# Nahuel-M/StereoVisionArray

Hardware: AMD Instinct MI355X
Metric: Mdisparities/sec (W·H·D/s) at 1080p D=128 (higher is better)
Workload: dtype u16

## Files before the change

### stereovisionarray_amd/csrc/sgm_common.h

```cpp
#pragma once

#include <utility>

#include "sva_device.h"
#include "sva_internal.h"
#include "sva_tuning.h"

namespace sva {
namespace sgm {

template <class F, int... S>
__device__ __forceinline__ void for_seq_impl(std::integer_sequence<int, S...>, F&& f) {
    (f(std::integral_constant<int, S>{}), ...);
}
template <int N, class F>
__device__ __forceinline__ void for_seq(F&& f) {
    for_seq_impl(std::make_integer_sequence<int, N>{}, static_cast<F&&>(f));
}

constexpr unsigned INF2 = 0x7fff7fffu;

struct PathGeom {
    int W, H, D;
    int P1, P2;
    int blk_h;
    int blk_w;
    size_t vol;
    int ckpt;
    int ns;
    size_t ckvol;
    int nsy;
    size_t ckvvol;
    int npair;
    size_t cstr, lstr, ckstr, ckvstr;
    int pair;
    int dreal;
};


typedef __amdgpu_buffer_rsrc_t rsrc_t;


constexpr int kStoreNT = 2;

__device__ __forceinline__ rsrc_t make_rsrc(const void* base, size_t bytes) {
    return __builtin_amdgcn_make_buffer_rsrc(const_cast<void*>(base), (short)0,
                                             (int)(unsigned)bytes, 0x00020000);
}

template <int NW>
struct Words {
    unsigned w[NW];
};

template <int NW, int AUX = tune::kCLoadAux>
__device__ __forceinline__ Words<NW> bload(rsrc_t r, unsigned off) {
    Words<NW> o;
    if constexpr (NW == 1) {
        o.w[0] = __builtin_amdgcn_raw_buffer_load_b32(r, off, 0, AUX);
    } else if constexpr (NW == 2) {
        auto v = __builtin_amdgcn_raw_buffer_load_b64(r, off, 0, AUX);
        o.w[0] = v[0]; o.w[1] = v[1];
    } else if constexpr (NW == 3) {
        auto v = __builtin_amdgcn_raw_buffer_load_b96(r, off, 0, AUX);
        o.w[0] = v[0]; o.w[1] = v[1]; o.w[2] = v[2];
    } else {
        auto v = __builtin_amdgcn_raw_buffer_load_b128(r, off, 0, AUX);
        o.w[0] = v[0]; o.w[1] = v[1]; o.w[2] = v[2]; o.w[3] = v[3];
    }
    return o;
}

template <int NW, int AUX = kStoreNT>
__device__ __forceinline__ void bstore(rsrc_t r, unsigned off, const unsigned (&w)[NW]) {
    if constexpr (NW == 1) {
        __builtin_amdgcn_raw_buffer_store_b32(w[0], r, off, 0, AUX);
    } else if constexpr (NW == 2) {
        typedef unsigned v2u __attribute__((ext_vector_type(2)));
        __builtin_amdgcn_raw_buffer_store_b64((v2u){w[0], w[1]}, r, off, 0, AUX);
    } else if constexpr (NW == 3) {
        typedef unsigned v3u __attribute__((ext_vector_type(3)));
        __builtin_amdgcn_raw_buffer_store_b96((v3u){w[0], w[1], w[2]}, r, off, 0, AUX);
    } else {
        typedef unsigned v4u __attribute__((ext_vector_type(4)));
        __builtin_amdgcn_raw_buffer_store_b128((v4u){w[0], w[1], w[2], w[3]}, r, off, 0, AUX);
    }
}

__device__ __forceinline__ unsigned add3(unsigned a, unsigned b, unsigned c) {
    unsigned r;
    asm("v_add3_u32 %0, %1, %2, %3" : "=v"(r) : "v"(a), "v"(b), "v"(c));
    return r;
}

template <bool DIAG>
struct Cursor {
    int x;
    unsigned off;
    __device__ __forceinline__ bool advance(int rx, unsigned stride, int W, unsigned WD) {
        off += stride;
        if constexpr (DIAG) {
            x += rx;
            const bool hi = x >= W, lo = x < 0;
            x = hi ? x - W : (lo ? x + W : x);
            off = hi ? off - WD : (lo ? off + WD : off);
            return hi || lo;
        }
        return false;
    }
};

__device__ __forceinline__ unsigned min3_u16x2(unsigned a, unsigned b, unsigned c) {
    unsigned r;
    asm("v_pk_minimum3_f16 %0, %1, %2, %3" : "=v"(r) : "v"(a), "v"(b), "v"(c));
    return r;
}

template <int NP>
__device__ __forceinline__ unsigned lane_min_u16(const unsigned (&A)[NP]) {
    unsigned mm[NP];
#pragma unroll
    for (int j = 0; j < NP; j++) mm[j] = A[j];
    int n = NP;
#pragma unroll
    for (int it = 0; it < 4; it++) {
        if (n > 1) {
            int o = 0, i = 0;
#pragma unroll
            for (int q = 0; q < 8; q++) {
                if (i + 2 < n) { mm[o++] = min3_u16x2(mm[i], mm[i + 1], mm[i + 2]); i += 3; }
                else if (i + 1 < n) { mm[o++] = as_u32(vmin2(as_v2(mm[i]), as_v2(mm[i + 1]))); i += 2; }
                else if (i < n) { mm[o++] = mm[i]; i += 1; }
            }
            n = o;
        }
    }
    const u16x2 mf = as_v2(mm[0]);
    return mf.x < mf.y ? mf.x : mf.y;
}

template <int DPL> __host__ __device__ constexpr int pair_d(int j, int h) {
    return tune::kSplitPairs ? j + h * (DPL / 2) : 2 * j + h;
}
template <int DPL> __host__ __device__ constexpr int pair_of(int e) {
    return tune::kSplitPairs ? e % (DPL / 2) : e >> 1;
}
template <int DPL> __host__ __device__ constexpr int half_of(int e) {
    return tune::kSplitPairs ? e / (DPL / 2) : e & 1;
}

template <int DPL>
__device__ __forceinline__ void words_to_pairs(const unsigned (&w)[DPL / 4], unsigned (&A)[DPL / 2]) {
    constexpr int NW = DPL / 4, NP = DPL / 2;
    if constexpr (tune::kSplitPairs != 0) {
#pragma unroll
        for (int j = 0; j < NP; j++) {
            constexpr unsigned Z = 0x0cu;
            const int el = j, eh = j + NP;
            const unsigned sel = (unsigned)(el & 3) | (Z << 8) | ((4u + (unsigned)(eh & 3)) << 16) | (Z << 24);
            A[j] = __builtin_amdgcn_perm(w[eh >> 2], w[el >> 2], sel);
        }
    } else {
#pragma unroll
        for (int q = 0; q < NW; q++) unpack4(w[q], A[2 * q], A[2 * q + 1]);
    }
}

template <int DPL>
__device__ __forceinline__ void pairs_to_words(const unsigned (&A)[DPL / 2], unsigned (&ow)[DPL / 4]) {
    constexpr int NW = DPL / 4, NP = DPL / 2;
    if constexpr (tune::kSplitPairs != 0) {
        unsigned T[NP / 2];
#pragma unroll
        for (int i = 0; i < NP / 2; i++) T[i] = __builtin_amdgcn_perm(A[2 * i + 1], A[2 * i], 0x06020400u);
        if constexpr (NP == 2) {
            ow[0] = T[0];
        } else {
#pragma unroll
            for (int q = 0; q < NW; q++) {
                const int e0 = 4 * q, e2 = 4 * q + 2;
                const int a = (e0 % NP) / 2, ha = e0 / NP, b = (e2 % NP) / 2, hb = e2 / NP;
                const unsigned sel = (unsigned)(2 * ha) | ((unsigned)(2 * ha + 1) << 8) |
                                     ((unsigned)(4 + 2 * hb) << 16) | ((unsigned)(5 + 2 * hb) << 24);
                ow[q] = __builtin_amdgcn_perm(T[b], T[a], sel);
            }
        }
    } else {
#pragma unroll
        for (int w = 0; w < NW; w++) ow[w] = pack4(A[2 * w], A[2 * w + 1]);
    }
}

struct Edges {
    unsigned X = INF2, Y = INF2;
};

template <int DPL, bool PIN = false>
__device__ __forceinline__ void sgm_step_c(const unsigned (&c)[DPL / 2], unsigned (&A)[DPL / 2],
                                           unsigned& m, unsigned (&ow)[DPL / 4], unsigned P1,
                                           unsigned P2, Edges& e) {
    constexpr int NP = DPL / 2;
    e.X = row_shr1(A[NP - 1], e.X);
    e.Y = row_shl1(A[0], e.Y);
    const unsigned X = e.X, Y = e.Y;
    unsigned lo[NP], hi[NP];
    if constexpr (tune::kSplitPairs != 0) {
#pragma unroll
        for (int j = 0; j < NP; j++) {
            lo[j] = j == 0 ? __builtin_amdgcn_alignbit(A[NP - 1], X, 16) : A[j - 1];
            hi[j] = j == NP - 1 ? __builtin_amdgcn_alignbit(Y, A[0], 16) : A[j + 1];
        }
    } else {
        unsigned M[NP];
        M[0] = __builtin_amdgcn_alignbit(A[0], X, 16);
#pragma unroll
        for (int j = 1; j < NP; j++) M[j] = __builtin_amdgcn_alignbit(A[j], A[j - 1], 16);
        const unsigned Qlast = __builtin_amdgcn_alignbit(Y, A[NP - 1], 16);
#pragma unroll
        for (int j = 0; j < NP; j++) {
            lo[j] = M[j];
            hi[j] = j < NP - 1 ? M[j + 1] : Qlast;
        }
    }
    unsigned K, mP2;
    asm("v_mul_i32_i24_e32 %0, 0xfffeffff, %1" : "=v"(K) : "v"(m));
    if constexpr (tune::kStepMadP2 != 0) {
        asm("v_mad_u32_u24 %0, %1, %2, %3" : "=&v"(mP2) : "v"(m), "s"(0x10001u), "v"(P2 * 0x10001u));
    } else {
        mP2 = P2 * 0x10001u - K;
    }
    u16x2 t[NP];
#pragma unroll
    for (int j = 0; j < NP; j++) t[j] = vmin2(as_v2(lo[j]), as_v2(hi[j]));
    unsigned tp[NP];
    if constexpr (tune::kStepAddU32 != 0) {
        const unsigned P1x2 = P1 * 0x10001u;
#pragma unroll
        for (int j = 0; j < NP; j++) tp[j] = as_u32(t[j]) + P1x2;
    } else {
#pragma unroll
        for (int j = 0; j < NP; j++) tp[j] = as_u32(t[j] + splat2(P1));
    }
#pragma unroll
    for (int j = 0; j < NP; j++) A[j] = add3(min3_u16x2(tp[j], A[j], mP2), c[j], K);
    pairs_to_words<DPL>(A, ow);
    m = row_min_u32<PIN>(lane_min_u16<NP>(A));
}

template <int DPL>
__device__ __forceinline__ void sgm_step_c(const unsigned (&c)[DPL / 2], unsigned (&A)[DPL / 2],
                                           unsigned& m, unsigned (&ow)[DPL / 4], unsigned P1,
                                           unsigned P2) {
    Edges e;
    sgm_step_c<DPL>(c, A, m, ow, P1, P2, e);
}

template <int DPL, bool PIN = false>
__device__ __forceinline__ void sgm_step(const unsigned (&cw)[DPL / 4], unsigned (&A)[DPL / 2],
                                         unsigned& m, unsigned (&ow)[DPL / 4], unsigned P1,
                                         unsigned P2, Edges& e) {
    unsigned c[DPL / 2];
    words_to_pairs<DPL>(cw, c);
    sgm_step_c<DPL, PIN>(c, A, m, ow, P1, P2, e);
}

__device__ __forceinline__ void dir_of(int r, int& rx, int& ry) {
    constexpr int T[8][2] = {{1, 0}, {-1, 0}, {0, 1}, {0, -1}, {1, 1}, {-1, -1}, {-1, 1}, {1, -1}};
    rx = T[r][0];
    ry = T[r][1];
}

template <int DPL> constexpr int pf_h() {
    return DPL == 4 ? tune::kPfH4 : DPL == 8 ? tune::kPfH8 : DPL == 12 ? tune::kPfH12 : tune::kPfH16;
}
template <int DPL> constexpr int pf_v() {
    return DPL == 4 ? tune::kPfV4 : DPL == 8 ? tune::kPfV8 : DPL == 12 ? tune::kPfV12 : tune::kPfV16;
}


template <int DPL, bool DIAG, int PF, int CKPT = 0, int SL = 0>
__device__ __forceinline__ void path_line(rsrc_t rC, rsrc_t rL, const PathGeom& g, int rx, int ry,
                                          int line, int k, rsrc_t rCK) {
    constexpr int NW = DPL / 4, NP = DPL / 2;
    const int W = g.W, H = g.H, D = g.D;
    const unsigned P1 = (unsigned)g.P1, P2 = (unsigned)g.P2;
    const int steps = ry == 0 ? W : H;
    const unsigned WD = (unsigned)W * (unsigned)D;
    const unsigned stride = (unsigned)((ry * W + rx) * D);
    int x0, y0;
    if (ry == 0) { y0 = line; x0 = rx > 0 ? 0 : W - 1; }
    else { y0 = ry > 0 ? 0 : H - 1; x0 = line; }
    Cursor<false> cc;
    cc.x = x0;
    cc.off = ((unsigned)y0 * (unsigned)W + (unsigned)x0) * (unsigned)D + (unsigned)(k * DPL);
    Cursor<false> pc = cc;
    constexpr bool STATIC_HITS = DPL <= tune::kStaticCkptHitsMaxDpl && (CKPT == 1 || CKPT == 2) &&
                                 SL > 0 && PF % (1 << SL) == 0;
    int lead = 0;
    if constexpr (STATIC_HITS) {
        constexpr int SEG = 1 << SL;
        lead = CKPT == 1 ? (rx > 0 ? 0 : (SEG - W % SEG) % SEG) : (ry > 0 ? 0 : (SEG - H % SEG) % SEG);
        pc.off -= (unsigned)lead * stride;
    }
    const int nsteps = steps + lead;
    int twc = 0, twp = 0, Tc = 0, Tp = 0;
    if constexpr (DIAG) {
        const int j = (int)((threadIdx.x >> 4) & 3);
        const int l0 = __builtin_amdgcn_readfirstlane(line - j);
        twc = twp = rx > 0 ? W - line : line + 1;
        Tc = Tp = rx > 0 ? W - l0 - 3 : l0 + 1;
    }
    const bool narrow = W < 4;

    unsigned A[NP];
#pragma unroll
    for (int j = 0; j < NP; j++) A[j] = 0u;
    unsigned m = 0u;
    Edges edges;

    Words<NW> ring[PF];
#pragma unroll
    for (int p = 0; p < PF; p++) {
        ring[p] = bload<NW>(rC, pc.off);
        if constexpr (STATIC_HITS) {
#pragma unroll
            for (int w = 0; w < NW; w++) ring[p].w[w] = p < lead ? 0u : ring[p].w[w];
        }
        pc.off += stride;
        if constexpr (DIAG) {
            if (p < PF - 1) {
                const bool w = p + 1 == twp;
                const unsigned fixed = rx > 0 ? pc.off - WD : pc.off + WD;
                pc.off = w ? fixed : pc.off;
                twp = w ? twp + W : twp;
            }
        }
    }
    if constexpr (DIAG) {
        while (Tp + 3 < PF) Tp += W;
    }

    auto step = [&](int p, bool refill, int ts) {
        unsigned cw[NW];
#pragma unroll
        for (int w = 0; w < NW; w++) cw[w] = ring[p].w[w];
        unsigned ow[NW];
        sgm_step<DPL>(cw, A, m, ow, P1, P2, edges);
        if constexpr (CKPT == 1 && STATIC_HITS) {
            constexpr int SEG = 1 << SL;
            if ((p & (SEG - 1)) == SEG - 1) {
                const int x = rx > 0 ? ts : W - 1 - (ts - lead);
                if (rx > 0 ? x + 1 < W : x > 0)
                    bstore<NW, tune::kCkptStoreAux>(rCK, ((unsigned)(y0 * g.ns + (x >> SL)) * (unsigned)D +
                                             (unsigned)(k * DPL)), ow);
            }
        } else if constexpr (CKPT == 2 && STATIC_HITS) {
            constexpr int SEG = 1 << SL;
            if ((p & (SEG - 1)) == SEG - 1) {
                const int y = ry > 0 ? ts : H - 1 - (ts - lead);
                if (ry > 0 ? y + 1 < H : y > 0)
                    bstore<NW, tune::kCkptStoreAux>(rCK, ((unsigned)((y >> SL) * W + x0) * (unsigned)D +
                                             (unsigned)(k * DPL)), ow);
            }
        } else if constexpr (CKPT == 1) {
            const int x = rx > 0 ? ts : W - 1 - ts;
            constexpr int SEG = 1 << SL;
            const bool hit = rx > 0 ? (((x + 1) & (SEG - 1)) == 0 && x + 1 < W)
                                    : ((x & (SEG - 1)) == 0 && x > 0);
            if (__builtin_expect(hit, 0))
                bstore<NW, tune::kCkptStoreAux>(rCK, ((unsigned)(y0 * g.ns + (x >> SL)) * (unsigned)D +
                                         (unsigned)(k * DPL)), ow);
        } else if constexpr (CKPT == 3) {
            const int y = ry > 0 ? ts : H - 1 - ts;
            constexpr int SEG = 1 << SL;
            const bool hit = ry > 0 ? (((y + 1) & (SEG - 1)) == 0 && y + 1 < H)
                                    : ((y & (SEG - 1)) == 0 && y > 0);
            if (__builtin_expect(hit, 0))
                bstore<NW, tune::kCkptStoreAux>(rCK, cc.off - (unsigned)(y - (y >> SL)) * WD, ow);
        } else if constexpr (CKPT == 2) {
            const int y = ry > 0 ? ts : H - 1 - ts;
            constexpr int SEG = 1 << SL;
            const bool hit = ry > 0 ? (((y + 1) & (SEG - 1)) == 0 && y + 1 < H)
                                    : ((y & (SEG - 1)) == 0 && y > 0);
            if (__builtin_expect(hit, 0))
                bstore<NW, tune::kCkptStoreAux>(rCK, ((unsigned)((y >> SL) * W + x0) * (unsigned)D +
                                         (unsigned)(k * DPL)), ow);
        } else {
            bstore<NW>(rL, cc.off, ow);
        }
        cc.off += stride;
        if constexpr (DIAG) {
            const int ec = ts + 1 - Tc;
            const int ep = ts + PF - Tp;
            const bool cev = narrow || (unsigned)ec < 4u;
            const bool pev = refill && (narrow || (unsigned)ep < 4u);
            if (__builtin_expect(cev || pev, 0)) {
                if (cev) {
                    const bool wrapped = ts + 1 == twc;
                    const unsigned fixed = rx > 0 ? cc.off - WD : cc.off + WD;
                    cc.off = wrapped ? fixed : cc.off;
                    twc = wrapped ? twc + W : twc;
#pragma unroll
                    for (int j = 0; j < NP; j++) A[j] = wrapped ? 0u : A[j];
                    m = wrapped ? 0u : m;
                    if (ec == 3) Tc += W;
                }
                if (pev) {
                    const bool wrapped = ts + PF == twp;
                    const unsigned fixed = rx > 0 ? pc.off - WD : pc.off + WD;
                    pc.off = wrapped ? fixed : pc.off;
                    twp = wrapped ? twp + W : twp;
                    if (ep == 3) Tp += W;
                }
            }
        }
        if (refill) {
            __builtin_amdgcn_sched_barrier(0);
            ring[p] = bload<NW>(rC, pc.off);
            pc.off += stride;
            __builtin_amdgcn_sched_barrier(0);
        }
    };

    int t = 0;
    for (; t + PF <= nsteps; t += PF) {
#pragma unroll
        for (int p = 0; p < PF; p++) step(p, true, t + p);
    }
#pragma unroll
    for (int p = 0; p < PF; p++)
        if (t + p < nsteps) step(p, false, t + p);
}



template <int NW>
__device__ __forceinline__ void unpack_add(const unsigned (&w)[NW], unsigned (&S)[2 * NW]) {
    unsigned a[2 * NW];
    words_to_pairs<4 * NW>(w, a);
#pragma unroll
    for (int j = 0; j < 2 * NW; j++) S[j] += a[j];
}

template <int DPL, bool PAD, bool PIN = false>
__device__ __forceinline__ void state_from_words(const Words<DPL / 4>& w, unsigned (&A)[DPL / 2],
                                                 unsigned& m, const unsigned (&padm)[DPL / 2]) {
    constexpr int NP = DPL / 2;
    words_to_pairs<DPL>(w.w, A);
    if constexpr (PAD) {
#pragma unroll
        for (int j = 0; j < NP; j++) A[j] |= padm[j] & 0x00ff00ffu;
    }
    if constexpr (tune::kStateMinTree) {
        m = row_min_u32<PIN>(lane_min_u16<NP>(A));
    } else {
        unsigned mm = 0xffffffffu;
#pragma unroll
        for (int j = 0; j < NP; j++) {
            const unsigned lo = A[j] & 0xffffu, hi = A[j] >> 16;
            mm = mm < lo ? mm : lo;
            mm = mm < hi ? mm : hi;
        }
        m = row_min_u32<PIN>(mm);
    }
}
template <int DPL, bool PAD, bool PIN = false>
__device__ __forceinline__ void load_state(rsrc_t r, unsigned off, unsigned (&A)[DPL / 2],
                                           unsigned& m, const unsigned (&padm)[DPL / 2]) {
    state_from_words<DPL, PAD, PIN>(bload<DPL / 4>(r, off), A, m, padm);
}

template <int DPL, int PF, int SL>
__device__ __forceinline__ void pair_line(rsrc_t rC, rsrc_t rE, const PathGeom& g, int rx, int line,
                                          int role, int k, rsrc_t rCK) {
    constexpr int NW = DPL / 4, NP = DPL / 2, SEG = 1 << SL;
    static_assert(PF >= SEG, "the lead steps sit in the prefetch prologue");
    const int W = g.W, H = g.H;
    const unsigned uW = (unsigned)W, uD = (unsigned)g.D;
    const unsigned WD = uW * uD;
    const unsigned P1 = (unsigned)g.P1, P2 = (unsigned)g.P2;
    const unsigned lane_d = (unsigned)(k * DPL);
    const int nseg = (H + SEG - 1) >> SL;
    const int qs = nseg >> 1;
    const int M = qs << SL;
    const bool up = role != 0;
    auto wrap = [&](int x) { return x >= W ? x - W : (x < 0 ? x + W : x); };
    auto col_of = [&](int y) {
        const int x = (line + rx * y) % W;
        return x < 0 ? x + W : x;
    };

    unsigned A1[NP], m1 = 0u;
    {
        const int n1 = M > H - M ? M : H - M;
        const int lead = n1 - (up ? H - M : M);
        const int ry = up ? -1 : 1, rxl = up ? -rx : rx;
        const int yv = up ? H - 1 + lead : -lead;
        const int xv = col_of(yv);
        const unsigned stride = (unsigned)((ry * W + rxl) * g.D);
        const unsigned wfix = rxl > 0 ? 0u - WD : WD;
        unsigned coff = (unsigned)(yv * W + xv) * uD + lane_d;
        unsigned poff = coff;
        int twc = rxl > 0 ? W - xv : xv + 1, twp = twc;
        const int zT = 1 - (n1 - M) - SEG, zB = H - 1 + (n1 - (H - M)) - (M + SEG);
        const int z0 = up ? zB : zT;
        const int zn = up ? H - (M + SEG) : M - 2 * SEG + 1;
#pragma unroll
        for (int j = 0; j < NP; j++) A1[j] = 0u;
        Edges e1;
        Words<NW> ring[PF];
#pragma unroll
        for (int p = 0; p < PF; p++) {
            ring[p] = bload<NW>(rC, poff);
#pragma unroll
            for (int w = 0; w < NW; w++) ring[p].w[w] = p < lead ? 0u : ring[p].w[w];
            poff += stride;
            if (p < PF - 1) {
                const bool wr = p + 1 == twp;
                poff = wr ? poff + wfix : poff;
                twp = wr ? twp + W : twp;
            }
        }
        auto step = [&](int p, bool refill, int ts) {
            unsigned cw[NW];
#pragma unroll
            for (int w = 0; w < NW; w++) cw[w] = ring[p].w[w];
            unsigned ow[NW];
            sgm_step<DPL>(cw, A1, m1, ow, P1, P2, e1);
            if (__builtin_expect((((zT + ts) & (SEG - 1)) == 0) | (((zB - ts) & (SEG - 1)) == 0), 0)) {
                const int zc = up ? z0 - ts : z0 + ts;
                if ((zc & (SEG - 1)) == 0 && zc >= 0 && zc < zn) {
                    const int y = zc + (up ? M + SEG : SEG - 1);
                    bstore<NW, tune::kCkptStoreAux>(rCK, coff - (unsigned)(y - (y >> SL)) * WD, ow);
                }
            }
            coff += stride;
            const bool cwr = ts + 1 == twc;
            const bool pwr = refill && ts + PF == twp;
            if (__builtin_expect(__builtin_amdgcn_ballot_w64(cwr || pwr) != 0, 0)) {
                coff = cwr ? coff + wfix : coff;
                twc = cwr ? twc + W : twc;
#pragma unroll
                for (int j = 0; j < NP; j++) A1[j] = cwr ? 0u : A1[j];
                m1 = cwr ? 0u : m1;
                poff = pwr ? poff + wfix : poff;
                twp = pwr ? twp + W : twp;
            }
            if (refill) {
                __builtin_amdgcn_sched_barrier(0);
                ring[p] = bload<NW>(rC, poff);
                poff += stride;
                __builtin_amdgcn_sched_barrier(0);
            }
        };
        int t = 0;
        for (; t + PF <= n1; t += PF) {
#pragma unroll
            for (int p = 0; p < PF; p++) step(p, true, t + p);
        }
#pragma unroll
        for (int p = 0; p < PF; p++)
            if (t + p < n1) step(p, false, t + p);
    }
    asm volatile("s_waitcnt vmcnt(0)" ::: "memory");

    const int nit = nseg - qs;
    const int xdn = rx > 0 ? 0 : W - 1, xup = rx > 0 ? W - 1 : 0;
    unsigned padm[NP];
#pragma unroll
    for (int j = 0; j < NP; j++) {
        const int dl = k * DPL + pair_d<DPL>(j, 0), dh = k * DPL + pair_d<DPL>(j, 1);
        padm[j] = (dl >= g.dreal ? 0x0000ffffu : 0u) | (dh >= g.dreal ? 0xffff0000u : 0u);
    }
    auto seg_of = [&](int i) {
        const int s = up ? qs - 1 - i : qs + i;
        return s < 0 ? 0 : s;
    };
    int s8 = (SEG * rx) % W;
    s8 = s8 < 0 ? s8 + W : s8;
    const int ds8 = up ? -s8 : s8;
    struct SegLoads {
        Words<NW> c[SEG], ck;
    };
    auto issue = [&](int s, int x, SegLoads& b) {
        const int xa = wrap(x - rx);
#pragma unroll
        for (int r = 0; r < SEG; r++) {
            b.c[r] = bload<NW>(rC, ((unsigned)((s << SL) + r) * uW + (unsigned)x) * uD + lane_d);
            x = wrap(x + rx);
        }
        const bool has = up ? s > 0 : s + 1 < nseg;
        const unsigned o = ((unsigned)(up ? s - 1 : s + 1) * uW + (unsigned)(up ? xa : x)) * uD + lane_d;
        b.ck = bload<NW, 16>(rCK, has ? o : lane_d);
    };
    auto reset_if = [&](bool rs, unsigned (&A)[NP], unsigned& m) {
        if (__builtin_expect(__builtin_amdgcn_ballot_w64(rs) != 0, 0)) {
#pragma unroll
            for (int j = 0; j < NP; j++) A[j] = rs ? 0u : A[j];
            m = rs ? 0u : m;
        }
    };

    unsigned Ad[NP], md = up ? 0u : m1, Au[NP], mu = up ? m1 : 0u;
#pragma unroll
    for (int j = 0; j < NP; j++) {
        Ad[j] = up ? 0u : A1[j];
        Au[j] = up ? A1[j] : 0u;
    }
    Edges ed, eu;
    SegLoads cur, nxt;
    int xs = col_of(seg_of(0) << SL), xn = xs;
    issue(seg_of(0), xs, cur);
    for (int i = 0; i < nit; i++) {
        __builtin_amdgcn_sched_barrier(0);
        if (i + 1 < nit) {
            xn = wrap(xs + ds8);
            issue(seg_of(i + 1), xn, nxt);
        }
        __builtin_amdgcn_sched_barrier(0);
        const int s = seg_of(i);
        const bool act = !up || i < qs;
        const int y0 = s << SL;
        const int nr = H - y0 < SEG ? H - y0 : SEG;
        int x[SEG];
        x[0] = xs;
#pragma unroll
        for (int r = 1; r < SEG; r++) x[r] = wrap(x[r - 1] + rx);
        {
            const bool has = up ? s > 0 : s + 1 < nseg;
            unsigned Ak[NP], mk;
            state_from_words<DPL, true>(cur.ck, Ak, mk, padm);
#pragma unroll
            for (int j = 0; j < NP; j++) {
                const unsigned a = has ? Ak[j] : 0u;
                Ad[j] = up ? a : Ad[j];
                Au[j] = up ? Au[j] : a;
            }
            mk = has ? mk : 0u;
            md = up ? mk : md;
            mu = up ? mu : mk;
        }
        unsigned Dn[SEG][NW];
        auto down_row = [&](int r, const Words<NW>& c) {
            unsigned cp[NP], ow[NW], t[NP];
            words_to_pairs<DPL>(c.w, cp);
            sgm_step_c<DPL>(cp, Ad, md, ow, P1, P2, ed);
#pragma unroll
            for (int j = 0; j < NP; j++) t[j] = Ad[j] - cp[j];
            pairs_to_words<DPL>(t, Dn[r]);
        };
        auto up_row = [&](const Words<NW>& c, unsigned (&e)[NW]) {
            unsigned cp[NP], ow[NW], t[NP];
            words_to_pairs<DPL>(c.w, cp);
            sgm_step_c<DPL>(cp, Au, mu, ow, P1, P2, eu);
#pragma unroll
            for (int j = 0; j < NP; j++) t[j] = Au[j] - cp[j];
            pairs_to_words<DPL>(t, e);
        };
        const bool inner = rx > 0 ? x[0] >= 1 && x[0] + SEG <= W - 1 : x[0] - SEG >= 0 && x[0] <= W - 2;
        if (__builtin_expect(__builtin_amdgcn_ballot_w64(!inner || nr != SEG || !act) == 0, 1)) {
            unsigned Up[SEG][NW];
            const unsigned off0 = ((unsigned)y0 * uW + (unsigned)x[0]) * uD + lane_d;
            const unsigned stride = (unsigned)((W + rx) * (int)uD);
            for_seq<SEG>([&](auto I) {
                constexpr int rd = decltype(I)::value, ru = SEG - 1 - rd;
                down_row(rd, cur.c[rd]);
                up_row(cur.c[ru], Up[ru]);
                if constexpr (rd >= SEG / 2) {
                    unsigned e[NW];
#pragma unroll
                    for (int w = 0; w < NW; w++) e[w] = Dn[rd][w] + Up[rd][w];
                    bstore<NW>(rE, off0 + (unsigned)rd * stride, e);
#pragma unroll
                    for (int w = 0; w < NW; w++) e[w] = Dn[ru][w] + Up[ru][w];
                    bstore<NW>(rE, off0 + (unsigned)ru * stride, e);
                }
            });
        } else {
            for_seq<SEG>([&](auto R) {
                constexpr int r = decltype(R)::value;
                if (r < nr && act) {
                    reset_if(x[r] == xdn, Ad, md);
                    down_row(r, cur.c[r]);
                }
            });
            for_seq<SEG>([&](auto Q) {
                constexpr int r = SEG - 1 - decltype(Q)::value;
                if (r < nr && act) {
                    reset_if(x[r] == xup, Au, mu);
                    unsigned e[NW];
                    up_row(cur.c[r], e);
#pragma unroll
                    for (int w = 0; w < NW; w++) e[w] += Dn[r][w];
                    bstore<NW>(rE, ((unsigned)(y0 + r) * uW + (unsigned)x[r]) * uD + lane_d, e);
                }
            });
        }
        if (i + 1 < nit) {
            cur = nxt;
            xs = xn;
        }
    }
}

}
}
```

### stereovisionarray_amd/csrc/sgm_paths.hip

```cpp
#include "sgm_common.h"
#include "sva_tuning.h"

namespace sva {
namespace {

using namespace sgm;

constexpr int PATH_BLOCK = 256;
constexpr int LINES_PER_BLOCK = PATH_BLOCK / 16;
constexpr int PAIR_LINES = LINES_PER_BLOCK / 2;

template <int DPL, bool PAIR>
__global__ __launch_bounds__(PATH_BLOCK) void sgm_paths_kernel(const uint8_t* __restrict__ C,
                                                               uint8_t* __restrict__ L8,
                                                               uint8_t* __restrict__ CK,
                                                               uint8_t* __restrict__ CKV,
                                                               PathGeom g) {
    int b = blockIdx.x, r, lb, f;
    if constexpr (PAIR) {
        f = 0;
        const int npb = 4 * g.blk_w;
        if (b < npb) {
            r = 4 + 2 * (b & 1);
            lb = b >> 1;
            __builtin_amdgcn_s_setprio(3);
        } else if (b < npb + 2 * g.blk_h) {
            b -= npb;
            r = b / g.blk_h;
            lb = b - r * g.blk_h;
            __builtin_amdgcn_s_setprio(1);
        } else {
            b -= npb + 2 * g.blk_h;
            r = 2 + (b & 1);
            lb = b >> 1;
        }
    } else if (b < 2 * g.blk_h * g.npair) {
        f = b / (2 * g.blk_h);
        b -= f * 2 * g.blk_h;
        r = b / g.blk_h;
        lb = b - r * g.blk_h;
        __builtin_amdgcn_s_setprio(1);
    } else {
        b -= 2 * g.blk_h * g.npair;
        f = b / (6 * g.blk_w);
        b -= f * 6 * g.blk_w;
        r = 2 + b % 6;
        lb = b / 6;
    }
    C += (size_t)f * g.cstr;
    L8 += (size_t)f * g.lstr;
    if (g.ckpt) {
        CK += (size_t)f * g.ckstr;
        CKV += (size_t)f * g.ckvstr;
    }
    int line = lb * LINES_PER_BLOCK + (threadIdx.x >> 4);
    int role = 0;
    if constexpr (PAIR) {
        if (r >= 4) {
            const int row = (int)(threadIdx.x >> 4);
            line = lb * PAIR_LINES + 2 * (row >> 2) + (row & 1);
            role = (row >> 1) & 1;
        }
    }
    const int k = threadIdx.x & 15;
    const int nlines = r < 2 ? g.H : g.W;
    if (line >= nlines) return;
    int rx, ry;
    dir_of(r, rx, ry);
    const rsrc_t rC = make_rsrc(C, g.vol);
    constexpr int SL = DPL <= 8 ? tune::kWtahvTileLog2 : tune::kWtahvTileLog2Wide;
    constexpr bool DOWN = diag_ckpt_down(DPL), UP = diag_ckpt_up(DPL);
    if constexpr (PAIR) {
        if (r >= 4) {
            const int pr = r == 4 ? 0 : 1;
            const rsrc_t rCK = make_rsrc(CKV + (size_t)(2 + pr) * g.ckvvol, g.ckvvol);
            const rsrc_t rE = make_rsrc(L8 + (size_t)pr * g.vol, g.vol);
            pair_line<DPL, pf_v<DPL>(), SL>(rC, rE, g, rx, line, role, k, rCK);
        } else if (r >= 2) {
            const rsrc_t rCK = make_rsrc(CKV + (size_t)(r - 2) * g.ckvvol, g.ckvvol);
            path_line<DPL, false, pf_v<DPL>(), 2, SL>(rC, rC, g, rx, ry, line, k, rCK);
        } else {
            const rsrc_t rCK = make_rsrc(CK + (size_t)r * g.ckvol, g.ckvol);
            path_line<DPL, false, pf_h<DPL>(), 1, SL>(rC, rC, g, rx, ry, line, k, rCK);
        }
    } else if (r >= 4 && g.ckpt && (ry > 0 ? DOWN : UP)) {
        const int plane = ry > 0 ? 2 + (r == 4 ? 0 : 1) : 2 + (DOWN ? 2 : 0) + (r == 5 ? 0 : 1);
        const rsrc_t rCK = make_rsrc(CKV + (size_t)plane * g.ckvvol, g.ckvvol);
        path_line<DPL, true, pf_v<DPL>(), 3, SL>(rC, rC, g, rx, ry, line, k, rCK);
    } else if (r >= 4) {
        const int slot = !g.ckpt ? r
                       : DOWN ? (r == 5 ? 0 : 1)
                       : UP ? (r == 4 ? 0 : 1)
                       : r - 4;
        const rsrc_t rL = make_rsrc(L8 + (size_t)slot * g.vol, g.vol);
        path_line<DPL, true, pf_v<DPL>()>(rC, rL, g, rx, ry, line, k, rL);
    } else if (r >= 2 && g.ckpt) {
        const rsrc_t rCK = make_rsrc(CKV + (size_t)(r - 2) * g.ckvvol, g.ckvvol);
        path_line<DPL, false, pf_v<DPL>(), 2, SL>(rC, rC, g, rx, ry, line, k, rCK);
    } else if (r >= 2) {
        const rsrc_t rL = make_rsrc(L8 + (size_t)r * g.vol, g.vol);
        path_line<DPL, false, pf_v<DPL>()>(rC, rL, g, rx, ry, line, k, rL);
    } else if (g.ckpt) {
        const rsrc_t rCK = make_rsrc(CK + (size_t)r * g.ckvol, g.ckvol);
        path_line<DPL, false, pf_h<DPL>(), 1, SL>(rC, rC, g, rx, ry, line, k, rCK);
    } else {
        const rsrc_t rL = make_rsrc(L8 + (size_t)r * g.vol, g.vol);
        path_line<DPL, false, pf_h<DPL>()>(rC, rL, g, rx, ry, line, k, rL);
    }
}

template <int DPL, bool EN>
void paths_launch(bool pair, dim3 grid, hipStream_t s, hipEvent_t start, hipEvent_t stop,
                  const uint8_t* C, uint8_t* L8, uint8_t* CK, uint8_t* CKV, const PathGeom& g) {
    if constexpr (EN) {
        if (pair) {
            hipExtLaunchKernelGGL((sgm_paths_kernel<DPL, true>), grid, dim3(PATH_BLOCK), 0, s, start,
                                  stop, 0, C, L8, CK, CKV, g);
            return;
        }
    }
    hipExtLaunchKernelGGL((sgm_paths_kernel<DPL, false>), grid, dim3(PATH_BLOCK), 0, s, start, stop,
                          0, C, L8, CK, CKV, g);
}

}

bool paths_supported(int D) { return D == 64 || D == 128 || D == 192 || D == 256; }

TileGeom tile_geom(int W, int H, int D) {
    TileGeom t;
    t.seg_log2 = D <= 128 ? tune::kWtahvTileLog2 : tune::kWtahvTileLog2Wide;
    const int seg = 1 << t.seg_log2;
    t.ntx = (W + 15) >> 4;
    t.nty = (H + seg - 1) >> t.seg_log2;
    t.nsx = (W + seg - 1) >> t.seg_log2;
    t.hck_bytes = 2 * (size_t)H * t.nsx * D;
    t.vck_bytes = 2 * (size_t)t.nty * W * D;
    const int dpl = D / 16;
    const int ndp = (diag_ckpt_down(dpl) ? 2 : 0) + (diag_ckpt_up(dpl) ? 2 : 0);
    t.dck_bytes = (size_t)ndp / 2 * t.vck_bytes;
    t.nvol = 4 - ndp;
    return t;
}

bool diag_pair_enabled(int D) {
    return (D == 64 && tune::kDiagPair4) || (D == 128 && tune::kDiagPair8) ||
           (D == 192 && tune::kDiagPair12) || (D == 256 && tune::kDiagPair16);
}

hipError_t launch_paths(Ctx& c, const uint8_t* C, int W, int H, int D, int P1, int P2,
                        uint8_t* L8, uint8_t* CK, uint8_t* CKV, int npair, bool pair, int dreal) {
    DispatchTimer t(c, "sgm_paths");
    PathGeom g;
    g.W = W; g.H = H; g.D = D; g.P1 = P1; g.P2 = P2;
    g.blk_h = (H + LINES_PER_BLOCK - 1) / LINES_PER_BLOCK;
    g.blk_w = (W + LINES_PER_BLOCK - 1) / LINES_PER_BLOCK;
    g.vol = (size_t)W * H * D;
    if ((CK == nullptr) != (CKV == nullptr)) return hipErrorInvalidValue;
    g.ckpt = CK ? 2 : 0;
    const TileGeom tg = tile_geom(W, H, D);
    g.nsy = tg.nty;
    g.ckvvol = tg.vck_bytes / 2;
    g.ns = tg.nsx;
    g.ckvol = tg.hck_bytes / 2;
    if (g.vol >= (size_t)1 << 32) return hipErrorInvalidValue;
    if (npair < 1 || (npair > 1 && !CK)) return hipErrorInvalidValue;
    g.npair = npair;
    g.cstr = g.vol;
    g.lstr = (size_t)tg.nvol * g.vol;
    g.ckstr = tg.hck_bytes;
    g.ckvstr = tg.vck_bytes + tg.dck_bytes;
    if (pair && (!CK || npair != 1 || 2 * P2 > 255 || !diag_pair_enabled(D) ||
                 tile_geom(W, H, D).nvol != 4))
        return hipErrorInvalidValue;
    g.pair = pair ? 1 : 0;
    g.dreal = dreal > 0 && dreal < D ? dreal : D;
    dim3 grid((unsigned)((2 * g.blk_h + 6 * g.blk_w) * npair));
    t.used = true;
    switch (D) {
        case 64: paths_launch<4, tune::kDiagPair4 != 0>(pair, grid, c.stream, t.start, t.stop, C, L8, CK, CKV, g); break;
        case 128: paths_launch<8, tune::kDiagPair8 != 0>(pair, grid, c.stream, t.start, t.stop, C, L8, CK, CKV, g); break;
        case 192: paths_launch<12, tune::kDiagPair12 != 0>(pair, grid, c.stream, t.start, t.stop, C, L8, CK, CKV, g); break;
        case 256: paths_launch<16, tune::kDiagPair16 != 0>(pair, grid, c.stream, t.start, t.stop, C, L8, CK, CKV, g); break;
        default: t.used = false; return hipErrorInvalidValue;
    }
    return hipGetLastError();
}

}
```

### stereovisionarray_amd/csrc/sva_api.cpp

```cpp
#include <hip/hip_runtime.h>

#include <algorithm>
#include <cstdio>
#include <cstring>
#include <new>
#include <string>
#include <functional>
#include <thread>
#include <vector>

#include "sva_internal.h"
#include "sva_tuning.h"

using namespace sva;

namespace sva {

hipEvent_t KernelTimer::get_event() {
    if (!pool.empty()) {
        hipEvent_t e = pool.back();
        pool.pop_back();
        return e;
    }
    hipEvent_t e = nullptr;
    if (hipEventCreate(&e) != hipSuccess) return nullptr;
    return e;
}

void KernelTimer::begin(hipStream_t s, const char*, hipEvent_t* start_out) {
    hipEvent_t e = get_event();
    if (e && hipEventRecord(e, s) == hipSuccess) *start_out = e;
    else *start_out = nullptr;
}

void KernelTimer::end(hipStream_t s, const char* name, hipEvent_t start) {
    hipEvent_t e = get_event();
    if (!e) return;
    if (hipEventRecord(e, s) != hipSuccess) { pool.push_back(e); return; }
    pending.push_back(Pending{name, start, e});
}

hipError_t KernelTimer::resolve() {
    hipError_t st = hipSuccess;
    for (auto& p : pending) {
        float ms = 0.f;
        hipError_t e = hipEventSynchronize(p.stop);
        if (e == hipSuccess) e = hipEventElapsedTime(&ms, p.start, p.stop);
        if (e != hipSuccess) st = e;
        auto& t = totals[p.name];
        t.first += ms;
        t.second += 1;
        pool.push_back(p.start);
        pool.push_back(p.stop);
    }
    pending.clear();
    return st;
}

void KernelTimer::release_all() {
    for (auto& p : pending) {
        (void)hipEventDestroy(p.start);
        (void)hipEventDestroy(p.stop);
    }
    pending.clear();
    for (auto e : pool) (void)hipEventDestroy(e);
    pool.clear();
}

hipError_t DevBuf::ensure(size_t n) {
    if (n <= bytes && ptr) return hipSuccess;
    if (ptr) {
        (void)hipFree(ptr);
        ptr = nullptr;
        bytes = 0;
    }
    size_t want = std::max<size_t>(n, 256);
    hipError_t e = flags ? hipExtMallocWithFlags(&ptr, want, flags) : hipMalloc(&ptr, want);
    if (e != hipSuccess) {
        ptr = nullptr;
        return e;
    }
    bytes = want;
    return hipSuccess;
}

void DevBuf::release() {
    if (ptr) (void)hipFree(ptr);
    ptr = nullptr;
    bytes = 0;
}

}

namespace {

Ctx* as_ctx(void* p) { return static_cast<Ctx*>(p); }

int fail(Ctx* c, int code, const std::string& msg) {
    if (c) c->last_error = msg;
    return code;
}

int hip_fail(Ctx* c, hipError_t e, const char* what) {
    std::string m = std::string(what) + ": " + hipGetErrorString(e);
    if (e == hipErrorOutOfMemory || e == hipErrorMemoryAllocation)
        return fail(c, SVA_ERR_OUT_OF_MEMORY, m);
    return fail(c, SVA_ERR_DEVICE, m);
}

#define SVA_HIP(c, expr, what)                           \
    do {                                                 \
        hipError_t _e = (expr);                          \
        if (_e != hipSuccess) return hip_fail(c, _e, what); \
    } while (0)

#define SVA_CHECK_CTX(c)                                                       \
    do {                                                                       \
        if (!(c)) return SVA_ERR_INVALID_ARG;                                  \
        if (hipSetDevice((c)->device) != hipSuccess)                           \
            return fail(c, SVA_ERR_DEVICE, "hipSetDevice failed");             \
    } while (0)

int check_image(Ctx* c, const void* a, int W, int H, size_t pitch) {
    if (!a) return fail(c, SVA_ERR_INVALID_ARG, "null image pointer");
    if (W <= 0 || H <= 0) return fail(c, SVA_ERR_INVALID_ARG, "image size must be positive");
    if (pitch < (size_t)W) return fail(c, SVA_ERR_INVALID_ARG, "pitch smaller than width");
    if ((long long)W * H > (1ll << 31) - 1) return fail(c, SVA_ERR_INVALID_ARG, "image too large");
    return SVA_OK;
}

int check_sgm(Ctx* c, const sva_sgm_params* p, int W, int H, bool native = false) {
    if (!p) return fail(c, SVA_ERR_INVALID_ARG, "null params");
    if (p->D <= 0) return fail(c, SVA_ERR_INVALID_ARG, "D must be positive");
    const int Dp = padded_D(p->D);
    if (!Dp) return fail(c, SVA_ERR_UNSUPPORTED, "GPU path built for D in 1..256");
    if (native && !paths_supported(p->D))
        return fail(c, SVA_ERR_UNSUPPORTED,
                    "stage entry points take D in {64,128,192,256} (whole frames: any D <= 256)");
    if (p->dir < -255 || p->dir > 255 || p->dir_y < -255 || p->dir_y > 255 ||
        (p->dir == 0 && p->dir_y == 0))
        return fail(c, SVA_ERR_INVALID_ARG, "(dir, dir_y) must be a nonzero step, |comp| <= 255");
    if (p->dmin < 0) return fail(c, SVA_ERR_INVALID_ARG, "dmin must be >= 0");
    if (p->dmin + p->D > 65535)
        return fail(c, SVA_ERR_INVALID_ARG, "dmin + D must fit the u16 disparity map");
    if (p->P1 < 0 || p->P2 < 0 || p->P1 > 193 || p->P2 > 193)
        return fail(c, SVA_ERR_INVALID_ARG, "penalties must satisfy 0 <= P1, P2 <= 193");
    if (p->lr_check && p->lr_max_diff < 0)
        return fail(c, SVA_ERR_INVALID_ARG, "lr_max_diff must be >= 0");
    if (H > 65535) return fail(c, SVA_ERR_UNSUPPORTED, "H must be <= 65535");
    if (W > 0 && H > 0 && (unsigned long long)W * (unsigned long long)H * (unsigned)Dp >=
                              (1ull << 32))
        return fail(c, SVA_ERR_UNSUPPORTED, "W*H*D must be < 2^32 (32-bit volume offsets)");
    return SVA_OK;
}

size_t pair_ckpt_bytes(const TileGeom& tg) { return tg.hck_bytes + tg.vck_bytes + tg.vck_bytes; }

int paths_wta(Ctx* c, const uint8_t* C, int W, int H, const sva_sgm_params* p, int Dp,
              uint16_t* disp, float* sub) {
    if (!wta_hv_supported(Dp)) return fail(c, SVA_ERR_UNSUPPORTED, "no tile pipeline for this D");
    const size_t nv = (size_t)W * H * (size_t)Dp;
    const TileGeom tg = tile_geom(W, H, Dp);
    const long long minpx = c->dbg_pair_min_pixels >= 0 ? (long long)c->dbg_pair_min_pixels
                                                        : tune::kDiagPairMinPixels;
    const bool pair = tg.nvol == 4 && diag_pair_ok(Dp, p->P2) && (long long)W * H >= minpx;
    SVA_HIP(c, c->paths.ensure(nv * (pair ? 2 : tg.nvol)), "path workspace");
    SVA_HIP(c, c->ckpt.ensure(pair ? pair_ckpt_bytes(tg) : tg.hck_bytes + tg.vck_bytes + tg.dck_bytes),
            "checkpoint workspace");
    uint8_t* L4 = (uint8_t*)c->paths.ptr;
    uint8_t* CK = (uint8_t*)c->ckpt.ptr;
    uint8_t* CKV = CK + tg.hck_bytes;
    SVA_HIP(c, launch_paths(*c, C, W, H, Dp, p->P1, p->P2, L4, CK, CKV, 1, pair, p->D), "paths launch");
    SVA_HIP(c, launch_wta_hv(*c, C, L4, CK, CKV, W, H, Dp, p->P1, p->P2, p->dmin, disp, sub, p->D, 1,
                             pair),
            "wta launch");
    c->last_diag_route = pair ? 1 : 0;
    return SVA_OK;
}

sva_tile_layout tile_layout(int W, int H, int D) {
    sva_tile_layout l;
    std::memset(&l, 0, sizeof(l));
    const TileGeom tg = tile_geom(W, H, D);
    l.seg = 1 << tg.seg_log2;
    l.nsx = tg.nsx;
    l.nsy = tg.nty;
    l.cost_bytes = (size_t)W * H * (size_t)D;
    l.diag_volumes = tg.nvol;
    l.diag_bytes = (size_t)tg.nvol * l.cost_bytes;
    l.hckpt_bytes = tg.hck_bytes;
    l.vckpt_bytes = tg.vck_bytes + tg.dck_bytes;
    return l;
}

int check_tile_buffers(Ctx* c, int W, int H, int D, const void* C, size_t C_bytes,
                       const void* diag, size_t diag_bytes, const void* hck, size_t hck_bytes,
                       const void* vck, size_t vck_bytes) {
    const sva_tile_layout l = tile_layout(W, H, D);
    if (!C || (!diag && l.diag_bytes) || !hck || !vck)
        return fail(c, SVA_ERR_INVALID_ARG, "null stage buffer");
    if (C_bytes < l.cost_bytes) return fail(c, SVA_ERR_INVALID_ARG, "cost buffer smaller than [H][W][D]");
    if (diag_bytes < l.diag_bytes)
        return fail(c, SVA_ERR_INVALID_ARG, "diagonal volume buffer smaller than [nvol][H][W][D]");
    if (hck_bytes < l.hckpt_bytes)
        return fail(c, SVA_ERR_INVALID_ARG, "horizontal checkpoint buffer smaller than [2][H][nsx][D]");
    if (vck_bytes < l.vckpt_bytes)
        return fail(c, SVA_ERR_INVALID_ARG, "row checkpoint buffer smaller than [np][nsy][W][D]");
    return SVA_OK;
}

int run_sgm_device(Ctx* c, const uint8_t* left, const uint8_t* right, int W, int H, size_t pitch,
                   const sva_sgm_params* p, uint16_t* disp, float* sub) {
    const int Dp = padded_D(p->D);
    const size_t np = (size_t)W * H, nv = np * (size_t)Dp;
    int s;
    SVA_HIP(c, c->cost.ensure(nv), "cost workspace");
    uint8_t* C = (uint8_t*)c->cost.ptr;
    uint16_t* dr = nullptr;
    if (p->lr_check) {
        SVA_HIP(c, c->disp_r.ensure(np * 2), "lr workspace");
        dr = (uint16_t*)c->disp_r.ptr;
    }
    if (p->dir_y == 0 && Dp >= tune::kCensusCostMinD && census_cost_supported(Dp)) {
        SVA_HIP(c, launch_census_cost(*c, left, right, W, H, pitch, Dp, p->dmin, p->dir, C, p->D),
                "cost launch");
        if ((s = paths_wta(c, C, W, H, p, Dp, disp, sub))) return s;
        if (p->lr_check) {
            SVA_HIP(c, launch_census_cost(*c, right, left, W, H, pitch, Dp, p->dmin, -p->dir, C,
                                          p->D),
                    "cost launch");
            if ((s = paths_wta(c, C, W, H, p, Dp, dr, nullptr))) return s;
            SVA_HIP(c, launch_lr_check(*c, disp, dr, sub, W, H, p->dir, 0, p->lr_max_diff,
                                       p->invalid),
                    "lr launch");
        }
        return SVA_OK;
    }
    if (census_cost2_supported(Dp, p->dir, p->dir_y)) {
        SVA_HIP(c, launch_census_cost2(*c, left, right, W, H, pitch, Dp, p->dmin, p->dir,
                                       p->dir_y, C, p->D),
                "cost launch");
        if ((s = paths_wta(c, C, W, H, p, Dp, disp, sub))) return s;
        if (p->lr_check) {
            SVA_HIP(c, launch_census_cost2(*c, right, left, W, H, pitch, Dp, p->dmin, -p->dir,
                                           -p->dir_y, C, p->D),
                    "cost launch");
            if ((s = paths_wta(c, C, W, H, p, Dp, dr, nullptr))) return s;
            SVA_HIP(c, launch_lr_check(*c, disp, dr, sub, W, H, p->dir, p->dir_y, p->lr_max_diff,
                                       p->invalid),
                    "lr launch");
        }
        return SVA_OK;
    }
    SVA_HIP(c, c->census_l.ensure(np * 8), "census workspace");
    SVA_HIP(c, c->census_r.ensure(np * 8), "census workspace");
    uint64_t* cl = (uint64_t*)c->census_l.ptr;
    uint64_t* cr = (uint64_t*)c->census_r.ptr;
    SVA_HIP(c, launch_census_pair(*c, left, right, W, H, pitch, cl, cr), "census launch");
    SVA_HIP(c, launch_cost2(*c, cl, cr, W, H, Dp, p->dmin, p->dir, p->dir_y, C, p->D),
            "cost launch");
    if ((s = paths_wta(c, C, W, H, p, Dp, disp, sub))) return s;
    if (p->lr_check) {
        SVA_HIP(c, launch_cost2(*c, cr, cl, W, H, Dp, p->dmin, -p->dir, -p->dir_y, C, p->D),
                "cost launch");
        if ((s = paths_wta(c, C, W, H, p, Dp, dr, nullptr))) return s;
        SVA_HIP(c, launch_lr_check(*c, disp, dr, sub, W, H, p->dir, p->dir_y, p->lr_max_diff,
                                   p->invalid),
                "lr launch");
    }
    return SVA_OK;
}

int run_sgm_batch(Ctx* c, const sva_pair_d* jobs, int n, int W, int H, size_t pitch,
                  uint16_t* maps, float* sub) {
    const sva_sgm_params* p = &jobs[0].params;
    const int Dp = padded_D(p->D);
    const size_t np = (size_t)W * H, nv = np * (size_t)Dp;
    const TileGeom tg = tile_geom(W, H, Dp);
    const size_t ckb = tg.hck_bytes + tg.vck_bytes + tg.dck_bytes;
    const int sb = tune::kBatchSubFrames > 0 ? std::min(n, tune::kBatchSubFrames) : n;
    const int nsub = (n + sb - 1) / sb;
    SVA_HIP(c, c->cost.ensure(nv * n), "cost workspace");
    SVA_HIP(c, c->paths.ensure(nv * tg.nvol * sb), "path workspace");
    SVA_HIP(c, c->ckpt.ensure(ckb * sb), "checkpoint workspace");
    uint8_t* C = (uint8_t*)c->cost.ptr;
    const int ns = std::min(n, tune::kBatchCostStreams);
    if (ns > 1) {
        while ((int)c->side.size() < ns) {
            hipStream_t s = nullptr;
            SVA_HIP(c, hipStreamCreateWithFlags(&s, hipStreamNonBlocking), "side stream");
            c->side.push_back(s);
        }
        while ((int)c->side_done.size() < ns * nsub) {
            hipEvent_t e = nullptr;
            SVA_HIP(c, hipEventCreateWithFlags(&e, hipEventDisableTiming), "side stream event");
            c->side_done.push_back(e);
        }
        if (!c->fork) SVA_HIP(c, hipEventCreateWithFlags(&c->fork, hipEventDisableTiming), "fork event");
        SVA_HIP(c, hipEventRecord(c->fork, c->stream), "fork");
        for (int s = 0; s < ns; s++) SVA_HIP(c, hipStreamWaitEvent(c->side[s], c->fork, 0), "fork");
    }
    SVA_HIP(c, c->census_side.ensure(np * 16 * (size_t)std::max(ns, 1)), "census workspace");
    const hipStream_t own = c->stream;
    const int fail_at = c->dbg_fail_cost_at;
    c->dbg_fail_cost_at = 0;
    int st = SVA_OK;
    for (int i = 0; i < n && st == SVA_OK; i++) {
        const sva_sgm_params* q = &jobs[i].params;
        uint8_t* Ci = C + (size_t)i * nv;
        if (ns > 1) c->stream = c->side[i % ns];
        hipError_t e;
        if (i + 1 == fail_at) {
            e = hipErrorLaunchFailure;
        } else if (q->dir_y == 0 && Dp >= tune::kCensusCostMinD && census_cost_supported(Dp)) {
            e = launch_census_cost(*c, jobs[i].left, jobs[i].right, W, H, pitch, Dp, q->dmin, q->dir,
                                   Ci, q->D);
        } else if (census_cost2_supported(Dp, q->dir, q->dir_y)) {
            e = launch_census_cost2(*c, jobs[i].left, jobs[i].right, W, H, pitch, Dp, q->dmin,
                                    q->dir, q->dir_y, Ci, q->D);
        } else {
            uint64_t* cl = (uint64_t*)c->census_side.ptr + (size_t)(i % std::max(ns, 1)) * 2 * np;
            uint64_t* cr = cl + np;
            e = launch_census_pair(*c, jobs[i].left, jobs[i].right, W, H, pitch, cl, cr);
            if (e == hipSuccess)
                e = launch_cost2(*c, cl, cr, W, H, Dp, q->dmin, q->dir, q->dir_y, Ci, q->D);
        }
        if (e == hipSuccess && ns > 1 && (i + ns >= n || (i + ns) / sb != i / sb))
            e = hipEventRecord(c->side_done[(size_t)(i / sb) * ns + i % ns], c->stream);
        c->stream = own;
        if (e != hipSuccess) st = hip_fail(c, e, "cost launch");
    }
    for (int j = 0; j < nsub && st == SVA_OK; j++) {
        const int i0 = j * sb, m = std::min(sb, n - i0);
        hipError_t e = hipSuccess;
        if (ns > 1) {
            for (int s = 0; s < ns && s < n && e == hipSuccess; s++) {
                bool has = false;
                for (int i = i0; i < i0 + m; i++) has = has || i % ns == s;
                if (has) e = hipStreamWaitEvent(c->stream, c->side_done[(size_t)j * ns + s], 0);
            }
        }
        if (e != hipSuccess) { st = hip_fail(c, e, "join"); break; }
        uint8_t* L4 = (uint8_t*)c->paths.ptr;
        uint8_t* CK = (uint8_t*)c->ckpt.ptr;
        uint8_t* CKV = CK + tg.hck_bytes * m;
        const uint8_t* Cj = C + (size_t)i0 * nv;
        if ((e = launch_paths(*c, Cj, W, H, Dp, p->P1, p->P2, L4, CK, CKV, m)) != hipSuccess) {
            st = hip_fail(c, e, "paths launch");
            break;
        }
        if ((e = launch_wta_hv(*c, Cj, L4, CK, CKV, W, H, Dp, p->P1, p->P2, p->dmin,
                               maps + (size_t)i0 * np, p->subpixel ? sub + (size_t)i0 * np : nullptr,
                               p->D, m)) != hipSuccess) {
            st = hip_fail(c, e, "wta launch");
            break;
        }
    }
    if (st != SVA_OK && ns > 1) {
        for (int s = 0; s < ns; s++) {
            if (hipEventRecord(c->side_done[s], c->side[s]) != hipSuccess ||
                hipStreamWaitEvent(c->stream, c->side_done[s], 0) != hipSuccess)
                (void)hipStreamSynchronize(c->side[s]);
        }
    }
    return st;
}

int check_camera(Ctx* c, const sva_camera* cam) {
    if (!cam) return fail(c, SVA_ERR_INVALID_ARG, "null camera");
    return SVA_OK;
}

int run_ref_device(Ctx* c, const uint8_t* ref, const uint8_t* other, int W, int H, size_t pitch,
                   const uint8_t* mask, const sva_camera* cref, const sva_camera* coth, int k,
                   double t_near, double t_far, uint8_t* d8, uint16_t* d16, uint8_t* valid) {
    const size_t np = (size_t)W * H;
    SVA_HIP(c, c->census_l.ensure(np * 16), "endpoint workspace");
    SVA_HIP(c, c->census_r.ensure(np), "endpoint workspace");
    int32_t* ends = (int32_t*)c->census_l.ptr;
    uint8_t* ok = (uint8_t*)c->census_r.ptr;
    SVA_HIP(c, launch_ref_endpoints(*c, W, H, *cref, *coth, k, t_near, t_far, ends, ok),
            "endpoint launch");
    SVA_HIP(c, launch_ref_match(*c, ref, other, W, H, pitch, mask, ends, ok, k, d8, d16, valid),
            "match launch");
    return SVA_OK;
}

int check_ref_args(Ctx* c, int W, int H, int k, double t_near, double t_far) {
    if (k < 1) return fail(c, SVA_ERR_INVALID_ARG, "kernel half-size k must be >= 1");
    if (2LL * k >= W || 2LL * k >= H) return fail(c, SVA_ERR_INVALID_ARG, "image smaller than window");
    if (!(t_near > 0.0) || !(t_far > 0.0))
        return fail(c, SVA_ERR_INVALID_ARG, "ray parameters must be positive");
    if (W > 32767 || H > 32767)
        return fail(c, SVA_ERR_UNSUPPORTED, "Mode R supports W, H <= 32767");
    return SVA_OK;
}


int check_planes(Ctx* c, int W, int H, size_t pitch) {
    if (W <= 0 || H <= 0) return fail(c, SVA_ERR_INVALID_ARG, "image size must be positive");
    if (pitch < (size_t)W) return fail(c, SVA_ERR_INVALID_ARG, "pitch smaller than width");
    if ((long long)W * H > (1ll << 31) - 1) return fail(c, SVA_ERR_INVALID_ARG, "image too large");
    if (H > 65535) return fail(c, SVA_ERR_UNSUPPORTED, "H must be <= 65535 (gridDim.y)");
    return SVA_OK;
}

int check_window(Ctx* c, int window_size) {
    if (window_size < 1 || (window_size - 1) / 2 > 32)
        return fail(c, SVA_ERR_UNSUPPORTED, "window_size must give kernelSize (w-1)/2 in 0..32");
    return SVA_OK;
}

int run_improve(Ctx* c, const uint8_t* disp, const uint8_t* center, const uint8_t* const* images,
                const sva_camera* cams, int n, int W, int H, size_t pitch, const uint8_t* mask,
                int window_size, int strict, uint8_t* out,
                const std::function<int(int, const uint8_t**)>& fetch) {
    const size_t bytes = (size_t)H * pitch;
    SVA_HIP(c, c->shifted.ensure(bytes), "shift workspace");
    SVA_HIP(c, c->total.ensure(sizeof(long long)), "fault flag");
    int* fault = (int*)c->total.ptr;
    SVA_HIP(c, hipMemsetAsync(fault, 0, sizeof(int), c->stream), "memset");
    uint8_t* sh = (uint8_t*)c->shifted.ptr;
    const int k = (window_size - 1) / 2;
    for (int i = 0; i < n; i++) {
        const uint8_t* img = images ? images[i] : nullptr;
        int s;
        if (fetch && (s = fetch(i, &img))) return s;
        SVA_HIP(c, launch_shift_perspective(*c, cams[2 * i], cams[2 * i + 1], disp, img, W, H,
                                            pitch, sh, true), "shift launch");
        SVA_HIP(c, launch_refine(*c, disp, center, sh, mask, W, H, pitch, k, cams[2 * i],
                                 cams[2 * i + 1], out, fault), "refine launch");
    }
    if (strict) {
        int f = 0;
        SVA_HIP(c, hipMemcpyAsync(&f, fault, sizeof(int), hipMemcpyDeviceToHost, c->stream),
                "download");
        SVA_HIP(c, hipStreamSynchronize(c->stream), "sync");
        if (f)
            return fail(c, SVA_ERR_INVALID_ARG,
                        "a masked pixel's window leaves the image (the reference's ROI throws)");
    }
    return SVA_OK;
}

}

extern "C" {

void sva_sgm_params_default(sva_sgm_params* p) {
    if (!p) return;
    std::memset(p, 0, sizeof(*p));
    p->D = 128;
    p->dmin = 0;
    p->dir = -1;
    p->P1 = 10;
    p->P2 = 120;
    p->subpixel = 0;
    p->lr_check = 0;
    p->lr_max_diff = 1;
    p->invalid = 0xffff;
}

int sva_abi_version(void) { return SVA_ABI_VERSION; }

int sva_device_count(int* count) {
    if (!count) return SVA_ERR_INVALID_ARG;
    int n = 0;
    if (hipGetDeviceCount(&n) != hipSuccess) n = 0;
    *count = n;
    return SVA_OK;
}

const char* sva_status_string(int s) {
    switch (s) {
        case SVA_OK: return "ok";
        case SVA_ERR_INVALID_ARG: return "invalid argument";
        case SVA_ERR_UNSUPPORTED: return "unsupported configuration";
        case SVA_ERR_DEVICE: return "device error";
        case SVA_ERR_OUT_OF_MEMORY: return "out of device memory";
        case SVA_ERR_NO_DEVICE: return "no usable HIP device";
        default: return "unknown status";
    }
}

int sva_create(int device, void** out) {
    if (!out) return SVA_ERR_INVALID_ARG;
    *out = nullptr;
    int n = 0;
    if (hipGetDeviceCount(&n) != hipSuccess || n <= 0) return SVA_ERR_NO_DEVICE;
    if (device < 0 || device >= n) return SVA_ERR_INVALID_ARG;
    if (hipSetDevice(device) != hipSuccess) return SVA_ERR_DEVICE;
    Ctx* c = new (std::nothrow) Ctx();
    if (!c) return SVA_ERR_OUT_OF_MEMORY;
    c->device = device;
    if (hipStreamCreateWithFlags(&c->own_stream, hipStreamNonBlocking) != hipSuccess) {
        delete c;
        return SVA_ERR_DEVICE;
    }
    c->stream = c->own_stream;
    hipDeviceProp_t prop;
    if (hipGetDeviceProperties(&prop, device) == hipSuccess) c->cu_count = prop.multiProcessorCount;
    *out = c;
    return SVA_OK;
}

int sva_destroy(void* ctx) {
    Ctx* c = as_ctx(ctx);
    if (!c) return SVA_ERR_INVALID_ARG;
    (void)hipSetDevice(c->device);
    if (c->stream) (void)hipStreamSynchronize(c->stream);
    c->batch_lane.reset();
    for (hipStream_t s : c->side) {
        (void)hipStreamSynchronize(s);
        (void)hipStreamDestroy(s);
    }
    for (hipEvent_t e : c->side_done) (void)hipEventDestroy(e);
    if (c->fork) (void)hipEventDestroy(c->fork);
    c->census_side.release();
    for (DevBuf* b : {&c->census_l, &c->census_r, &c->cost, &c->paths, &c->ckpt, &c->scratch_u16,
                      &c->disp_r, &c->in_a, &c->in_b, &c->in_mask, &c->out_a, &c->out_b,
                      &c->out_c, &c->in_c, &c->shifted, &c->keys, &c->counts, &c->total, &c->ref_keys})
        b->release();
    c->timer.release_all();
    if (c->own_stream) (void)hipStreamDestroy(c->own_stream);
    delete c;
    return SVA_OK;
}

int sva_set_stream(void* ctx, void* stream) {
    Ctx* c = as_ctx(ctx);
    SVA_CHECK_CTX(c);
    c->stream = stream ? (hipStream_t)stream : c->own_stream;
    return SVA_OK;
}

int sva_synchronize(void* ctx) {
    Ctx* c = as_ctx(ctx);
    SVA_CHECK_CTX(c);
    SVA_HIP(c, hipStreamSynchronize(c->stream), "hipStreamSynchronize");
    return SVA_OK;
}

const char* sva_last_error(void* ctx) {
    Ctx* c = as_ctx(ctx);
    return c ? c->last_error.c_str() : "null context";
}

namespace {

int time_stage_set(Ctx* c, int W, int H, int D, int64_t* ns) {
    const TileGeom tg = tile_geom(W, H, D);
    const uint8_t* C = (const uint8_t*)c->cost.ptr;
    uint8_t* L4 = (uint8_t*)c->paths.ptr;
    uint8_t* CK = (uint8_t*)c->ckpt.ptr;
    hipEvent_t a = nullptr, b = nullptr;
    SVA_HIP(c, hipEventCreate(&a), "placement event");
    if (hipEventCreate(&b) != hipSuccess) {
        (void)hipEventDestroy(a);
        return fail(c, SVA_ERR_DEVICE, "placement event");
    }
    hipError_t e = hipSuccess;
    float best = 0.f;
    for (int r = 0; r < 4 && e == hipSuccess; r++) {
        e = hipEventRecord(a, c->stream);
        if (e == hipSuccess)
            e = launch_paths(*c, C, W, H, D, 10, 120, L4, CK, CK + tg.hck_bytes, 1,
                             tg.nvol == 4 && diag_pair_ok(D, 120) &&
                                 (long long)W * H >= tune::kDiagPairMinPixels);
        if (e == hipSuccess) e = hipEventRecord(b, c->stream);
        if (e == hipSuccess) e = hipEventSynchronize(b);
        float ms = 0.f;
        if (e == hipSuccess) e = hipEventElapsedTime(&ms, a, b);
        if (e == hipSuccess && r > 0) best = r == 1 ? ms : std::min(best, ms);
    }
    (void)hipEventDestroy(a);
    (void)hipEventDestroy(b);
    if (e != hipSuccess) return hip_fail(c, e, "placement timing");
    *ns = (int64_t)((double)best * 1e6);
    return SVA_OK;
}

int place_stage_buffers(Ctx* c, int W, int H, int D, int trials) {
    struct Set {
        DevBuf cost, paths, ckpt;
        int64_t ns = 0;
    };
    const bool timing = c->timer.enabled;
    c->timer.enabled = false;
    std::vector<Set> sets(1);
    int rc = time_stage_set(c, W, H, D, &sets[0].ns);
    const size_t set_bytes = c->cost.bytes + c->paths.bytes + c->ckpt.bytes;
    for (int t = 1; rc == SVA_OK && t < trials; t++) {
        size_t free_b = 0, total_b = 0;
        if (hipMemGetInfo(&free_b, &total_b) != hipSuccess) break;
        const size_t keep = std::max(total_b / 4, (size_t)16 << 30);
        if (free_b < set_bytes + keep) break;
        Set n;
        n.cost.flags = c->cost.flags;
        n.paths.flags = c->paths.flags;
        n.ckpt.flags = c->ckpt.flags;
        if (n.cost.ensure(c->cost.bytes) != hipSuccess || n.paths.ensure(c->paths.bytes) != hipSuccess ||
            n.ckpt.ensure(c->ckpt.bytes) != hipSuccess) {
            n.cost.release();
            n.paths.release();
            n.ckpt.release();
            (void)hipGetLastError();
            break;
        }
        std::swap(c->cost, n.cost);
        std::swap(c->paths, n.paths);
        std::swap(c->ckpt, n.ckpt);
        rc = time_stage_set(c, W, H, D, &n.ns);
        std::swap(c->cost, n.cost);
        std::swap(c->paths, n.paths);
        std::swap(c->ckpt, n.ckpt);
        sets.push_back(n);
    }
    c->timer.enabled = timing;
    size_t best = 0;
    int64_t worst = sets[0].ns;
    for (size_t i = 1; i < sets.size(); i++) {
        if (sets[i].ns < sets[best].ns) best = i;
        worst = std::max(worst, sets[i].ns);
    }
    if (rc == SVA_OK && best != 0) {
        std::swap(c->cost, sets[best].cost);
        std::swap(c->paths, sets[best].paths);
        std::swap(c->ckpt, sets[best].ckpt);
    }
    const int64_t kept = sets[rc == SVA_OK ? best : 0].ns;
    for (size_t i = 1; i < sets.size(); i++) {
        sets[i].cost.release();
        sets[i].paths.release();
        sets[i].ckpt.release();
    }
    if (rc != SVA_OK) return rc;
    c->placement_ns = kept;
    c->placement_worst_ns = worst;
    c->placement_paths = c->paths.ptr;
    return SVA_OK;
}

}

int sva_reserve(void* ctx, int W, int H, int D) {
    Ctx* c = as_ctx(ctx);
    SVA_CHECK_CTX(c);
    if (W <= 0 || H <= 0 || D <= 0) return fail(c, SVA_ERR_INVALID_ARG, "bad reserve size");
    if (padded_D(D)) D = padded_D(D);
    const size_t np = (size_t)W * H, nv = np * (size_t)D;
    SVA_HIP(c, c->census_l.ensure(np * 8), "reserve");
    SVA_HIP(c, c->census_r.ensure(np * 8), "reserve");
    SVA_HIP(c, c->cost.ensure(nv), "reserve");
    const TileGeom tg = tile_geom(W, H, D);
    const size_t ckb = tg.nvol == 4 && diag_pair_enabled(D)
                           ? pair_ckpt_bytes(tg)
                           : tg.hck_bytes + tg.vck_bytes + tg.dck_bytes;
    SVA_HIP(c, c->paths.ensure(nv * tg.nvol), "reserve");
    SVA_HIP(c, c->ckpt.ensure(ckb), "reserve");
    const int trials = c->placement_trials > 0 ? c->placement_trials : tune::kPlacementTrials;
    if (trials > 1 && wta_hv_supported(D) && nv < ((size_t)1 << 32) &&
        nv + nv * tg.nvol + ckb >= tune::kPlacementMinBytes && c->paths.ptr != c->placement_paths)
        return place_stage_buffers(c, W, H, D, trials);
    return SVA_OK;
}

int sva_set_path_kernel(void* ctx, int kernel) {
    Ctx* c = as_ctx(ctx);
    SVA_CHECK_CTX(c);
    if (kernel == SVA_PATH_KERNEL_FUSED)
        return fail(c, SVA_ERR_UNSUPPORTED,
                    "the census-fused path kernel was removed in ABI v4 (DESIGN.md §4.5)");
    if (kernel != SVA_PATH_KERNEL_COST_VOLUME && kernel != SVA_PATH_KERNEL_AUTO)
        return fail(c, SVA_ERR_INVALID_ARG, "unknown path kernel");
    return SVA_OK;
}

int sva_set_timing(void* ctx, int enable) {
    Ctx* c = as_ctx(ctx);
    SVA_CHECK_CTX(c);
    if (enable < 0 || enable > SVA_TIMING_AGG)
        return fail(c, SVA_ERR_INVALID_ARG, "timing mode must be 0, 1, 2 or 3");
    c->timer.enabled = enable != 0;
    c->timer.mode = enable;
    return SVA_OK;
}

int sva_reset_timing(void* ctx) {
    Ctx* c = as_ctx(ctx);
    SVA_CHECK_CTX(c);
    hipError_t e = c->timer.resolve();
    c->timer.totals.clear();
    if (e != hipSuccess) return hip_fail(c, e, "timer resolve");
    return SVA_OK;
}

int sva_set_debug(void* ctx, int key, int64_t value) {
    Ctx* c = as_ctx(ctx);
    SVA_CHECK_CTX(c);
    switch (key) {
        case SVA_DEBUG_PLANE_SPLIT:
            if (value < 0 || value > 16) return fail(c, SVA_ERR_INVALID_ARG, "plane split must be 0..16");
            c->dbg_plane_split = (int)value;
            return SVA_OK;
        case SVA_DEBUG_FAIL_COST_AT:
            if (value < 0 || value > (1 << 30)) return fail(c, SVA_ERR_INVALID_ARG, "bad frame index");
            c->dbg_fail_cost_at = (int)value;
            return SVA_OK;
        case SVA_DEBUG_PLACEMENT_TRIALS:
            if (value < 0 || value > 8) return fail(c, SVA_ERR_INVALID_ARG, "placement trials must be 0..8");
            c->placement_trials = (int)value;
            return SVA_OK;
        case SVA_DEBUG_DIAG_PAIR_MIN_PIXELS:
            if (value < -1) return fail(c, SVA_ERR_INVALID_ARG, "pair route threshold must be >= -1");
            c->dbg_pair_min_pixels = value;
            return SVA_OK;
        default:
            return fail(c, SVA_ERR_INVALID_ARG, "unknown or read-only debug key");
    }
}

int sva_get_debug(void* ctx, int key, int64_t* value) {
    Ctx* c = as_ctx(ctx);
    SVA_CHECK_CTX(c);
    if (!value) return fail(c, SVA_ERR_INVALID_ARG, "null value");
    switch (key) {
        case SVA_DEBUG_PLANE_SPLIT: *value = c->dbg_plane_split; return SVA_OK;
        case SVA_DEBUG_FAIL_COST_AT: *value = c->dbg_fail_cost_at; return SVA_OK;
        case SVA_DEBUG_PLACEMENT_TRIALS: *value = c->placement_trials; return SVA_OK;
        case SVA_DEBUG_PLACEMENT_NS: *value = c->placement_ns; return SVA_OK;
        case SVA_DEBUG_PLACEMENT_WORST_NS: *value = c->placement_worst_ns; return SVA_OK;
        case SVA_DEBUG_DIAG_ROUTE: *value = c->last_diag_route; return SVA_OK;
        case SVA_DEBUG_DIAG_PAIR_MIN_PIXELS:
            *value = c->dbg_pair_min_pixels >= 0 ? c->dbg_pair_min_pixels : (int64_t)tune::kDiagPairMinPixels;
            return SVA_OK;
        case SVA_DEBUG_SIDE_IDLE: {
            bool idle = true;
            for (hipStream_t s : c->side) {
                const hipError_t e = hipStreamQuery(s);
                if (e == hipErrorNotReady) idle = false;
                else if (e != hipSuccess) return hip_fail(c, e, "side stream query");
            }
            *value = idle ? 1 : 0;
            return SVA_OK;
        }
        default:
            return fail(c, SVA_ERR_INVALID_ARG, "unknown debug key");
    }
}

int sva_kernel_time(void* ctx, const char* name, double* total_ms, int64_t* count) {
    Ctx* c = as_ctx(ctx);
    SVA_CHECK_CTX(c);
    if (!name || !total_ms || !count) return fail(c, SVA_ERR_INVALID_ARG, "null argument");
    hipError_t e = c->timer.resolve();
    if (e != hipSuccess) return hip_fail(c, e, "timer resolve");
    auto it = c->timer.totals.find(name);
    *total_ms = it == c->timer.totals.end() ? 0.0 : it->second.first;
    *count = it == c->timer.totals.end() ? 0 : it->second.second;
    return SVA_OK;
}

int sva_disparity_sgm_d(void* ctx, const uint8_t* left, const uint8_t* right, int W, int H,
                        size_t pitch, const sva_sgm_params* p, uint16_t* disp, float* sub) {
    Ctx* c = as_ctx(ctx);
    SVA_CHECK_CTX(c);
    int s;
    if ((s = check_image(c, left, W, H, pitch)) || (s = check_image(c, right, W, H, pitch)) ||
        (s = check_sgm(c, p, W, H)))
        return s;
    if (!disp) return fail(c, SVA_ERR_INVALID_ARG, "null disparity output");
    return run_sgm_device(c, left, right, W, H, pitch, p, disp, p->subpixel ? sub : nullptr);
}

int sva_disparity_sgm_batch_d(void* ctx, const sva_pair_d* jobs, int n, int W, int H,
                              size_t pitch, uint16_t* maps, float* sub) {
    Ctx* c = as_ctx(ctx);
    SVA_CHECK_CTX(c);
    if (!jobs || n <= 0 || !maps) return fail(c, SVA_ERR_INVALID_ARG, "bad batch argument");
    int s;
    const sva_sgm_params* p0 = &jobs[0].params;
    for (int i = 0; i < n; i++) {
        const sva_sgm_params* q = &jobs[i].params;
        if ((s = check_image(c, jobs[i].left, W, H, pitch)) ||
            (s = check_image(c, jobs[i].right, W, H, pitch)) || (s = check_sgm(c, q, W, H)))
            return s;
        if (q->D != p0->D || q->dmin != p0->dmin || q->P1 != p0->P1 || q->P2 != p0->P2 ||
            q->subpixel != p0->subpixel)
            return fail(c, SVA_ERR_INVALID_ARG,
                        "a batch's pairs must share D, dmin, P1, P2 and subpixel");
        if (q->lr_check) return fail(c, SVA_ERR_UNSUPPORTED, "the batch route has no L/R check");
    }
    if (!wta_hv_supported(padded_D(p0->D)))
        return fail(c, SVA_ERR_UNSUPPORTED, "no tile pipeline for this D");
    const int Dp = padded_D(p0->D);
    const TileGeom tg = tile_geom(W, H, Dp);
    const size_t per = (size_t)W * H * (size_t)Dp * (1 + tg.nvol) + tg.hck_bytes + tg.vck_bytes +
                       tg.dck_bytes;
    int chunk = tune::kBatchMaxPairs;
    while (chunk > 1 && per * (size_t)chunk > tune::kBatchMaxBytes) chunk--;
    const size_t np = (size_t)W * H;
    for (int i0 = 0; i0 < n; i0 += chunk) {
        const int m = std::min(chunk, n - i0);
        if ((s = run_sgm_batch(c, jobs + i0, m, W, H, pitch, maps + (size_t)i0 * np,
                               sub ? sub + (size_t)i0 * np : nullptr)))
            return s;
    }
    return SVA_OK;
}

int sva_disparity_sgm(void* ctx, const uint8_t* left, const uint8_t* right, int W, int H,
                      size_t pitch, const sva_sgm_params* p, uint16_t* disp, float* sub) {
    Ctx* c = as_ctx(ctx);
    SVA_CHECK_CTX(c);
    int s;
    if ((s = check_image(c, left, W, H, pitch)) || (s = check_image(c, right, W, H, pitch)) ||
        (s = check_sgm(c, p, W, H)))
        return s;
    if (!disp) return fail(c, SVA_ERR_INVALID_ARG, "null disparity output");
    const bool want_sub = p->subpixel && sub;
    const size_t np = (size_t)W * H;
    SVA_HIP(c, c->in_a.ensure(np), "staging");
    SVA_HIP(c, c->in_b.ensure(np), "staging");
    SVA_HIP(c, c->out_a.ensure(np * 2), "staging");
    if (want_sub) SVA_HIP(c, c->out_b.ensure(np * 4), "staging");
    SVA_HIP(c, hipMemcpy2DAsync(c->in_a.ptr, W, left, pitch, W, H, hipMemcpyHostToDevice, c->stream),
            "upload");
    SVA_HIP(c, hipMemcpy2DAsync(c->in_b.ptr, W, right, pitch, W, H, hipMemcpyHostToDevice, c->stream),
            "upload");
    if ((s = run_sgm_device(c, (uint8_t*)c->in_a.ptr, (uint8_t*)c->in_b.ptr, W, H, W, p,
                            (uint16_t*)c->out_a.ptr, want_sub ? (float*)c->out_b.ptr : nullptr)))
        return s;
    SVA_HIP(c, hipMemcpyAsync(disp, c->out_a.ptr, np * 2, hipMemcpyDeviceToHost, c->stream),
            "download");
    if (want_sub)
        SVA_HIP(c, hipMemcpyAsync(sub, c->out_b.ptr, np * 4, hipMemcpyDeviceToHost, c->stream),
                "download");
    SVA_HIP(c, hipStreamSynchronize(c->stream), "sync");
    return SVA_OK;
}

int sva_census_d(void* ctx, const uint8_t* img, int W, int H, size_t pitch, uint64_t* census) {
    Ctx* c = as_ctx(ctx);
    SVA_CHECK_CTX(c);
    int s;
    if ((s = check_image(c, img, W, H, pitch))) return s;
    if (!census) return fail(c, SVA_ERR_INVALID_ARG, "null census output");
    SVA_HIP(c, launch_census(*c, img, W, H, pitch, census), "census launch");
    return SVA_OK;
}

int sva_cost_d(void* ctx, const uint64_t* cl, const uint64_t* cr, int W, int H,
               const sva_sgm_params* p, uint8_t* C) {
    Ctx* c = as_ctx(ctx);
    SVA_CHECK_CTX(c);
    int s;
    if ((s = check_sgm(c, p, W, H, true))) return s;
    if (!cl || !cr || !C || W <= 0 || H <= 0) return fail(c, SVA_ERR_INVALID_ARG, "bad argument");
    SVA_HIP(c, launch_cost2(*c, cl, cr, W, H, p->D, p->dmin, p->dir, p->dir_y, C), "cost launch");
    return SVA_OK;
}

int sva_census_cost_d(void* ctx, const uint8_t* left, const uint8_t* right, int W, int H,
                      size_t pitch, const sva_sgm_params* p, uint8_t* C) {
    Ctx* c = as_ctx(ctx);
    SVA_CHECK_CTX(c);
    int s;
    if ((s = check_sgm(c, p, W, H, true))) return s;
    if ((s = check_image(c, left, W, H, pitch))) return s;
    if ((s = check_image(c, right, W, H, pitch))) return s;
    if (!C) return fail(c, SVA_ERR_INVALID_ARG, "null cost output");
    if (p->dir_y == 0 && census_cost_supported(p->D)) {
        SVA_HIP(c, launch_census_cost(*c, left, right, W, H, pitch, p->D, p->dmin, p->dir, C),
                "cost launch");
        return SVA_OK;
    }
    if (!census_cost2_supported(p->D, p->dir, p->dir_y))
        return fail(c, SVA_ERR_UNSUPPORTED,
                    "census+cost kernel: D in {64,128,192,256}, 1-D steps or 2-D steps whose "
                    "primitive form has |dir_y| = 1 and |dir| <= 3");
    SVA_HIP(c, launch_census_cost2(*c, left, right, W, H, pitch, p->D, p->dmin, p->dir, p->dir_y, C),
            "cost launch");
    return SVA_OK;
}

int sva_paths_d(void* ctx, const uint8_t* C, int W, int H, const sva_sgm_params* p, uint8_t* L8) {
    Ctx* c = as_ctx(ctx);
    SVA_CHECK_CTX(c);
    int s;
    if ((s = check_sgm(c, p, W, H, true))) return s;
    if (!C || !L8 || W <= 0 || H <= 0) return fail(c, SVA_ERR_INVALID_ARG, "bad argument");
    SVA_HIP(c, launch_paths(*c, C, W, H, p->D, p->P1, p->P2, L8), "paths launch");
    return SVA_OK;
}

int sva_aggregate_d(void* ctx, const uint8_t* C, int W, int H, const sva_sgm_params* p,
                    uint16_t* S) {
    Ctx* c = as_ctx(ctx);
    SVA_CHECK_CTX(c);
    int s;
    if ((s = check_sgm(c, p, W, H, true))) return s;
    if (!C || !S || W <= 0 || H <= 0) return fail(c, SVA_ERR_INVALID_ARG, "bad argument");
    const size_t nv = (size_t)W * H * (size_t)p->D;
    SVA_HIP(c, c->paths.ensure(nv * 8), "path workspace");
    uint8_t* L8 = (uint8_t*)c->paths.ptr;
    SVA_HIP(c, launch_paths(*c, C, W, H, p->D, p->P1, p->P2, L8), "paths launch");
    SVA_HIP(c, launch_sum(*c, L8, W, H, p->D, S), "sum launch");
    return SVA_OK;
}

int sva_tile_layout_of(int W, int H, int D, sva_tile_layout* out) {
    if (!out || W <= 0 || H <= 0 || !paths_supported(D)) return SVA_ERR_INVALID_ARG;
    *out = tile_layout(W, H, D);
    return SVA_OK;
}

int sva_tile_check(int W, int H, int D, size_t C_bytes, size_t diag_bytes, size_t hckpt_bytes,
                   size_t vckpt_bytes) {
    if (W <= 0 || H <= 0 || !paths_supported(D)) return SVA_ERR_INVALID_ARG;
    const char one = 0;
    return check_tile_buffers(nullptr, W, H, D, &one, C_bytes, &one, diag_bytes, &one, hckpt_bytes,
                              &one, vckpt_bytes);
}

int sva_paths_tile_d(void* ctx, const uint8_t* C, size_t C_bytes, int W, int H,
                     const sva_sgm_params* p, uint8_t* diag, size_t diag_bytes, uint8_t* hckpt,
                     size_t hckpt_bytes, uint8_t* vckpt, size_t vckpt_bytes) {
    Ctx* c = as_ctx(ctx);
    SVA_CHECK_CTX(c);
    int s;
    if ((s = check_sgm(c, p, W, H, true))) return s;
    if ((s = check_tile_buffers(c, W, H, p->D, C, C_bytes, diag, diag_bytes, hckpt, hckpt_bytes,
                                vckpt, vckpt_bytes)))
        return s;
    SVA_HIP(c, launch_paths(*c, C, W, H, p->D, p->P1, p->P2, diag, hckpt, vckpt), "paths launch");
    return SVA_OK;
}

int sva_wta_hv_d(void* ctx, const uint8_t* C, size_t C_bytes, const uint8_t* diag,
                 size_t diag_bytes, const uint8_t* hckpt, size_t hckpt_bytes, const uint8_t* vckpt,
                 size_t vckpt_bytes, int W, int H, const sva_sgm_params* p, uint16_t* disp,
                 float* sub) {
    Ctx* c = as_ctx(ctx);
    SVA_CHECK_CTX(c);
    int s;
    if ((s = check_sgm(c, p, W, H, true))) return s;
    if ((s = check_tile_buffers(c, W, H, p->D, C, C_bytes, diag, diag_bytes, hckpt, hckpt_bytes,
                                vckpt, vckpt_bytes)))
        return s;
    if (!disp) return fail(c, SVA_ERR_INVALID_ARG, "null disparity output");
    SVA_HIP(c, launch_wta_hv(*c, C, diag, hckpt, vckpt, W, H, p->D, p->P1, p->P2, p->dmin, disp,
                             p->subpixel ? sub : nullptr),
            "wta launch");
    return SVA_OK;
}

int sva_wta_d(void* ctx, const uint16_t* S, int W, int H, const sva_sgm_params* p, uint16_t* disp,
              float* sub) {
    Ctx* c = as_ctx(ctx);
    SVA_CHECK_CTX(c);
    int s;
    if ((s = check_sgm(c, p, W, H, true))) return s;
    if (!S || !disp || W <= 0 || H <= 0) return fail(c, SVA_ERR_INVALID_ARG, "bad argument");
    SVA_HIP(c, launch_wta_from_sum(*c, S, W, H, p->D, p->dmin, disp, p->subpixel ? sub : nullptr),
            "wta launch");
    return SVA_OK;
}

int sva_ref_endpoints_d(void* ctx, int W, int H, const sva_camera* cref, const sva_camera* coth,
                        int k, double t_near, double t_far, int32_t* ends, uint8_t* valid) {
    Ctx* c = as_ctx(ctx);
    SVA_CHECK_CTX(c);
    int s;
    if ((s = check_camera(c, cref)) || (s = check_camera(c, coth)) ||
        (s = check_ref_args(c, W, H, k, t_near, t_far)))
        return s;
    if (!ends || !valid) return fail(c, SVA_ERR_INVALID_ARG, "null output");
    SVA_HIP(c, launch_ref_endpoints(*c, W, H, *cref, *coth, k, t_near, t_far, ends, valid),
            "endpoint launch");
    return SVA_OK;
}

int sva_disparity_ref_d(void* ctx, const uint8_t* ref, const uint8_t* other, int W, int H,
                        size_t pitch, const uint8_t* mask, const sva_camera* cref,
                        const sva_camera* coth, int k, double t_near, double t_far, uint8_t* d8,
                        uint16_t* d16, uint8_t* valid) {
    Ctx* c = as_ctx(ctx);
    SVA_CHECK_CTX(c);
    int s;
    if ((s = check_image(c, ref, W, H, pitch)) || (s = check_image(c, other, W, H, pitch)) ||
        (s = check_camera(c, cref)) || (s = check_camera(c, coth)) ||
        (s = check_ref_args(c, W, H, k, t_near, t_far)))
        return s;
    if (!d8) return fail(c, SVA_ERR_INVALID_ARG, "null disparity output");
    return run_ref_device(c, ref, other, W, H, pitch, mask, cref, coth, k, t_near, t_far, d8, d16,
                          valid);
}

int sva_disparity_ref(void* ctx, const uint8_t* ref, const uint8_t* other, int W, int H,
                      size_t pitch, const uint8_t* mask, const sva_camera* cref,
                      const sva_camera* coth, int k, double t_near, double t_far, uint8_t* d8,
                      uint16_t* d16, uint8_t* valid) {
    Ctx* c = as_ctx(ctx);
    SVA_CHECK_CTX(c);
    int s;
    if ((s = check_image(c, ref, W, H, pitch)) || (s = check_image(c, other, W, H, pitch)) ||
        (s = check_camera(c, cref)) || (s = check_camera(c, coth)) ||
        (s = check_ref_args(c, W, H, k, t_near, t_far)))
        return s;
    if (!d8) return fail(c, SVA_ERR_INVALID_ARG, "null disparity output");
    const size_t np = (size_t)W * H;
    SVA_HIP(c, c->in_a.ensure(np), "staging");
    SVA_HIP(c, c->in_b.ensure(np), "staging");
    SVA_HIP(c, c->out_a.ensure(np), "staging");
    if (mask) SVA_HIP(c, c->in_mask.ensure(np), "staging");
    if (d16) SVA_HIP(c, c->out_b.ensure(np * 2), "staging");
    if (valid) SVA_HIP(c, c->out_c.ensure(np), "staging");
    hipStream_t st = c->stream;
    SVA_HIP(c, hipMemcpy2DAsync(c->in_a.ptr, W, ref, pitch, W, H, hipMemcpyHostToDevice, st), "upload");
    SVA_HIP(c, hipMemcpy2DAsync(c->in_b.ptr, W, other, pitch, W, H, hipMemcpyHostToDevice, st), "upload");
    if (mask) SVA_HIP(c, hipMemcpyAsync(c->in_mask.ptr, mask, np, hipMemcpyHostToDevice, st), "upload");
    SVA_HIP(c, hipMemcpyAsync(c->out_a.ptr, d8, np, hipMemcpyHostToDevice, st), "upload");
    if (d16) SVA_HIP(c, hipMemcpyAsync(c->out_b.ptr, d16, np * 2, hipMemcpyHostToDevice, st), "upload");
    if (valid) SVA_HIP(c, hipMemcpyAsync(c->out_c.ptr, valid, np, hipMemcpyHostToDevice, st), "upload");
    if ((s = run_ref_device(c, (uint8_t*)c->in_a.ptr, (uint8_t*)c->in_b.ptr, W, H, W,
                            mask ? (uint8_t*)c->in_mask.ptr : nullptr, cref, coth, k, t_near,
                            t_far, (uint8_t*)c->out_a.ptr, d16 ? (uint16_t*)c->out_b.ptr : nullptr,
                            valid ? (uint8_t*)c->out_c.ptr : nullptr)))
        return s;
    SVA_HIP(c, hipMemcpyAsync(d8, c->out_a.ptr, np, hipMemcpyDeviceToHost, st), "download");
    if (d16) SVA_HIP(c, hipMemcpyAsync(d16, c->out_b.ptr, np * 2, hipMemcpyDeviceToHost, st), "download");
    if (valid) SVA_HIP(c, hipMemcpyAsync(valid, c->out_c.ptr, np, hipMemcpyDeviceToHost, st), "download");
    SVA_HIP(c, hipStreamSynchronize(st), "sync");
    return SVA_OK;
}

int sva_disparity_to_depth_d(void* ctx, const uint8_t* disp, int n, double cam_distance,
                             double f, double pixel_size, double* depth) {
    Ctx* c = as_ctx(ctx);
    SVA_CHECK_CTX(c);
    if (!disp || !depth || n < 0) return fail(c, SVA_ERR_INVALID_ARG, "bad argument");
    if (n == 0) return SVA_OK;
    SVA_HIP(c, launch_disp_to_depth(*c, disp, n, cam_distance, f, pixel_size, depth), "depth launch");
    return SVA_OK;
}

int sva_disparity_to_depth(void* ctx, const uint8_t* disp, int n, double cam_distance, double f,
                           double pixel_size, double* depth) {
    Ctx* c = as_ctx(ctx);
    SVA_CHECK_CTX(c);
    if (!disp || !depth || n < 0) return fail(c, SVA_ERR_INVALID_ARG, "bad argument");
    if (n == 0) return SVA_OK;
    SVA_HIP(c, c->in_a.ensure((size_t)n), "staging");
    SVA_HIP(c, c->out_a.ensure((size_t)n * 8), "staging");
    SVA_HIP(c, hipMemcpyAsync(c->in_a.ptr, disp, (size_t)n, hipMemcpyHostToDevice, c->stream),
            "upload");
    SVA_HIP(c, launch_disp_to_depth(*c, (uint8_t*)c->in_a.ptr, n, cam_distance, f, pixel_size,
                                    (double*)c->out_a.ptr), "depth launch");
    SVA_HIP(c, hipMemcpyAsync(depth, c->out_a.ptr, (size_t)n * 8, hipMemcpyDeviceToHost, c->stream),
            "download");
    SVA_HIP(c, hipStreamSynchronize(c->stream), "sync");
    return SVA_OK;
}

int check_fuse(Ctx* c, const uint16_t* disps, int n_maps, int W, int H, const double* b,
               const double* depth) {
    if (!disps || !b || !depth) return fail(c, SVA_ERR_INVALID_ARG, "null pointer");
    if (n_maps < 1 || n_maps > 32) return fail(c, SVA_ERR_UNSUPPORTED, "n_maps must be 1..32");
    if (W <= 0 || H <= 0) return fail(c, SVA_ERR_INVALID_ARG, "image size must be positive");
    return SVA_OK;
}

int sva_fuse_depth_d(void* ctx, const uint16_t* disps, int n_maps, int W, int H,
                     const double* baselines, double f, double pixel_size, uint16_t invalid,
                     double* depth, uint8_t* n_valid) {
    Ctx* c = as_ctx(ctx);
    SVA_CHECK_CTX(c);
    int s;
    if ((s = check_fuse(c, disps, n_maps, W, H, baselines, depth))) return s;
    double num[32];
    for (int i = 0; i < n_maps; i++) num[i] = baselines[i] * f;
    SVA_HIP(c, launch_fuse_depth(*c, disps, n_maps, (size_t)W * H, num, pixel_size, invalid,
                                 depth, n_valid), "fuse launch");
    return SVA_OK;
}

int sva_fuse_depth(void* ctx, const uint16_t* disps, int n_maps, int W, int H,
                   const double* baselines, double f, double pixel_size, uint16_t invalid,
                   double* depth, uint8_t* n_valid) {
    Ctx* c = as_ctx(ctx);
    SVA_CHECK_CTX(c);
    int s;
    if ((s = check_fuse(c, disps, n_maps, W, H, baselines, depth))) return s;
    const size_t np = (size_t)W * H, in_bytes = np * 2 * (size_t)n_maps;
    double num[32];
    for (int i = 0; i < n_maps; i++) num[i] = baselines[i] * f;
    SVA_HIP(c, c->in_a.ensure(in_bytes), "staging");
    SVA_HIP(c, c->out_a.ensure(np * 8), "staging");
    SVA_HIP(c, c->out_b.ensure(np), "staging");
    SVA_HIP(c, hipMemcpyAsync(c->in_a.ptr, disps, in_bytes, hipMemcpyHostToDevice, c->stream),
            "upload");
    SVA_HIP(c, launch_fuse_depth(*c, (const uint16_t*)c->in_a.ptr, n_maps, np, num, pixel_size,
                                 invalid, (double*)c->out_a.ptr, (uint8_t*)c->out_b.ptr),
            "fuse launch");
    SVA_HIP(c, hipMemcpyAsync(depth, c->out_a.ptr, np * 8, hipMemcpyDeviceToHost, c->stream),
            "download");
    if (n_valid)
        SVA_HIP(c, hipMemcpyAsync(n_valid, c->out_b.ptr, np, hipMemcpyDeviceToHost, c->stream),
                "download");
    SVA_HIP(c, hipStreamSynchronize(c->stream), "sync");
    return SVA_OK;
}

int sva_shift_perspective_d(void* ctx, const sva_camera* in_cam, const sva_camera* out_cam,
                            const uint8_t* disparity, const uint8_t* image, int W, int H,
                            size_t pitch, uint8_t* shifted) {
    Ctx* c = as_ctx(ctx);
    SVA_CHECK_CTX(c);
    int s;
    if ((s = check_planes(c, W, H, pitch)) || (s = check_camera(c, in_cam)) ||
        (s = check_camera(c, out_cam)))
        return s;
    if (!disparity || !image || !shifted) return fail(c, SVA_ERR_INVALID_ARG, "null plane");
    SVA_HIP(c, launch_shift_perspective(*c, *in_cam, *out_cam, disparity, image, W, H, pitch,
                                        shifted), "shift launch");
    return SVA_OK;
}

int sva_shift_perspective(void* ctx, const sva_camera* in_cam, const sva_camera* out_cam,
                          const uint8_t* disparity, const uint8_t* image, int W, int H,
                          size_t pitch, uint8_t* shifted) {
    Ctx* c = as_ctx(ctx);
    SVA_CHECK_CTX(c);
    int s;
    if ((s = check_planes(c, W, H, pitch)) || (s = check_camera(c, in_cam)) ||
        (s = check_camera(c, out_cam)))
        return s;
    if (!disparity || !image || !shifted) return fail(c, SVA_ERR_INVALID_ARG, "null plane");
    const size_t bytes = (size_t)H * pitch;
    SVA_HIP(c, c->in_a.ensure(bytes), "staging");
    SVA_HIP(c, c->in_b.ensure(bytes), "staging");
    SVA_HIP(c, c->out_a.ensure(bytes), "staging");
    hipStream_t st = c->stream;
    SVA_HIP(c, hipMemcpyAsync(c->in_a.ptr, disparity, bytes, hipMemcpyHostToDevice, st), "upload");
    SVA_HIP(c, hipMemcpyAsync(c->in_b.ptr, image, bytes, hipMemcpyHostToDevice, st), "upload");
    SVA_HIP(c, hipMemcpyAsync(c->out_a.ptr, shifted, bytes, hipMemcpyHostToDevice, st), "upload");
    SVA_HIP(c, launch_shift_perspective(*c, *in_cam, *out_cam, (uint8_t*)c->in_a.ptr,
                                        (uint8_t*)c->in_b.ptr, W, H, pitch,
                                        (uint8_t*)c->out_a.ptr), "shift launch");
    SVA_HIP(c, hipMemcpyAsync(shifted, c->out_a.ptr, bytes, hipMemcpyDeviceToHost, st), "download");
    SVA_HIP(c, hipStreamSynchronize(st), "sync");
    return SVA_OK;
}

int sva_improve_with_disparity_d(void* ctx, const uint8_t* disparity, const uint8_t* center,
                                 const uint8_t* const* images, const sva_camera* cam_pairs,
                                 int n_pairs, int W, int H, size_t pitch, const uint8_t* mask,
                                 int window_size, int strict, uint8_t* out) {
    Ctx* c = as_ctx(ctx);
    SVA_CHECK_CTX(c);
    int s;
    if ((s = check_planes(c, W, H, pitch)) || (s = check_window(c, window_size))) return s;
    if (n_pairs < 0 || (n_pairs > 0 && (!images || !cam_pairs)))
        return fail(c, SVA_ERR_INVALID_ARG, "bad pair list");
    if (!disparity || !center || !out) return fail(c, SVA_ERR_INVALID_ARG, "null plane");
    for (int i = 0; i < n_pairs; i++)
        if (!images[i]) return fail(c, SVA_ERR_INVALID_ARG, "null pair image");
    return run_improve(c, disparity, center, images, cam_pairs, n_pairs, W, H, pitch, mask,
                       window_size, strict, out, nullptr);
}

int sva_improve_with_disparity(void* ctx, const uint8_t* disparity, const uint8_t* center,
                               const uint8_t* const* images, const sva_camera* cam_pairs,
                               int n_pairs, int W, int H, size_t pitch, const uint8_t* mask,
                               int window_size, int strict, uint8_t* out) {
    Ctx* c = as_ctx(ctx);
    SVA_CHECK_CTX(c);
    int s;
    if ((s = check_planes(c, W, H, pitch)) || (s = check_window(c, window_size))) return s;
    if (n_pairs < 0 || (n_pairs > 0 && (!images || !cam_pairs)))
        return fail(c, SVA_ERR_INVALID_ARG, "bad pair list");
    if (!disparity || !center || !out) return fail(c, SVA_ERR_INVALID_ARG, "null plane");
    for (int i = 0; i < n_pairs; i++)
        if (!images[i]) return fail(c, SVA_ERR_INVALID_ARG, "null pair image");
    const size_t bytes = (size_t)H * pitch;
    SVA_HIP(c, c->in_a.ensure(bytes), "staging");
    SVA_HIP(c, c->in_b.ensure(bytes), "staging");
    SVA_HIP(c, c->in_c.ensure(bytes), "staging");
    SVA_HIP(c, c->out_a.ensure(bytes), "staging");
    if (mask) SVA_HIP(c, c->in_mask.ensure(bytes), "staging");
    hipStream_t st = c->stream;
    SVA_HIP(c, hipMemcpyAsync(c->in_a.ptr, disparity, bytes, hipMemcpyHostToDevice, st), "upload");
    SVA_HIP(c, hipMemcpyAsync(c->in_b.ptr, center, bytes, hipMemcpyHostToDevice, st), "upload");
    if (mask) SVA_HIP(c, hipMemcpyAsync(c->in_mask.ptr, mask, bytes, hipMemcpyHostToDevice, st), "upload");
    SVA_HIP(c, hipMemcpyAsync(c->out_a.ptr, out, bytes, hipMemcpyHostToDevice, st), "upload");
    uint8_t* dimg = (uint8_t*)c->in_c.ptr;
    auto fetch = [&](int i, const uint8_t** img) -> int {
        SVA_HIP(c, hipMemcpyAsync(dimg, images[i], bytes, hipMemcpyHostToDevice, st), "upload");
        *img = dimg;
        return SVA_OK;
    };
    if ((s = run_improve(c, (uint8_t*)c->in_a.ptr, (uint8_t*)c->in_b.ptr, nullptr, cam_pairs,
                         n_pairs, W, H, pitch, mask ? (uint8_t*)c->in_mask.ptr : nullptr,
                         window_size, strict, (uint8_t*)c->out_a.ptr, fetch)))
        return s;
    SVA_HIP(c, hipMemcpyAsync(out, c->out_a.ptr, bytes, hipMemcpyDeviceToHost, st), "download");
    SVA_HIP(c, hipStreamSynchronize(st), "sync");
    return SVA_OK;
}

int sva_shift_perspective2_d(void* ctx, const sva_camera* in_cam, const sva_camera* out_cam,
                             const double* depth, int W, int H, double* shifted) {
    Ctx* c = as_ctx(ctx);
    SVA_CHECK_CTX(c);
    int s;
    if ((s = check_planes(c, W, H, (size_t)W)) || (s = check_camera(c, in_cam)) ||
        (s = check_camera(c, out_cam)))
        return s;
    if (!depth || !shifted) return fail(c, SVA_ERR_INVALID_ARG, "null plane");
    SVA_HIP(c, c->keys.ensure((size_t)W * H * 4), "key workspace");
    SVA_HIP(c, launch_shift_perspective2(*c, *in_cam, *out_cam, depth, W, H,
                                         (unsigned*)c->keys.ptr, shifted), "shift2 launch");
    return SVA_OK;
}

int sva_shift_perspective2(void* ctx, const sva_camera* in_cam, const sva_camera* out_cam,
                           const double* depth, int W, int H, double* shifted) {
    Ctx* c = as_ctx(ctx);
    SVA_CHECK_CTX(c);
    int s;
    if ((s = check_planes(c, W, H, (size_t)W)) || (s = check_camera(c, in_cam)) ||
        (s = check_camera(c, out_cam)))
        return s;
    if (!depth || !shifted) return fail(c, SVA_ERR_INVALID_ARG, "null plane");
    const size_t bytes = (size_t)W * H * 8;
    SVA_HIP(c, c->in_a.ensure(bytes), "staging");
    SVA_HIP(c, c->out_a.ensure(bytes), "staging");
    SVA_HIP(c, c->keys.ensure((size_t)W * H * 4), "key workspace");
    hipStream_t st = c->stream;
    SVA_HIP(c, hipMemcpyAsync(c->in_a.ptr, depth, bytes, hipMemcpyHostToDevice, st), "upload");
    SVA_HIP(c, hipMemcpyAsync(c->out_a.ptr, shifted, bytes, hipMemcpyHostToDevice, st), "upload");
    SVA_HIP(c, launch_shift_perspective2(*c, *in_cam, *out_cam, (double*)c->in_a.ptr, W, H,
                                         (unsigned*)c->keys.ptr, (double*)c->out_a.ptr),
            "shift2 launch");
    SVA_HIP(c, hipMemcpyAsync(shifted, c->out_a.ptr, bytes, hipMemcpyDeviceToHost, st), "download");
    SVA_HIP(c, hipStreamSynchronize(st), "sync");
    return SVA_OK;
}

int sva_points_to_depth_d(void* ctx, const double* points, int64_t n_points,
                          const sva_camera* cam, int W, int H, double* depth) {
    Ctx* c = as_ctx(ctx);
    SVA_CHECK_CTX(c);
    int s;
    if ((s = check_planes(c, W, H, (size_t)W)) || (s = check_camera(c, cam))) return s;
    if (n_points < 0 || n_points > 0xfffffffell || (n_points > 0 && !points) || !depth)
        return fail(c, SVA_ERR_INVALID_ARG, "bad point list");
    SVA_HIP(c, c->keys.ensure((size_t)W * H * 4), "key workspace");
    SVA_HIP(c, launch_points_to_depth(*c, points, n_points, *cam, W, H, (unsigned*)c->keys.ptr,
                                      depth), "points launch");
    return SVA_OK;
}

int sva_points_to_depth(void* ctx, const double* points, int64_t n_points, const sva_camera* cam,
                        int W, int H, double* depth) {
    Ctx* c = as_ctx(ctx);
    SVA_CHECK_CTX(c);
    int s;
    if ((s = check_planes(c, W, H, (size_t)W)) || (s = check_camera(c, cam))) return s;
    if (n_points < 0 || n_points > 0xfffffffell || (n_points > 0 && !points) || !depth)
        return fail(c, SVA_ERR_INVALID_ARG, "bad point list");
    const size_t pbytes = (size_t)n_points * 24, dbytes = (size_t)W * H * 8;
    SVA_HIP(c, c->in_a.ensure(pbytes ? pbytes : 8), "staging");
    SVA_HIP(c, c->out_a.ensure(dbytes), "staging");
    SVA_HIP(c, c->keys.ensure((size_t)W * H * 4), "key workspace");
    hipStream_t st = c->stream;
    if (pbytes)
        SVA_HIP(c, hipMemcpyAsync(c->in_a.ptr, points, pbytes, hipMemcpyHostToDevice, st), "upload");
    SVA_HIP(c, hipMemcpyAsync(c->out_a.ptr, depth, dbytes, hipMemcpyHostToDevice, st), "upload");
    SVA_HIP(c, launch_points_to_depth(*c, (double*)c->in_a.ptr, n_points, *cam, W, H,
                                      (unsigned*)c->keys.ptr, (double*)c->out_a.ptr),
            "points launch");
    SVA_HIP(c, hipMemcpyAsync(depth, c->out_a.ptr, dbytes, hipMemcpyDeviceToHost, st), "download");
    SVA_HIP(c, hipStreamSynchronize(st), "sync");
    return SVA_OK;
}

int sva_depth_to_points_d(void* ctx, const double* depth, int W, int H, const sva_camera* cam,
                          double* points, int64_t* n_points) {
    Ctx* c = as_ctx(ctx);
    SVA_CHECK_CTX(c);
    int s;
    if ((s = check_planes(c, W, H, (size_t)W)) || (s = check_camera(c, cam))) return s;
    if (!depth || !points || !n_points) return fail(c, SVA_ERR_INVALID_ARG, "null argument");
    SVA_HIP(c, c->counts.ensure(d2p_units(W, H) * 4), "count workspace");
    SVA_HIP(c, c->total.ensure(sizeof(long long)), "count workspace");
    SVA_HIP(c, launch_depth_to_points(*c, depth, W, H, *cam, (unsigned*)c->counts.ptr,
                                      (long long*)c->total.ptr, points), "d2p launch");
    long long n = 0;
    SVA_HIP(c, hipMemcpyAsync(&n, c->total.ptr, sizeof(n), hipMemcpyDeviceToHost, c->stream),
            "download");
    SVA_HIP(c, hipStreamSynchronize(c->stream), "sync");
    *n_points = n;
    return SVA_OK;
}

int sva_depth_to_points(void* ctx, const double* depth, int W, int H, const sva_camera* cam,
                        double* points, int64_t* n_points) {
    Ctx* c = as_ctx(ctx);
    SVA_CHECK_CTX(c);
    int s;
    if ((s = check_planes(c, W, H, (size_t)W)) || (s = check_camera(c, cam))) return s;
    if (!depth || !points || !n_points) return fail(c, SVA_ERR_INVALID_ARG, "null argument");
    const size_t np = (size_t)W * H;
    SVA_HIP(c, c->in_a.ensure(np * 8), "staging");
    SVA_HIP(c, c->out_a.ensure(np * 24), "staging");
    SVA_HIP(c, c->counts.ensure(d2p_units(W, H) * 4), "count workspace");
    SVA_HIP(c, c->total.ensure(sizeof(long long)), "count workspace");
    hipStream_t st = c->stream;
    SVA_HIP(c, hipMemcpyAsync(c->in_a.ptr, depth, np * 8, hipMemcpyHostToDevice, st), "upload");
    SVA_HIP(c, launch_depth_to_points(*c, (double*)c->in_a.ptr, W, H, *cam,
                                      (unsigned*)c->counts.ptr, (long long*)c->total.ptr,
                                      (double*)c->out_a.ptr), "d2p launch");
    long long n = 0;
    SVA_HIP(c, hipMemcpyAsync(&n, c->total.ptr, sizeof(n), hipMemcpyDeviceToHost, st), "download");
    SVA_HIP(c, hipStreamSynchronize(st), "sync");
    if (n > 0)
        SVA_HIP(c, hipMemcpyAsync(points, c->out_a.ptr, (size_t)n * 24, hipMemcpyDeviceToHost, st),
                "download");
    SVA_HIP(c, hipStreamSynchronize(st), "sync");
    *n_points = n;
    return SVA_OK;
}

int sva_resize_half_size(int W, int H, int* out_w, int* out_h) {
    if (W < 0 || H < 0 || !out_w || !out_h) return SVA_ERR_INVALID_ARG;
    resize_half_size(W, H, out_w, out_h);
    return SVA_OK;
}

int sva_resize_half_d(void* ctx, const uint8_t* src, int W, int H, size_t pitch, uint8_t* dst,
                      size_t dst_pitch) {
    Ctx* c = as_ctx(ctx);
    SVA_CHECK_CTX(c);
    int s, dw, dh;
    if ((s = check_planes(c, W, H, pitch))) return s;
    resize_half_size(W, H, &dw, &dh);
    if (!src || (!dst && dw > 0 && dh > 0) || dst_pitch < (size_t)dw)
        return fail(c, SVA_ERR_INVALID_ARG, "bad resize argument");
    SVA_HIP(c, launch_resize_half(*c, src, W, H, pitch, dst, dst_pitch), "resize launch");
    return SVA_OK;
}

int sva_resize_half(void* ctx, const uint8_t* src, int W, int H, size_t pitch, uint8_t* dst,
                    size_t dst_pitch) {
    Ctx* c = as_ctx(ctx);
    SVA_CHECK_CTX(c);
    int s, dw, dh;
    if ((s = check_planes(c, W, H, pitch))) return s;
    resize_half_size(W, H, &dw, &dh);
    if (!src || (!dst && dw > 0 && dh > 0) || dst_pitch < (size_t)dw)
        return fail(c, SVA_ERR_INVALID_ARG, "bad resize argument");
    if (dw == 0 || dh == 0) return SVA_OK;
    const size_t sb = (size_t)H * pitch, db = (size_t)dh * dst_pitch;
    SVA_HIP(c, c->in_a.ensure(sb), "staging");
    SVA_HIP(c, c->out_a.ensure(db), "staging");
    hipStream_t st = c->stream;
    SVA_HIP(c, hipMemcpyAsync(c->in_a.ptr, src, sb, hipMemcpyHostToDevice, st), "upload");
    SVA_HIP(c, launch_resize_half(*c, (uint8_t*)c->in_a.ptr, W, H, pitch, (uint8_t*)c->out_a.ptr,
                                  dst_pitch), "resize launch");
    SVA_HIP(c, hipMemcpyAsync(dst, c->out_a.ptr, db, hipMemcpyDeviceToHost, st), "download");
    SVA_HIP(c, hipStreamSynchronize(st), "sync");
    return SVA_OK;
}

namespace {
int check_dims(Ctx* c, int w, int h) {
    if (w <= 0 || h <= 0 || (size_t)w * h > ((size_t)1 << 31))
        return fail(c, SVA_ERR_INVALID_ARG, "matrix dimensions must be positive (< 2^31 elements)");
    return SVA_OK;
}

int host_resize(Ctx* c, const double* src, int sw, int sh, const double* ref, int dw, int dh,
                double scale, double* dst) {
    const size_t sb = (size_t)sw * sh * 8, db = (size_t)dw * dh * 8;
    SVA_HIP(c, c->in_a.ensure(sb), "staging");
    SVA_HIP(c, c->out_a.ensure(db), "staging");
    if (ref) SVA_HIP(c, c->in_b.ensure(db), "staging");
    hipStream_t st = c->stream;
    SVA_HIP(c, hipMemcpyAsync(c->in_a.ptr, src, sb, hipMemcpyHostToDevice, st), "upload");
    if (ref) SVA_HIP(c, hipMemcpyAsync(c->in_b.ptr, ref, db, hipMemcpyHostToDevice, st), "upload");
    SVA_HIP(c, launch_resize_linear(*c, (double*)c->in_a.ptr, sw, sh, (double*)c->out_a.ptr, dw, dh,
                                    ref ? (double*)c->in_b.ptr : nullptr, scale), "resize launch");
    SVA_HIP(c, hipMemcpyAsync(dst, c->out_a.ptr, db, hipMemcpyDeviceToHost, st), "download");
    SVA_HIP(c, hipStreamSynchronize(st), "sync");
    return SVA_OK;
}
}

int sva_resize_linear_f64_d(void* ctx, const double* src, int sw, int sh, double* dst, int dw,
                            int dh) {
    Ctx* c = as_ctx(ctx);
    SVA_CHECK_CTX(c);
    int s;
    if ((s = check_dims(c, sw, sh)) || (s = check_dims(c, dw, dh))) return s;
    if (!src || !dst) return fail(c, SVA_ERR_INVALID_ARG, "null matrix");
    SVA_HIP(c, launch_resize_linear(*c, src, sw, sh, dst, dw, dh, nullptr, 0.0), "resize launch");
    return SVA_OK;
}

int sva_resize_linear_f64(void* ctx, const double* src, int sw, int sh, double* dst, int dw,
                          int dh) {
    Ctx* c = as_ctx(ctx);
    SVA_CHECK_CTX(c);
    int s;
    if ((s = check_dims(c, sw, sh)) || (s = check_dims(c, dw, dh))) return s;
    if (!src || !dst) return fail(c, SVA_ERR_INVALID_ARG, "null matrix");
    return host_resize(c, src, sw, sh, nullptr, dw, dh, 0.0, dst);
}

int sva_ref_error_d(void* ctx, const double* depth, int w, int h, const double* ref, int rw,
                    int rh, double scale, double* error) {
    Ctx* c = as_ctx(ctx);
    SVA_CHECK_CTX(c);
    int s;
    if ((s = check_dims(c, w, h)) || (s = check_dims(c, rw, rh))) return s;
    if (!depth || !ref || !error) return fail(c, SVA_ERR_INVALID_ARG, "null matrix");
    SVA_HIP(c, launch_resize_linear(*c, depth, w, h, error, rw, rh, ref, scale), "resize launch");
    return SVA_OK;
}

int sva_ref_error(void* ctx, const double* depth, int w, int h, const double* ref, int rw, int rh,
                  double scale, double* error) {
    Ctx* c = as_ctx(ctx);
    SVA_CHECK_CTX(c);
    int s;
    if ((s = check_dims(c, w, h)) || (s = check_dims(c, rw, rh))) return s;
    if (!depth || !ref || !error) return fail(c, SVA_ERR_INVALID_ARG, "null matrix");
    return host_resize(c, depth, w, h, ref, rw, rh, scale, error);
}

int sva_masked_mean_d(void* ctx, const double* image, const uint8_t* mask, int w, int h,
                      double* mean) {
    Ctx* c = as_ctx(ctx);
    SVA_CHECK_CTX(c);
    int s;
    if ((s = check_dims(c, w, h))) return s;
    if (!image || !mean) return fail(c, SVA_ERR_INVALID_ARG, "null argument");
    SVA_HIP(c, c->scratch_u16.ensure(masked_mean_workspace()), "reduction workspace");
    double* dmean = (double*)((char*)c->scratch_u16.ptr + masked_mean_workspace() - sizeof(double));
    SVA_HIP(c, launch_masked_mean(*c, image, mask, (size_t)w * h, c->scratch_u16.ptr, dmean),
            "mean launch");
    SVA_HIP(c, hipMemcpyAsync(mean, dmean, sizeof(double), hipMemcpyDeviceToHost, c->stream),
            "download");
    SVA_HIP(c, hipStreamSynchronize(c->stream), "sync");
    return SVA_OK;
}

int sva_masked_mean(void* ctx, const double* image, const uint8_t* mask, int w, int h,
                    double* mean) {
    Ctx* c = as_ctx(ctx);
    SVA_CHECK_CTX(c);
    int s;
    if ((s = check_dims(c, w, h))) return s;
    if (!image || !mean) return fail(c, SVA_ERR_INVALID_ARG, "null argument");
    const size_t n = (size_t)w * h;
    SVA_HIP(c, c->in_a.ensure(n * 8), "staging");
    SVA_HIP(c, c->in_mask.ensure(mask ? n : 1), "staging");
    hipStream_t st = c->stream;
    SVA_HIP(c, hipMemcpyAsync(c->in_a.ptr, image, n * 8, hipMemcpyHostToDevice, st), "upload");
    if (mask) SVA_HIP(c, hipMemcpyAsync(c->in_mask.ptr, mask, n, hipMemcpyHostToDevice, st), "upload");
    return sva_masked_mean_d(ctx, (double*)c->in_a.ptr, mask ? (uint8_t*)c->in_mask.ptr : nullptr, w,
                             h, mean);
}

}
```

### stereovisionarray_amd/csrc/sva_internal.h

```cpp
#pragma once

#include <hip/hip_ext.h>
#include <hip/hip_runtime.h>

#include <cstdint>
#include <cstring>
#include <map>
#include <memory>
#include <string>
#include <vector>

#include "sva.h"
#include "sva_tuning.h"

namespace sva {

struct Status {
    int code = SVA_OK;
    std::string msg;
};

struct KernelTimer {
    bool enabled = false;
    int mode = 0;
    struct Pending {
        std::string name;
        hipEvent_t start, stop;
    };
    std::vector<Pending> pending;
    std::vector<hipEvent_t> pool;
    std::map<std::string, std::pair<double, int64_t>> totals;

    hipEvent_t get_event();
    void begin(hipStream_t s, const char* name, hipEvent_t* start_out);
    void end(hipStream_t s, const char* name, hipEvent_t start);
    hipError_t resolve();
    void release_all();
};

struct DevBuf {
    void* ptr = nullptr;
    size_t bytes = 0;
    unsigned flags = 0;
    hipError_t ensure(size_t n);
    void release();
};

struct Ctx {
    int device = -1;
    hipStream_t own_stream = nullptr;
    hipStream_t stream = nullptr;
    std::string last_error;
    KernelTimer timer;
    DevBuf census_l, census_r, cost, paths, ckpt, scratch_u16, disp_r;
    DevBuf in_a, in_b, in_mask, out_a, out_b, out_c;
    DevBuf in_c, shifted, keys, counts, total;
    DevBuf ref_keys;
    size_t ref_keys_clean = 0;
    const void* ref_keys_alloc = nullptr;
    int cu_count = 256;
    std::shared_ptr<void> batch_lane;
    std::vector<hipStream_t> side;
    std::vector<hipEvent_t> side_done;
    hipEvent_t fork = nullptr;
    DevBuf census_side;
    int dbg_plane_split = 0;
    int dbg_fail_cost_at = 0;
    int last_diag_route = 0;
    int64_t dbg_pair_min_pixels = -1;
    int placement_trials = 0;
    int64_t placement_ns = 0, placement_worst_ns = 0;
    const void* placement_paths = nullptr;
};

inline bool timer_wants(const KernelTimer& t, const char* name) {
    if (!t.enabled) return false;
    if (t.mode == SVA_TIMING_ALL) return true;
    if (std::strcmp(name, "sgm_paths") == 0) return true;
    return t.mode == SVA_TIMING_AGG && std::strcmp(name, "wta_hv") == 0;
}

struct ScopedKernelTimer {
    Ctx& c;
    const char* name;
    hipEvent_t start = nullptr;
    ScopedKernelTimer(Ctx& ctx, const char* n) : c(ctx), name(n) {
        if (timer_wants(c.timer, name)) c.timer.begin(c.stream, name, &start);
    }
    ~ScopedKernelTimer() {
        if (c.timer.enabled && start) c.timer.end(c.stream, name, start);
    }
};

struct DispatchTimer {
    Ctx& c;
    const char* name;
    hipEvent_t start = nullptr, stop = nullptr;
    bool used = false;
    DispatchTimer(Ctx& ctx, const char* n) : c(ctx), name(n) {
        if (timer_wants(c.timer, name)) {
            start = c.timer.get_event();
            stop = start ? c.timer.get_event() : nullptr;
            if (!stop && start) { c.timer.pool.push_back(start); start = nullptr; }
        }
    }
    ~DispatchTimer() {
        if (start && stop && used)
            c.timer.pending.push_back(KernelTimer::Pending{name, start, stop});
        else if (start && stop) {
            c.timer.pool.push_back(start);
            c.timer.pool.push_back(stop);
        }
    }
};


hipError_t launch_census(Ctx& c, const uint8_t* img, int W, int H, size_t pitch, uint64_t* out);
hipError_t launch_census_pair(Ctx& c, const uint8_t* left, const uint8_t* right, int W, int H,
                              size_t pitch, uint64_t* out_l, uint64_t* out_r);
bool census_cost_supported(int D);
hipError_t launch_census_cost(Ctx& c, const uint8_t* left, const uint8_t* right, int W, int H,
                              size_t pitch, int D, int dmin, int dir, uint8_t* C, int dreal = 0);
bool census_cost2_supported(int D, int sx, int sy);
hipError_t launch_census_cost2(Ctx& c, const uint8_t* left, const uint8_t* right, int W, int H,
                               size_t pitch, int D, int dmin, int sx, int sy, uint8_t* C,
                               int dreal = 0);
hipError_t launch_cost(Ctx& c, const uint64_t* cl, const uint64_t* cr, int W, int H, int D,
                       int dmin, int dir, uint8_t* C, int dreal = 0);
hipError_t launch_paths(Ctx& c, const uint8_t* C, int W, int H, int D, int P1, int P2,
                        uint8_t* L8, uint8_t* CK = nullptr, uint8_t* CKV = nullptr,
                        int npair = 1, bool pair = false, int dreal = 0);
bool diag_pair_enabled(int D);
inline bool diag_pair_ok(int D, int P2) { return diag_pair_enabled(D) && 2 * P2 <= 255; }
struct TileGeom {
    int seg_log2;
    int ntx, nty;
    int nsx;
    size_t hck_bytes;
    size_t vck_bytes;
    size_t dck_bytes;
    int nvol;
};
TileGeom tile_geom(int W, int H, int D);
constexpr bool diag_ckpt_down(int dpl) {
    return (tune::kStripRoute != 0 && dpl <= 8) || tune::kTileDiagDown != 0;
}
constexpr bool diag_ckpt_up(int dpl) {
    return (tune::kStripRoute != 0 && dpl <= 8) || tune::kTileDiagUp != 0;
}
bool wta_strip_supported(int D);
hipError_t launch_wta_strip(Ctx& c, const uint8_t* C, const uint8_t* CK, const uint8_t* CKV, int W,
                            int H, int D, int P1, int P2, int dmin, uint16_t* disp, float* sub,
                            int dreal = 0, int npair = 1);
bool paths_supported(int D);
inline int padded_D(int D) {
    return D <= 0 ? 0 : D <= 64 ? 64 : D <= 128 ? 128 : D <= 192 ? 192 : D <= 256 ? 256 : 0;
}
bool wta_hv_supported(int D);
hipError_t launch_wta_hv(Ctx& c, const uint8_t* C, const uint8_t* L4, const uint8_t* CK,
                         const uint8_t* CKV, int W, int H, int D, int P1, int P2, int dmin,
                         uint16_t* disp, float* sub, int dreal = 0, int npair = 1,
                         bool pair = false);
hipError_t launch_sum(Ctx& c, const uint8_t* L8, int W, int H, int D, uint16_t* S);
hipError_t launch_wta_from_sum(Ctx& c, const uint16_t* S, int W, int H, int D, int dmin,
                               uint16_t* disp, float* sub);
hipError_t launch_lr_check(Ctx& c, uint16_t* disp_l, const uint16_t* disp_r, float* sub, int W, int H,
                           int sx, int sy, int max_diff, uint16_t invalid);
hipError_t launch_cost2(Ctx& c, const uint64_t* cl, const uint64_t* cr, int W, int H, int D,
                        int dmin, int sx, int sy, uint8_t* C, int dreal = 0);
hipError_t launch_fuse_depth(Ctx& c, const uint16_t* disps, int n_maps, size_t np,
                             const double* num, double pixel_size, uint16_t invalid,
                             double* depth, uint8_t* n_valid);
hipError_t launch_ref_endpoints(Ctx& c, int W, int H, const sva_camera& cref,
                                const sva_camera& coth, int k, double t_near, double t_far,
                                int32_t* ends, uint8_t* valid);
hipError_t launch_ref_match(Ctx& c, const uint8_t* ref, const uint8_t* other, int W, int H,
                            size_t pitch, const uint8_t* mask, const int32_t* ends,
                            const uint8_t* valid_in, int k, uint8_t* disp_u8,
                            uint16_t* disp_u16, uint8_t* valid_out);
hipError_t launch_shift_perspective(Ctx& c, const sva_camera& in, const sva_camera& out,
                                    const uint8_t* disp, const uint8_t* img, int W, int H,
                                    size_t pitch, uint8_t* shifted, bool zero_fill = false);
hipError_t launch_refine(Ctx& c, const uint8_t* disp, const uint8_t* center,
                         const uint8_t* shifted, const uint8_t* mask, int W, int H, size_t pitch,
                         int k, const sva_camera& c0, const sva_camera& c1, uint8_t* out,
                         int* fault);
hipError_t launch_shift_perspective2(Ctx& c, const sva_camera& in, const sva_camera& out,
                                     const double* depth, int W, int H, unsigned* keys,
                                     double* shifted);
hipError_t launch_points_to_depth(Ctx& c, const double* pts, long long n, const sva_camera& cam,
                                  int W, int H, unsigned* keys, double* depth);
size_t d2p_units(int W, int H);
hipError_t launch_depth_to_points(Ctx& c, const double* depth, int W, int H,
                                  const sva_camera& cam, unsigned* counts, long long* total,
                                  double* pts);
void resize_half_size(int W, int H, int* dw, int* dh);
hipError_t launch_resize_linear(Ctx& c, const double* src, int sw, int sh, double* dst, int dw,
                                int dh, const double* ref, double scale);
size_t masked_mean_workspace();
hipError_t launch_masked_mean(Ctx& c, const double* img, const uint8_t* mask, size_t n,
                              void* ws, double* mean);
hipError_t launch_resize_half(Ctx& c, const uint8_t* src, int W, int H, size_t pitch,
                              uint8_t* dst, size_t dpitch);
hipError_t launch_disp_to_depth(Ctx& c, const uint8_t* disp, int n, double cam_distance,
                                double f, double pixel_size, double* depth);

}
```

### stereovisionarray_amd/csrc/sva_tuning.h

```cpp
#pragma once

#include <cstddef>

namespace sva {
namespace tune {

constexpr int kStepAddU32 = 1;
constexpr int kSplitPairs = 1;
constexpr int kStepMadP2 = 0;
constexpr int kPfH4 = 40, kPfV4 = 24;
constexpr int kPfH8 = 32, kPfV8 = 12;
constexpr int kPfH12 = 24, kPfV12 = 8;
constexpr int kPfH16 = 12, kPfV16 = 8;
constexpr int kCLoadAux = 0;
constexpr int kCkptStoreAux = 0;
constexpr int kStaticCkptHitsMaxDpl = 4;

constexpr int kStateMinTree = 1;

constexpr int kTileDiagDown = 0;
constexpr int kTileDiagUp = 0;
constexpr int kDiagPair4 = 0, kDiagPair8 = 1, kDiagPair12 = 0, kDiagPair16 = 0;
constexpr long long kDiagPairMinPixels = 1450000;
constexpr int kWtahvPfVolPair = 4;
constexpr int kStripRoute = 0;
constexpr int kStripTileW = 16;
constexpr int kStripCols = 128;
constexpr int kStripMinWaves = 3;
constexpr int kWtahvTileLog2 = 3;
constexpr int kWtahvTileLog2Wide = 3;
constexpr int kWtahvPfVol = 3;
constexpr int kWtahvPfVol4 = 4;
constexpr int kWtahvPfVol16 = 2;
constexpr int kWtahvInterleaveV = 0;
constexpr int kWtahvEarlyLoads = 1;
constexpr int kWtahvRowCFirst = 1;
constexpr int kWtahvKeepU16 = 3;
constexpr int kWtahvKeepU16Wide = 3;
constexpr int kWtahvPinRowMin = 1;
constexpr int kWtahvPinWta = 1;
constexpr int kWtahvSubLds = 1;
constexpr int kWtahvKeyPerm = 1;
constexpr int kWtahvSubDeferred = 1;
constexpr int kWtahvUnpackOnce = 0;
constexpr int kWtahvMinWaves = 1;
constexpr int kWtahvVSwizzle = 0;

constexpr int kBatchMaxPairs = 8;
constexpr int kBatchCostStreams = 3;
constexpr int kBatchSubFrames = 4;
constexpr size_t kBatchMaxBytes = (size_t)24 << 30;

constexpr int kPlacementTrials = 6;
constexpr size_t kPlacementMinBytes = (size_t)4 << 30;

constexpr int kCensusRows = 16;
constexpr int kCensusCostMinD = 64;
constexpr int kCensusCostRows = 8;
constexpr int kCensusCostRowsSmall = 4;
constexpr int kCensusCostMinGroups = 1536;
constexpr int kCensusCostPx4 = 64, kCensusCostPx8 = 64, kCensusCostPx12 = 64, kCensusCostPx16 = 128;
constexpr int kCostStoreNT = 1;
constexpr int kCensusCostSlotOrder = 1;
constexpr int kCensusCostWS = 0;
constexpr int kCensusCost2Lines = 8;

constexpr int kPlaneOuKB = 24;
constexpr int kPlaneWords = 1024;
constexpr int kPlaneMinBlocks = 3;
constexpr int kPlaneStageMajor = 2;
constexpr int kPlaneNoHoistDiv = 0;
constexpr int kPlanePoLds = 1;
constexpr int kPlaneSplitMin = 3;
constexpr int kPlaneSplitMax = 6;
constexpr int kPlaneSplitRounds = 4;
constexpr int kPlaneSplitInner = 2;
constexpr int kPlaneWalkRange = 1;

}
}
```

### stereovisionarray_amd/csrc/wta_hv.hip

```cpp
#include "sgm_common.h"
#include "wta_common.h"
#include "sva_tuning.h"

namespace sva {
namespace {

using namespace sgm;

constexpr int TB = 256;
constexpr int TW = 16;

struct WtaHvGeom {
    int W, H, D, P1, P2, dmin;
    int ntx, nty;
    int nsx;
    int dreal;
    unsigned vol;
    unsigned hck;
    unsigned vck;
    int tiles;
};

template <int DPL, bool PAIR> constexpr int pf_vol() {
    return PAIR ? tune::kWtahvPfVolPair : DPL >= 16 ? tune::kWtahvPfVol16 : DPL <= 4 ? tune::kWtahvPfVol4 : tune::kWtahvPfVol;
}

template <int DPL, int TYL, bool PAD, bool PAIR>
__global__ __launch_bounds__(TB, tune::kWtahvMinWaves) void wta_hv_kernel(const uint8_t* __restrict__ C,
                                                    const uint8_t* __restrict__ L4,
                                                    const uint8_t* __restrict__ CK,
                                                    const uint8_t* __restrict__ CKV, WtaHvGeom g,
                                                    uint16_t* __restrict__ disp,
                                                    float* __restrict__ sub) {
    constexpr int NW = DPL / 4, NP = DPL / 2;
    constexpr int TY = 1 << TYL;
    constexpr int kPfVol = pf_vol<DPL, PAIR>();
    constexpr int KEEPM = DPL <= 8 ? tune::kWtahvKeepU16 : tune::kWtahvKeepU16Wide;
    constexpr bool KEEP16 = (KEEPM & 1) != 0, KEEP16H = (KEEPM & 2) != 0;
    constexpr bool PIN = tune::kWtahvPinRowMin != 0;
    constexpr bool UNPACK1 = ((tune::kWtahvUnpackOnce >> (DPL / 4 - 1)) & 1) != 0;

    constexpr int SPR = TW / TY;
    static_assert(TY <= TW && TW % TY == 0, "tile rows must divide 16");
    const unsigned f = blockIdx.x / (unsigned)g.tiles;
    const unsigned tb = blockIdx.x - f * (unsigned)g.tiles;
    const int tx = (int)(tb % (unsigned)g.ntx);
    const int ty = (int)(tb / (unsigned)g.ntx);
    constexpr bool DOWN = diag_ckpt_down(DPL), UP = diag_ckpt_up(DPL);
    constexpr int ND = (DOWN ? 2 : 0) + (UP ? 2 : 0);
    constexpr int NV = PAIR ? 2 : 4 - ND;
    static_assert(!PAIR || ND == 0, "the pair route replaces all four diagonal volumes");
    C += (size_t)f * g.vol;
    L4 += (size_t)f * NV * g.vol;
    CK += (size_t)f * 2 * g.hck;
    CKV += (size_t)f * (2 + ND) * g.vck;
    disp += (size_t)f * (size_t)g.W * (size_t)g.H;
    if (sub) sub += (size_t)f * (size_t)g.W * (size_t)g.H;
    const int slot = (int)(threadIdx.x >> 4);
    const int k = (int)(threadIdx.x & 15);
    const int W = g.W, H = g.H;
    const unsigned uD = (unsigned)g.D, uW = (unsigned)W;
    const unsigned P1 = (unsigned)g.P1, P2 = (unsigned)g.P2;
    const int x0 = tx * TW, y0 = ty * TY;
    const int nx = W - x0 < TW ? W - x0 : TW;
    const int ny = H - y0 < TY ? H - y0 : TY;
    const unsigned lane_d = (unsigned)(k * DPL);
    const rsrc_t rC = make_rsrc(C, g.vol);
    unsigned padm[NP];
#pragma unroll
    for (int j = 0; j < NP; j++) {
        const int dl = k * DPL + pair_d<DPL>(j, 0), dh = k * DPL + pair_d<DPL>(j, 1);
        padm[j] = PAD ? ((dl >= g.dreal ? 0x0000ffffu : 0u) | (dh >= g.dreal ? 0xffff0000u : 0u))
                      : 0u;
    }

    __shared__ unsigned vsum[TY * TW * 16 * NP];
    constexpr bool VSW = NP == 8 && tune::kWtahvVSwizzle != 0;
    auto vsw_of = [](int kk) -> int { return VSW ? (((kk >> 2) ^ (kk >> 3)) & 1) * 4 : 0; };
    const int vb0 = k * NP + vsw_of(k), vb1 = k * NP + (4 ^ vsw_of(k));
    auto vw = [&](int p) -> int { return (p < 4 ? vb0 : vb1) + (p & 3); };

    const bool vcol = slot < nx;
    const int hr = slot / SPR, hseg = slot % SPR;
    const int hx = x0 + hseg * TY;
    const int nh = W - hx < TY ? W - hx : TY;
    const bool hrow = hr < ny && nh > 0;
    const unsigned xv = (unsigned)(x0 + slot), yh = (unsigned)(y0 + hr);

    Words<NW> cv[TY], ch[TY];
#pragma unroll
    for (int r = 0; r < TY; r++)
        cv[r] = bload<NW>(rC, ((unsigned)(y0 + r) * uW + xv) * uD + lane_d);
    auto load_row = [&]() {
#pragma unroll
        for (int j = 0; j < TY; j++)
            ch[j] = bload<NW>(rC, (yh * uW + (unsigned)(hx + j)) * uD + lane_d);
    };
    if constexpr (tune::kWtahvRowCFirst != 0) load_row();

    auto zero_state = [](unsigned (&A)[NP], unsigned& m) {
#pragma unroll
        for (int j = 0; j < NP; j++) A[j] = 0u;
        m = 0u;
    };
    unsigned Aa[NP], Ab[NP], ma, mb;
    Edges ea, eb;
    if (vcol) {
        if (ty > 0)
            load_state<DPL, PAD, PIN>(make_rsrc(CKV, g.vck), ((unsigned)(ty - 1) * uW + xv) * uD + lane_d,
                                 Aa, ma, padm);
        else
            zero_state(Aa, ma);
        if (y0 + TY < H)
            load_state<DPL, PAD, PIN>(make_rsrc(CKV + g.vck, g.vck),
                                 ((unsigned)(ty + 1) * uW + xv) * uD + lane_d, Ab, mb, padm);
        else
            zero_state(Ab, mb);
        constexpr int NK = KEEP16 ? NP : NW;
        auto keep = [&](unsigned (&dst)[NK], const unsigned (&A)[NP], const unsigned (&ow)[NW]) {
#pragma unroll
            for (int q = 0; q < NK; q++) dst[q] = KEEP16 ? A[q] : ow[q];
        };
        auto put_v = [&](int r, const unsigned (&ld)[NK], const unsigned (&Au)[NP],
                         const unsigned (&lu)[NW], const unsigned (&cw)[NW]) {
            unsigned V[NP];
            if constexpr (KEEP16) {
#pragma unroll
                for (int p = 0; p < NP; p++) V[p] = ld[p] + Au[p];
            } else {
                words_to_pairs<DPL>(ld, V);
                unpack_add<NW>(lu, V);
            }
            if constexpr (PAIR) {
                unsigned c4[NP];
                words_to_pairs<DPL>(cw, c4);
#pragma unroll
                for (int p = 0; p < NP; p++) V[p] += c4[p] << 2;
            }
            unsigned* dst = &vsum[(r * TW + slot) * 16 * NP];
#pragma unroll
            for (int p = 0; p < NP; p++) dst[vw(p)] = V[p];
        };
        unsigned LD[TY][NK];
        if constexpr (tune::kWtahvInterleaveV != 0) {
            unsigned LU[TY][NK];
            for_seq<TY>([&](auto I) {
                constexpr int i = decltype(I)::value, ru = TY - 1 - i;
                unsigned ow[NW];
                if (i < ny) { sgm_step<DPL, PIN>(cv[i].w, Aa, ma, ow, P1, P2, ea); keep(LD[i], Aa, ow); }
                if (ru < ny) { sgm_step<DPL, PIN>(cv[ru].w, Ab, mb, ow, P1, P2, eb); keep(LU[ru], Ab, ow); }
            });
            for_seq<TY>([&](auto R) {
                constexpr int r = decltype(R)::value;
                if (r < ny) {
                    if constexpr (KEEP16) {
                        const unsigned none[NW] = {};
                        put_v(r, LD[r], LU[r], none, cv[r].w);
                    } else {
                        unsigned V[NP] = {};
                        put_v(r, LD[r], V, LU[r], cv[r].w);
                    }
                }
            });
        } else {
            unsigned cvp[UNPACK1 ? TY : 1][NP];
            for_seq<TY>([&](auto I) {
                constexpr int i = decltype(I)::value;
                unsigned ow[NW];
                if (i < ny) {
                    if constexpr (UNPACK1) {
                        words_to_pairs<DPL>(cv[i].w, cvp[i]);
                        sgm_step_c<DPL, PIN>(cvp[i], Aa, ma, ow, P1, P2, ea);
                    } else {
                        sgm_step<DPL, PIN>(cv[i].w, Aa, ma, ow, P1, P2, ea);
                    }
                    keep(LD[i], Aa, ow);
                }
            });
            for_seq<TY>([&](auto Q) {
                constexpr int r = TY - 1 - decltype(Q)::value;
                if (r < ny) {
                    unsigned lu[NW];
                    if constexpr (UNPACK1) sgm_step_c<DPL, PIN>(cvp[UNPACK1 ? r : 0], Ab, mb, lu, P1, P2, eb);
                    else sgm_step<DPL, PIN>(cv[r].w, Ab, mb, lu, P1, P2, eb);
                    put_v(r, LD[r], Ab, lu, cv[r].w);
                }
            });
        }
    }
    if constexpr (ND > 0) {
        __syncthreads();
        constexpr int NL = TW + TY - 1;
        constexpr int NRUN = (ND * NL + 15) / 16;
        const rsrc_t rCKD = make_rsrc(CKV + 2 * (size_t)g.vck, (unsigned)ND * g.vck);
        struct Run {
            int c, rx, yck;
            unsigned plane;
            bool up, ok;
        };
        auto run_of = [&](int i) __attribute__((always_inline)) -> Run {
            Run u;
            const int q = slot + 16 * i;
            const int dd = q / NL, li = q - dd * NL;
            u.ok = q < ND * NL;
            u.up = !DOWN || dd >= 2;
            const int e = u.up && DOWN ? dd - 2 : dd;
            u.rx = u.up ? (e ? 1 : -1) : (e ? -1 : 1);
            u.c = u.rx > 0 ? x0 - TY + li : x0 + 1 + li;
            u.plane = (unsigned)dd;
            u.yck = u.up ? (y0 + TY < H ? ty + 1 : -1) : ty - 1;
            return u;
        };
        auto issue_d = [&](int i, Words<NW>& ck, Words<NW> (&cd)[TY]) __attribute__((always_inline)) {
            const Run u = run_of(i);
            const bool ckin = u.yck >= 0 && (unsigned)u.c < (unsigned)W;
            ck = bload<NW>(rCKD, ckin ? u.plane * g.vck + ((unsigned)u.yck * uW + (unsigned)u.c) * uD +
                                            lane_d
                                      : 0u);
#pragma unroll
            for (int s = 0; s < TY; s++) {
                const int x = u.c + u.rx * (s + 1);
                const int y = u.up ? y0 + TY - 1 - s : y0 + s;
                cd[s] = bload<NW>(rC, (unsigned)x < (unsigned)W && y < H
                                          ? ((unsigned)y * uW + (unsigned)x) * uD + lane_d
                                          : 0u);
            }
        };
        auto run_d = [&](int i, const Words<NW>& ck, const Words<NW> (&cd)[TY]) __attribute__((always_inline)) {
            const Run u = run_of(i);
            if (!u.ok) return;
            unsigned A[NP], m;
            if (u.yck >= 0 && (unsigned)u.c < (unsigned)W) state_from_words<DPL, PAD, PIN>(ck, A, m, padm);
            else zero_state(A, m);
            for_seq<TY>([&](auto R) {
                constexpr int s = decltype(R)::value;
                const int x = u.c + u.rx * (s + 1);
                const int r = u.up ? TY - 1 - s : s;
                if ((unsigned)x < (unsigned)W && r < ny) {
                    unsigned ow[NW];
                    sgm_step<DPL, PIN>(cd[s].w, A, m, ow, P1, P2, eb);
                    if (x >= x0 && x < x0 + nx) {
                        unsigned* dst = &vsum[(r * TW + (x - x0)) * 16 * NP];
#pragma unroll
                        for (int p = 0; p < NP; p++) atomicAdd(&dst[vw(p)], A[p]);
                    }
                } else {
                    zero_state(A, m);
                }
            });
        };
        if constexpr (DPL <= 8) {
            Words<NW> ck[2], cd[2][TY];
            issue_d(0, ck[0], cd[0]);
            for_seq<NRUN>([&](auto I) {
                constexpr int i = decltype(I)::value;
                if constexpr (i + 1 < NRUN) issue_d(i + 1, ck[(i + 1) & 1], cd[(i + 1) & 1]);
                run_d(i, ck[i & 1], cd[i & 1]);
            });
        } else {
            Words<NW> ck, cd[TY];
            for_seq<NRUN>([&](auto I) {
                constexpr int i = decltype(I)::value;
                issue_d(i, ck, cd);
                run_d(i, ck, cd);
            });
        }
    }
    if constexpr (tune::kWtahvRowCFirst == 0) load_row();
    const int hs = hx >> TYL;
    const unsigned ckrow = yh * (unsigned)g.nsx;
    Words<NW> ckw[2];
    constexpr int NVA = NV > 0 ? NV : 1;
    rsrc_t rV[NVA];
#pragma unroll
    for (int r = 0; r < NV; r++) rV[r] = make_rsrc(L4 + (size_t)r * g.vol, g.vol);
    Words<NW> rv[kPfVol][NVA];
    auto issue = [&](int s, int j) {
        const unsigned off = (yh * uW + (unsigned)(hx + j)) * uD + lane_d;
#pragma unroll
        for (int r = 0; r < NV; r++) rv[s][r] = bload<NW, 2>(rV[r], off);
    };
    auto issue_first = [&]() {
        ckw[0] = bload<NW>(make_rsrc(CK, g.hck), (ckrow + (unsigned)(hs - 1)) * uD + lane_d);
        ckw[1] = bload<NW>(make_rsrc(CK + g.hck, g.hck), (ckrow + (unsigned)(hs + 1)) * uD + lane_d);
#pragma unroll
        for (int q = 0; q < kPfVol && q < TY; q++) issue(q, TY - 1 - q);
    };
    if constexpr (tune::kWtahvEarlyLoads != 0) {
        if (hrow) issue_first();
    }
    __syncthreads();

    if (!hrow) return;
    if constexpr (tune::kWtahvEarlyLoads == 0) issue_first();
    if (hs > 0) state_from_words<DPL, PAD, PIN>(ckw[0], Aa, ma, padm);
    else zero_state(Aa, ma);
    constexpr int NKH = KEEP16H ? NP : NW;
    unsigned LF[TY][NKH];
    unsigned chp[UNPACK1 ? TY : 1][NP];
    for_seq<TY>([&](auto I) {
        constexpr int i = decltype(I)::value;
        unsigned ow[NW];
        if (i < nh) {
            if constexpr (UNPACK1) {
                words_to_pairs<DPL>(ch[i].w, chp[i]);
                sgm_step_c<DPL, PIN>(chp[i], Aa, ma, ow, P1, P2, ea);
            } else {
                sgm_step<DPL, PIN>(ch[i].w, Aa, ma, ow, P1, P2, ea);
            }
#pragma unroll
            for (int q = 0; q < NKH; q++) LF[i][q] = KEEP16H ? Aa[q] : ow[q];
        }
    });
    if (hx + TY < W) state_from_words<DPL, PAD, PIN>(ckw[1], Aa, ma, padm);
    else zero_state(Aa, ma);
    unsigned dres = 0u, sm = 0u, s0 = 0u;
    const bool want_sub = sub != nullptr;
    unsigned dpair[NP];
#pragma unroll
    for (int j = 0; j < NP; j++)
        dpair[j] = (lane_d + (unsigned)pair_d<DPL>(j, 0)) | ((lane_d + (unsigned)pair_d<DPL>(j, 1)) << 16);
    constexpr bool DEFER = tune::kWtahvSubLds != 0 && tune::kWtahvSubDeferred != 0;
    unsigned* const vrow = &vsum[(hr * TW + hseg * TY) * 16 * NP];
    for_seq<TY>([&](auto Q) {
        constexpr int q = decltype(Q)::value, j = TY - 1 - q, s = q % kPfVol;
        if (j < nh) {
            unsigned ow[NW];
            if constexpr (UNPACK1) sgm_step_c<DPL, PIN>(chp[UNPACK1 ? j : 0], Aa, ma, ow, P1, P2, ea);
            else sgm_step<DPL, PIN>(ch[j].w, Aa, ma, ow, P1, P2, ea);
            unsigned* const vpix = vrow + j * 16 * NP;
            unsigned S[NP];
#pragma unroll
            for (int p = 0; p < NP; p++) S[p] = vpix[vw(p)] + Aa[p];
            if constexpr (KEEP16H) {
#pragma unroll
                for (int p = 0; p < NP; p++) S[p] += LF[j][p];
            } else {
                unpack_add<NW>(LF[j], S);
            }
#pragma unroll
            for (int r = 0; r < NV; r++) unpack_add<NW>(rv[s][r].w, S);
            if constexpr (PAD) {
#pragma unroll
                for (int p = 0; p < NP; p++) S[p] |= padm[p];
            }
            unsigned spm, sb;
            if constexpr (tune::kWtahvSubLds != 0) {
                const unsigned best = tune::kWtahvKeyPerm
                                          ? wta_pick_key_perm<DPL, PIN && tune::kWtahvPinWta>(S, dpair)
                                          : wta_pick_key<DPL, PIN && tune::kWtahvPinWta, tune::kSplitPairs != 0>(S, k);
                const int ds = (int)(best & 0xffffu);
                if (want_sub) {
#pragma unroll
                    for (int p = 0; p < NP; p++) vpix[vw(p)] = S[p];
                    if constexpr (!DEFER) {
                        __builtin_amdgcn_fence(__ATOMIC_RELEASE, "wavefront");
                        __builtin_amdgcn_wave_barrier();
                        __builtin_amdgcn_fence(__ATOMIC_ACQUIRE, "wavefront");
                    }
                }
                if constexpr (DEFER) {
                    dres = k == j ? (unsigned)ds : dres;
                    s0 = k == j ? best >> 16 : s0;
                } else if (k == j) {
                    dres = (unsigned)ds;
                    s0 = best >> 16;
                    if (want_sub) {
                        const uint16_t* s16 = reinterpret_cast<const uint16_t*>(vpix);
                        const int dm = ds > 0 ? ds - 1 : 0, dp = ds + 1 < 16 * DPL ? ds + 1 : ds;
                        auto at = [&](int d) {
                            const int kk = d / DPL, pp = pair_of<DPL>(d % DPL), hh = half_of<DPL>(d % DPL);
                            return (unsigned)s16[2 * (kk * NP + (pp ^ vsw_of(kk))) + hh];
                        };
                        sm = at(dm) | (at(dp) << 16);
                    }
                }
            } else {
                const int ds = wta_pick_raw<DPL, PIN && tune::kWtahvPinWta, tune::kSplitPairs != 0>(S, k, want_sub, &spm, &sb);
                if (k == j) {
                    dres = (unsigned)ds;
                    sm = spm;
                    s0 = sb;
                }
            }
        }
        if constexpr (q + kPfVol < TY) {
            __builtin_amdgcn_sched_barrier(0);
            issue(s, TY - 1 - (q + kPfVol));
            __builtin_amdgcn_sched_barrier(0);
        }
    });
    if constexpr (DEFER) {
        if (want_sub) {
            __builtin_amdgcn_fence(__ATOMIC_RELEASE, "wavefront");
            __builtin_amdgcn_wave_barrier();
            __builtin_amdgcn_fence(__ATOMIC_ACQUIRE, "wavefront");
            if (k < nh) {
                const uint16_t* s16 = reinterpret_cast<const uint16_t*>(vrow + k * 16 * NP);
                const int ds = (int)dres;
                const int dm = ds > 0 ? ds - 1 : 0, dp = ds + 1 < 16 * DPL ? ds + 1 : ds;
                auto at = [&](int d) {
                    const int kk = d / DPL, pp = pair_of<DPL>(d % DPL), hh = half_of<DPL>(d % DPL);
                    return (unsigned)s16[2 * (kk * NP + (pp ^ vsw_of(kk))) + hh];
                };
                sm = at(dm) | (at(dp) << 16);
            }
        }
    }
    if (k < nh) {
        const size_t at = (size_t)yh * (size_t)W + (size_t)(hx + k);
        disp[at] = (uint16_t)(g.dmin + (int)dres);
        if (want_sub) sub[at] = subpixel(g.dmin, (int)dres, g.dreal, sm & 0xffffu, s0, sm >> 16);
    }
}

template <int DPL, int TYL, bool PAIR>
void wtahv_launch(bool pad, dim3 grid, hipStream_t s, hipEvent_t start, hipEvent_t stop,
                  const uint8_t* C, const uint8_t* L4, const uint8_t* CK, const uint8_t* CKV,
                  const WtaHvGeom& g, uint16_t* disp, float* sub) {
    if (pad)
        hipExtLaunchKernelGGL((wta_hv_kernel<DPL, TYL, true, PAIR>), grid, dim3(TB), 0, s, start,
                              stop, 0, C, L4, CK, CKV, g, disp, sub);
    else
        hipExtLaunchKernelGGL((wta_hv_kernel<DPL, TYL, false, PAIR>), grid, dim3(TB), 0, s, start,
                              stop, 0, C, L4, CK, CKV, g, disp, sub);
}

}

bool wta_hv_supported(int D) { return D == 64 || D == 128 || D == 192 || D == 256; }

hipError_t launch_wta_hv(Ctx& c, const uint8_t* C, const uint8_t* L4, const uint8_t* CK,
                         const uint8_t* CKV, int W, int H, int D, int P1, int P2, int dmin,
                         uint16_t* disp, float* sub, int dreal, int npair, bool pair) {
    if (tune::kStripRoute != 0 && wta_strip_supported(D))
        return launch_wta_strip(c, C, CK, CKV, W, H, D, P1, P2, dmin, disp, sub, dreal, npair);
    DispatchTimer t(c, "wta_hv");
    if (!wta_hv_supported(D)) return hipErrorInvalidValue;
    const TileGeom tg = tile_geom(W, H, D);
    WtaHvGeom g;
    g.W = W; g.H = H; g.D = D; g.P1 = P1; g.P2 = P2; g.dmin = dmin;
    g.dreal = dreal > 0 && dreal < D ? dreal : D;
    g.ntx = tg.ntx;
    g.nty = tg.nty;
    g.nsx = tg.nsx;
    const size_t vol = (size_t)W * H * D;
    if (vol >= (size_t)1 << 32) return hipErrorInvalidValue;
    g.vol = (unsigned)vol;
    g.hck = (unsigned)(tg.hck_bytes / 2);
    g.vck = (unsigned)(tg.vck_bytes / 2);
    const bool pad = g.dreal < D;
    if (npair < 1) return hipErrorInvalidValue;
    g.tiles = g.ntx * g.nty;
    const dim3 grid((unsigned)(g.tiles * npair));
#define SVA_WTAHV(DPL_, TYL_)                                                                 \
    wtahv_launch<DPL_, TYL_, false>(pad, grid, c.stream, t.start, t.stop, C, L4, CK, CKV, g,  \
                                    disp, sub);                                               \
    t.used = true
#define SVA_WTAHV_P(DPL_, TYL_, EN_)                                                          \
    if (pair) {                                                                               \
        wtahv_launch<DPL_, TYL_, (EN_) != 0>(pad, grid, c.stream, t.start, t.stop, C, L4, CK, \
                                             CKV, g, disp, sub);                              \
        t.used = true;                                                                        \
    } else {                                                                                  \
        SVA_WTAHV(DPL_, TYL_);                                                                \
    }
    constexpr int TYL = tune::kWtahvTileLog2, TYLW = tune::kWtahvTileLog2Wide;
    if (tg.seg_log2 != (D <= 128 ? TYL : TYLW)) return hipErrorInvalidValue;
    if (pair && (npair != 1 || !diag_pair_ok(D, P2) || tg.nvol != 4)) return hipErrorInvalidValue;
    switch (D) {
        case 64: SVA_WTAHV_P(4, TYL, tune::kDiagPair4); break;
        case 128: SVA_WTAHV_P(8, TYL, tune::kDiagPair8); break;
        case 192: SVA_WTAHV_P(12, TYLW, tune::kDiagPair12); break;
        case 256: SVA_WTAHV_P(16, TYLW, tune::kDiagPair16); break;
        default: return hipErrorInvalidValue;
    }
#undef SVA_WTAHV_P
#undef SVA_WTAHV
    return hipGetLastError();
}

}
```

Baseline: 331,600.

## Store per-step path minima in paths pass and reuse them in WTA recompute

The horizontal and vertical checkpointed path passes now record each step's previous row minimum as a byte into a side buffer, one 8-byte word per 8-pixel segment. The WTA kernel loads these and skips the cross-lane min reduction in each recomputed SGM step. This targets the costly lane/row min reduction on the recompute critical path. In exchange it adds extra stores and workspace in the paths kernel and relies on minima fitting in a byte at the stored offset, which is a correctness risk for large costs.

```diff
diff --git a/stereovisionarray_amd/csrc/sgm_common.h b/stereovisionarray_amd/csrc/sgm_common.h
--- a/stereovisionarray_amd/csrc/sgm_common.h
+++ b/stereovisionarray_amd/csrc/sgm_common.h
@@ -195,7 +195,7 @@
     unsigned X = INF2, Y = INF2;
 };
 
-template <int DPL, bool PIN = false>
+template <int DPL, bool PIN = false, bool GIVEN_M = false>
 __device__ __forceinline__ void sgm_step_c(const unsigned (&c)[DPL / 2], unsigned (&A)[DPL / 2],
                                            unsigned& m, unsigned (&ow)[DPL / 4], unsigned P1,
                                            unsigned P2, Edges& e) {
@@ -244,7 +244,7 @@
 #pragma unroll
     for (int j = 0; j < NP; j++) A[j] = add3(min3_u16x2(tp[j], A[j], mP2), c[j], K);
     pairs_to_words<DPL>(A, ow);
-    m = row_min_u32<PIN>(lane_min_u16<NP>(A));
+    if constexpr (!GIVEN_M) m = row_min_u32<PIN>(lane_min_u16<NP>(A));
 }
 
 template <int DPL>
@@ -255,13 +255,27 @@
     sgm_step_c<DPL>(c, A, m, ow, P1, P2, e);
 }
 
-template <int DPL, bool PIN = false>
+template <int DPL, bool PIN = false, bool GIVEN_M = false>
 __device__ __forceinline__ void sgm_step(const unsigned (&cw)[DPL / 4], unsigned (&A)[DPL / 2],
                                          unsigned& m, unsigned (&ow)[DPL / 4], unsigned P1,
                                          unsigned P2, Edges& e) {
     unsigned c[DPL / 2];
     words_to_pairs<DPL>(cw, c);
-    sgm_step_c<DPL, PIN>(c, A, m, ow, P1, P2, e);
+    sgm_step_c<DPL, PIN, GIVEN_M>(c, A, m, ow, P1, P2, e);
+}
+
+constexpr int kMinimaSeg = 8;
+
+struct MinWindow {
+    unsigned lo = 0u, hi = 0u;
+    __device__ __forceinline__ void push(unsigned m) {
+        lo = __builtin_amdgcn_alignbit(hi, lo, 8);
+        hi = __builtin_amdgcn_alignbit(m, hi, 8);
+    }
+};
+
+__device__ __forceinline__ unsigned minima_byte(const Words<2>& w, int i) {
+    return (w.w[i >> 2] >> ((i & 3) * 8)) & 0xffu;
 }
 
 __device__ __forceinline__ void dir_of(int r, int& rx, int& ry) {
@@ -278,10 +292,12 @@
 }
 
 
-template <int DPL, bool DIAG, int PF, int CKPT = 0, int SL = 0>
+template <int DPL, bool DIAG, int PF, int CKPT = 0, int SL = 0, bool MN = false>
 __device__ __forceinline__ void path_line(rsrc_t rC, rsrc_t rL, const PathGeom& g, int rx, int ry,
-                                          int line, int k, rsrc_t rCK) {
+                                          int line, int k, rsrc_t rCK, rsrc_t rMN) {
     constexpr int NW = DPL / 4, NP = DPL / 2;
+    static_assert(!MN || ((CKPT == 1 || CKPT == 2) && (1 << SL) == kMinimaSeg),
+                  "path minima: horizontal and vertical checkpoint lines, 8-pixel segments");
     const int W = g.W, H = g.H, D = g.D;
     const unsigned P1 = (unsigned)g.P1, P2 = (unsigned)g.P2;
     const int steps = ry == 0 ? W : H;
@@ -302,6 +318,7 @@
         lead = CKPT == 1 ? (rx > 0 ? 0 : (SEG - W % SEG) % SEG) : (ry > 0 ? 0 : (SEG - H % SEG) % SEG);
         pc.off -= (unsigned)lead * stride;
     }
+    static_assert(!(MN && STATIC_HITS), "path minima are stored by the runtime segment test");
     const int nsteps = steps + lead;
     int twc = 0, twp = 0, Tc = 0, Tp = 0;
     if constexpr (DIAG) {
@@ -317,6 +334,17 @@
     for (int j = 0; j < NP; j++) A[j] = 0u;
     unsigned m = 0u;
     Edges edges;
+    MinWindow mw;
+    const bool fwd = CKPT == 1 ? rx > 0 : ry > 0;
+    const int mn_end = fwd ? steps : -1, ck_none = fwd ? steps : 0, mn_fmask = fwd ? kMinimaSeg - 1 : 0;
+    auto store_minima = [&](unsigned seg_off, int e) {
+        unsigned long long w = ((unsigned long long)mw.hi << 32) | mw.lo;
+        w >>= (unsigned)(-e & mn_fmask) * 8u;
+        if (k == 0) {
+            const unsigned ww[2] = {(unsigned)w, (unsigned)(w >> 32)};
+            bstore<2, tune::kCkptStoreAux>(rMN, seg_off * (unsigned)kMinimaSeg, ww);
+        }
+    };
 
     Words<NW> ring[PF];
 #pragma unroll
@@ -345,6 +373,7 @@
 #pragma unroll
         for (int w = 0; w < NW; w++) cw[w] = ring[p].w[w];
         unsigned ow[NW];
+        if constexpr (MN) mw.push(m);
         sgm_step<DPL>(cw, A, m, ow, P1, P2, edges);
         if constexpr (CKPT == 1 && STATIC_HITS) {
             constexpr int SEG = 1 << SL;
@@ -361,6 +390,16 @@
                 if (ry > 0 ? y + 1 < H : y > 0)
                     bstore<NW, tune::kCkptStoreAux>(rCK, ((unsigned)((y >> SL) * W + x0) * (unsigned)D +
                                              (unsigned)(k * DPL)), ow);
+            }
+        } else if constexpr (MN) {
+            constexpr int SEG = 1 << SL;
+            const int e = fwd ? ts + 1 : steps - 1 - ts;
+            if (__builtin_expect((int)((e & (SEG - 1)) == 0) | (int)(e == mn_end), 0)) {
+                const int sg = (fwd ? e - 1 : e) >> SL;
+                const unsigned so = CKPT == 1 ? (unsigned)(y0 * g.ns + sg) : (unsigned)(sg * W + x0);
+                if (e != ck_none)
+                    bstore<NW, tune::kCkptStoreAux>(rCK, so * (unsigned)D + (unsigned)(k * DPL), ow);
+                store_minima(so, e);
             }
         } else if constexpr (CKPT == 1) {
             const int x = rx > 0 ? ts : W - 1 - ts;
@@ -442,7 +481,7 @@
     for (int j = 0; j < 2 * NW; j++) S[j] += a[j];
 }
 
-template <int DPL, bool PAD, bool PIN = false>
+template <int DPL, bool PAD, bool PIN = false, bool GIVEN_M = false>
 __device__ __forceinline__ void state_from_words(const Words<DPL / 4>& w, unsigned (&A)[DPL / 2],
                                                  unsigned& m, const unsigned (&padm)[DPL / 2]) {
     constexpr int NP = DPL / 2;
@@ -451,7 +490,8 @@
 #pragma unroll
         for (int j = 0; j < NP; j++) A[j] |= padm[j] & 0x00ff00ffu;
     }
-    if constexpr (tune::kStateMinTree) {
+    if constexpr (GIVEN_M) {
+    } else if constexpr (tune::kStateMinTree) {
         m = row_min_u32<PIN>(lane_min_u16<NP>(A));
     } else {
         unsigned mm = 0xffffffffu;
@@ -464,10 +504,10 @@
         m = row_min_u32<PIN>(mm);
     }
 }
-template <int DPL, bool PAD, bool PIN = false>
+template <int DPL, bool PAD, bool PIN = false, bool GIVEN_M = false>
 __device__ __forceinline__ void load_state(rsrc_t r, unsigned off, unsigned (&A)[DPL / 2],
                                            unsigned& m, const unsigned (&padm)[DPL / 2]) {
-    state_from_words<DPL, PAD, PIN>(bload<DPL / 4>(r, off), A, m, padm);
+    state_from_words<DPL, PAD, PIN, GIVEN_M>(bload<DPL / 4>(r, off), A, m, padm);
 }
 
 template <int DPL, int PF, int SL>
diff --git a/stereovisionarray_amd/csrc/sgm_paths.hip b/stereovisionarray_amd/csrc/sgm_paths.hip
--- a/stereovisionarray_amd/csrc/sgm_paths.hip
+++ b/stereovisionarray_amd/csrc/sgm_paths.hip
@@ -10,11 +10,12 @@
 constexpr int LINES_PER_BLOCK = PATH_BLOCK / 16;
 constexpr int PAIR_LINES = LINES_PER_BLOCK / 2;
 
-template <int DPL, bool PAIR>
+template <int DPL, bool PAIR, bool MN>
 __global__ __launch_bounds__(PATH_BLOCK) void sgm_paths_kernel(const uint8_t* __restrict__ C,
                                                                uint8_t* __restrict__ L8,
                                                                uint8_t* __restrict__ CK,
                                                                uint8_t* __restrict__ CKV,
+                                                               uint8_t* __restrict__ MNP,
                                                                PathGeom g) {
     int b = blockIdx.x, r, lb, f;
     if constexpr (PAIR) {
@@ -70,6 +71,10 @@
     const rsrc_t rC = make_rsrc(C, g.vol);
     constexpr int SL = DPL <= 8 ? tune::kWtahvTileLog2 : tune::kWtahvTileLog2Wide;
     constexpr bool DOWN = diag_ckpt_down(DPL), UP = diag_ckpt_up(DPL);
+    const size_t mnh = (size_t)g.H * g.ns * kMinimaSeg, mnv = (size_t)g.nsy * g.W * kMinimaSeg;
+    const rsrc_t rMN = !MN || r >= 4 ? rC
+                       : r >= 2 ? make_rsrc(MNP + 2 * mnh + (size_t)(r - 2) * mnv, mnv)
+                                : make_rsrc(MNP + (size_t)r * mnh, mnh);
     if constexpr (PAIR) {
         if (r >= 4) {
             const int pr = r == 4 ? 0 : 1;
@@ -78,49 +83,62 @@
             pair_line<DPL, pf_v<DPL>(), SL>(rC, rE, g, rx, line, role, k, rCK);
         } else if (r >= 2) {
             const rsrc_t rCK = make_rsrc(CKV + (size_t)(r - 2) * g.ckvvol, g.ckvvol);
-            path_line<DPL, false, pf_v<DPL>(), 2, SL>(rC, rC, g, rx, ry, line, k, rCK);
+            path_line<DPL, false, pf_v<DPL>(), 2, SL, MN>(rC, rC, g, rx, ry, line, k, rCK, rMN);
         } else {
             const rsrc_t rCK = make_rsrc(CK + (size_t)r * g.ckvol, g.ckvol);
-            path_line<DPL, false, pf_h<DPL>(), 1, SL>(rC, rC, g, rx, ry, line, k, rCK);
+            path_line<DPL, false, pf_h<DPL>(), 1, SL, MN>(rC, rC, g, rx, ry, line, k, rCK, rMN);
         }
     } else if (r >= 4 && g.ckpt && (ry > 0 ? DOWN : UP)) {
         const int plane = ry > 0 ? 2 + (r == 4 ? 0 : 1) : 2 + (DOWN ? 2 : 0) + (r == 5 ? 0 : 1);
         const rsrc_t rCK = make_rsrc(CKV + (size_t)plane * g.ckvvol, g.ckvvol);
-        path_line<DPL, true, pf_v<DPL>(), 3, SL>(rC, rC, g, rx, ry, line, k, rCK);
+        path_line<DPL, true, pf_v<DPL>(), 3, SL>(rC, rC, g, rx, ry, line, k, rCK, rCK);
     } else if (r >= 4) {
         const int slot = !g.ckpt ? r
                        : DOWN ? (r == 5 ? 0 : 1)
                        : UP ? (r == 4 ? 0 : 1)
                        : r - 4;
         const rsrc_t rL = make_rsrc(L8 + (size_t)slot * g.vol, g.vol);
-        path_line<DPL, true, pf_v<DPL>()>(rC, rL, g, rx, ry, line, k, rL);
+        path_line<DPL, true, pf_v<DPL>()>(rC, rL, g, rx, ry, line, k, rL, rL);
     } else if (r >= 2 && g.ckpt) {
         const rsrc_t rCK = make_rsrc(CKV + (size_t)(r - 2) * g.ckvvol, g.ckvvol);
-        path_line<DPL, false, pf_v<DPL>(), 2, SL>(rC, rC, g, rx, ry, line, k, rCK);
+        path_line<DPL, false, pf_v<DPL>(), 2, SL, MN>(rC, rC, g, rx, ry, line, k, rCK, rMN);
     } else if (r >= 2) {
         const rsrc_t rL = make_rsrc(L8 + (size_t)r * g.vol, g.vol);
-        path_line<DPL, false, pf_v<DPL>()>(rC, rL, g, rx, ry, line, k, rL);
+        path_line<DPL, false, pf_v<DPL>()>(rC, rL, g, rx, ry, line, k, rL, rL);
     } else if (g.ckpt) {
         const rsrc_t rCK = make_rsrc(CK + (size_t)r * g.ckvol, g.ckvol);
-        path_line<DPL, false, pf_h<DPL>(), 1, SL>(rC, rC, g, rx, ry, line, k, rCK);
+        path_line<DPL, false, pf_h<DPL>(), 1, SL, MN>(rC, rC, g, rx, ry, line, k, rCK, rMN);
     } else {
         const rsrc_t rL = make_rsrc(L8 + (size_t)r * g.vol, g.vol);
-        path_line<DPL, false, pf_h<DPL>()>(rC, rL, g, rx, ry, line, k, rL);
-    }
-}
-
-template <int DPL, bool EN>
-void paths_launch(bool pair, dim3 grid, hipStream_t s, hipEvent_t start, hipEvent_t stop,
-                  const uint8_t* C, uint8_t* L8, uint8_t* CK, uint8_t* CKV, const PathGeom& g) {
+        path_line<DPL, false, pf_h<DPL>()>(rC, rL, g, rx, ry, line, k, rL, rL);
+    }
+}
+
+template <int DPL, bool EN, bool MN>
+void paths_launch_mn(bool pair, dim3 grid, hipStream_t s, hipEvent_t start, hipEvent_t stop,
+                     const uint8_t* C, uint8_t* L8, uint8_t* CK, uint8_t* CKV, uint8_t* MNP,
+                     const PathGeom& g) {
     if constexpr (EN) {
         if (pair) {
-            hipExtLaunchKernelGGL((sgm_paths_kernel<DPL, true>), grid, dim3(PATH_BLOCK), 0, s, start,
-                                  stop, 0, C, L8, CK, CKV, g);
+            hipExtLaunchKernelGGL((sgm_paths_kernel<DPL, true, MN>), grid, dim3(PATH_BLOCK), 0, s,
+                                  start, stop, 0, C, L8, CK, CKV, MNP, g);
             return;
         }
     }
-    hipExtLaunchKernelGGL((sgm_paths_kernel<DPL, false>), grid, dim3(PATH_BLOCK), 0, s, start, stop,
-                          0, C, L8, CK, CKV, g);
+    hipExtLaunchKernelGGL((sgm_paths_kernel<DPL, false, MN>), grid, dim3(PATH_BLOCK), 0, s, start,
+                          stop, 0, C, L8, CK, CKV, MNP, g);
+}
+template <int DPL, bool EN, bool MNEN>
+void paths_launch(bool pair, dim3 grid, hipStream_t s, hipEvent_t start, hipEvent_t stop,
+                  const uint8_t* C, uint8_t* L8, uint8_t* CK, uint8_t* CKV, uint8_t* MNP,
+                  const PathGeom& g) {
+    if constexpr (MNEN) {
+        if (MNP) {
+            paths_launch_mn<DPL, EN, true>(pair, grid, s, start, stop, C, L8, CK, CKV, MNP, g);
+            return;
+        }
+    }
+    paths_launch_mn<DPL, EN, false>(pair, grid, s, start, stop, C, L8, CK, CKV, nullptr, g);
 }
 
 }
@@ -140,7 +158,14 @@
     const int ndp = (diag_ckpt_down(dpl) ? 2 : 0) + (diag_ckpt_up(dpl) ? 2 : 0);
     t.dck_bytes = (size_t)ndp / 2 * t.vck_bytes;
     t.nvol = 4 - ndp;
+    t.hmn_bytes = 2 * (size_t)H * t.nsx * sgm::kMinimaSeg;
+    t.vmn_bytes = 2 * (size_t)t.nty * W * sgm::kMinimaSeg;
     return t;
+}
+
+bool path_minima_enabled(int D) {
+    return (D == 64 && tune::kPathMinima4) || (D == 128 && tune::kPathMinima8) ||
+           (D == 192 && tune::kPathMinima12) || (D == 256 && tune::kPathMinima16);
 }
 
 bool diag_pair_enabled(int D) {
@@ -149,7 +174,8 @@
 }
 
 hipError_t launch_paths(Ctx& c, const uint8_t* C, int W, int H, int D, int P1, int P2,
-                        uint8_t* L8, uint8_t* CK, uint8_t* CKV, int npair, bool pair, int dreal) {
+                        uint8_t* L8, uint8_t* CK, uint8_t* CKV, int npair, bool pair, int dreal,
+                        uint8_t* MN) {
     DispatchTimer t(c, "sgm_paths");
     PathGeom g;
     g.W = W; g.H = H; g.D = D; g.P1 = P1; g.P2 = P2;
@@ -174,14 +200,16 @@
                  tile_geom(W, H, D).nvol != 4))
         return hipErrorInvalidValue;
     g.pair = pair ? 1 : 0;
+    if (MN && (!CK || npair != 1 || !path_minima_enabled(D) || (1 << tg.seg_log2) != sgm::kMinimaSeg))
+        return hipErrorInvalidValue;
     g.dreal = dreal > 0 && dreal < D ? dreal : D;
     dim3 grid((unsigned)((2 * g.blk_h + 6 * g.blk_w) * npair));
     t.used = true;
     switch (D) {
-        case 64: paths_launch<4, tune::kDiagPair4 != 0>(pair, grid, c.stream, t.start, t.stop, C, L8, CK, CKV, g); break;
-        case 128: paths_launch<8, tune::kDiagPair8 != 0>(pair, grid, c.stream, t.start, t.stop, C, L8, CK, CKV, g); break;
-        case 192: paths_launch<12, tune::kDiagPair12 != 0>(pair, grid, c.stream, t.start, t.stop, C, L8, CK, CKV, g); break;
-        case 256: paths_launch<16, tune::kDiagPair16 != 0>(pair, grid, c.stream, t.start, t.stop, C, L8, CK, CKV, g); break;
+        case 64: paths_launch<4, tune::kDiagPair4 != 0, tune::kPathMinima4 != 0>(pair, grid, c.stream, t.start, t.stop, C, L8, CK, CKV, MN, g); break;
+        case 128: paths_launch<8, tune::kDiagPair8 != 0, tune::kPathMinima8 != 0>(pair, grid, c.stream, t.start, t.stop, C, L8, CK, CKV, MN, g); break;
+        case 192: paths_launch<12, tune::kDiagPair12 != 0, tune::kPathMinima12 != 0>(pair, grid, c.stream, t.start, t.stop, C, L8, CK, CKV, MN, g); break;
+        case 256: paths_launch<16, tune::kDiagPair16 != 0, tune::kPathMinima16 != 0>(pair, grid, c.stream, t.start, t.stop, C, L8, CK, CKV, MN, g); break;
         default: t.used = false; return hipErrorInvalidValue;
     }
     return hipGetLastError();
diff --git a/stereovisionarray_amd/csrc/sva_api.cpp b/stereovisionarray_amd/csrc/sva_api.cpp
--- a/stereovisionarray_amd/csrc/sva_api.cpp
+++ b/stereovisionarray_amd/csrc/sva_api.cpp
@@ -155,6 +155,12 @@
 }
 
 size_t pair_ckpt_bytes(const TileGeom& tg) { return tg.hck_bytes + tg.vck_bytes + tg.vck_bytes; }
+size_t frame_ckpt_bytes(const TileGeom& tg, bool pair) {
+    return pair ? pair_ckpt_bytes(tg) : tg.hck_bytes + tg.vck_bytes + tg.dck_bytes;
+}
+size_t frame_minima_bytes(const TileGeom& tg, int Dp) {
+    return tg.nvol == 4 && path_minima_enabled(Dp) ? tg.hmn_bytes + tg.vmn_bytes : 0;
+}
 
 int paths_wta(Ctx* c, const uint8_t* C, int W, int H, const sva_sgm_params* p, int Dp,
               uint16_t* disp, float* sub) {
@@ -165,14 +171,16 @@
                                                         : tune::kDiagPairMinPixels;
     const bool pair = tg.nvol == 4 && diag_pair_ok(Dp, p->P2) && (long long)W * H >= minpx;
     SVA_HIP(c, c->paths.ensure(nv * (pair ? 2 : tg.nvol)), "path workspace");
-    SVA_HIP(c, c->ckpt.ensure(pair ? pair_ckpt_bytes(tg) : tg.hck_bytes + tg.vck_bytes + tg.dck_bytes),
-            "checkpoint workspace");
+    const size_t ckb = frame_ckpt_bytes(tg, pair), mnb = frame_minima_bytes(tg, Dp);
+    SVA_HIP(c, c->ckpt.ensure(ckb + mnb), "checkpoint workspace");
     uint8_t* L4 = (uint8_t*)c->paths.ptr;
     uint8_t* CK = (uint8_t*)c->ckpt.ptr;
     uint8_t* CKV = CK + tg.hck_bytes;
-    SVA_HIP(c, launch_paths(*c, C, W, H, Dp, p->P1, p->P2, L4, CK, CKV, 1, pair, p->D), "paths launch");
+    uint8_t* MN = mnb ? CK + ckb : nullptr;
+    SVA_HIP(c, launch_paths(*c, C, W, H, Dp, p->P1, p->P2, L4, CK, CKV, 1, pair, p->D, MN),
+            "paths launch");
     SVA_HIP(c, launch_wta_hv(*c, C, L4, CK, CKV, W, H, Dp, p->P1, p->P2, p->dmin, disp, sub, p->D, 1,
-                             pair),
+                             pair, MN),
             "wta launch");
     c->last_diag_route = pair ? 1 : 0;
     return SVA_OK;
@@ -563,10 +571,11 @@
     float best = 0.f;
     for (int r = 0; r < 4 && e == hipSuccess; r++) {
         e = hipEventRecord(a, c->stream);
+        const bool pair = tg.nvol == 4 && diag_pair_ok(D, 120) &&
+                          (long long)W * H >= tune::kDiagPairMinPixels;
         if (e == hipSuccess)
-            e = launch_paths(*c, C, W, H, D, 10, 120, L4, CK, CK + tg.hck_bytes, 1,
-                             tg.nvol == 4 && diag_pair_ok(D, 120) &&
-                                 (long long)W * H >= tune::kDiagPairMinPixels);
+            e = launch_paths(*c, C, W, H, D, 10, 120, L4, CK, CK + tg.hck_bytes, 1, pair, 0,
+                             frame_minima_bytes(tg, D) ? CK + frame_ckpt_bytes(tg, pair) : nullptr);
         if (e == hipSuccess) e = hipEventRecord(b, c->stream);
         if (e == hipSuccess) e = hipEventSynchronize(b);
         float ms = 0.f;
@@ -653,9 +662,8 @@
     SVA_HIP(c, c->census_r.ensure(np * 8), "reserve");
     SVA_HIP(c, c->cost.ensure(nv), "reserve");
     const TileGeom tg = tile_geom(W, H, D);
-    const size_t ckb = tg.nvol == 4 && diag_pair_enabled(D)
-                           ? pair_ckpt_bytes(tg)
-                           : tg.hck_bytes + tg.vck_bytes + tg.dck_bytes;
+    const size_t ckb = frame_ckpt_bytes(tg, tg.nvol == 4 && diag_pair_enabled(D)) +
+                       frame_minima_bytes(tg, D);
     SVA_HIP(c, c->paths.ensure(nv * tg.nvol), "reserve");
     SVA_HIP(c, c->ckpt.ensure(ckb), "reserve");
     const int trials = c->placement_trials > 0 ? c->placement_trials : tune::kPlacementTrials;
diff --git a/stereovisionarray_amd/csrc/sva_internal.h b/stereovisionarray_amd/csrc/sva_internal.h
--- a/stereovisionarray_amd/csrc/sva_internal.h
+++ b/stereovisionarray_amd/csrc/sva_internal.h
@@ -129,7 +129,8 @@
                        int dmin, int dir, uint8_t* C, int dreal = 0);
 hipError_t launch_paths(Ctx& c, const uint8_t* C, int W, int H, int D, int P1, int P2,
                         uint8_t* L8, uint8_t* CK = nullptr, uint8_t* CKV = nullptr,
-                        int npair = 1, bool pair = false, int dreal = 0);
+                        int npair = 1, bool pair = false, int dreal = 0, uint8_t* MN = nullptr);
+bool path_minima_enabled(int D);
 bool diag_pair_enabled(int D);
 inline bool diag_pair_ok(int D, int P2) { return diag_pair_enabled(D) && 2 * P2 <= 255; }
 struct TileGeom {
@@ -140,6 +141,8 @@
     size_t vck_bytes;
     size_t dck_bytes;
     int nvol;
+    size_t hmn_bytes;
+    size_t vmn_bytes;
 };
 TileGeom tile_geom(int W, int H, int D);
 constexpr bool diag_ckpt_down(int dpl) {
@@ -160,7 +163,7 @@
 hipError_t launch_wta_hv(Ctx& c, const uint8_t* C, const uint8_t* L4, const uint8_t* CK,
                          const uint8_t* CKV, int W, int H, int D, int P1, int P2, int dmin,
                          uint16_t* disp, float* sub, int dreal = 0, int npair = 1,
-                         bool pair = false);
+                         bool pair = false, const uint8_t* MN = nullptr);
 hipError_t launch_sum(Ctx& c, const uint8_t* L8, int W, int H, int D, uint16_t* S);
 hipError_t launch_wta_from_sum(Ctx& c, const uint16_t* S, int W, int H, int D, int dmin,
                                uint16_t* disp, float* sub);
diff --git a/stereovisionarray_amd/csrc/sva_tuning.h b/stereovisionarray_amd/csrc/sva_tuning.h
--- a/stereovisionarray_amd/csrc/sva_tuning.h
+++ b/stereovisionarray_amd/csrc/sva_tuning.h
@@ -22,6 +22,7 @@
 constexpr int kTileDiagUp = 0;
 constexpr int kDiagPair4 = 0, kDiagPair8 = 1, kDiagPair12 = 0, kDiagPair16 = 0;
 constexpr long long kDiagPairMinPixels = 1450000;
+constexpr int kPathMinima4 = 0, kPathMinima8 = 1, kPathMinima12 = 0, kPathMinima16 = 0;
 constexpr int kWtahvPfVolPair = 4;
 constexpr int kStripRoute = 0;
 constexpr int kStripTileW = 16;
diff --git a/stereovisionarray_amd/csrc/wta_hv.hip b/stereovisionarray_amd/csrc/wta_hv.hip
--- a/stereovisionarray_amd/csrc/wta_hv.hip
+++ b/stereovisionarray_amd/csrc/wta_hv.hip
@@ -25,11 +25,12 @@
     return PAIR ? tune::kWtahvPfVolPair : DPL >= 16 ? tune::kWtahvPfVol16 : DPL <= 4 ? tune::kWtahvPfVol4 : tune::kWtahvPfVol;
 }
 
-template <int DPL, int TYL, bool PAD, bool PAIR>
+template <int DPL, int TYL, bool PAD, bool PAIR, bool MN>
 __global__ __launch_bounds__(TB, tune::kWtahvMinWaves) void wta_hv_kernel(const uint8_t* __restrict__ C,
                                                     const uint8_t* __restrict__ L4,
                                                     const uint8_t* __restrict__ CK,
-                                                    const uint8_t* __restrict__ CKV, WtaHvGeom g,
+                                                    const uint8_t* __restrict__ CKV,
+                                                    const uint8_t* __restrict__ MNP, WtaHvGeom g,
                                                     uint16_t* __restrict__ disp,
                                                     float* __restrict__ sub) {
     constexpr int NW = DPL / 4, NP = DPL / 2;
@@ -50,6 +51,7 @@
     constexpr int ND = (DOWN ? 2 : 0) + (UP ? 2 : 0);
     constexpr int NV = PAIR ? 2 : 4 - ND;
     static_assert(!PAIR || ND == 0, "the pair route replaces all four diagonal volumes");
+    static_assert(!MN || (TY == kMinimaSeg && ND == 0), "path minima: 8-pixel segments, no phase D");
     C += (size_t)f * g.vol;
     L4 += (size_t)f * NV * g.vol;
     CK += (size_t)f * 2 * g.hck;
@@ -97,6 +99,22 @@
             ch[j] = bload<NW>(rC, (yh * uW + (unsigned)(hx + j)) * uD + lane_d);
     };
     if constexpr (tune::kWtahvRowCFirst != 0) load_row();
+    Words<2> mv[2] = {}, mh[2] = {};
+    if constexpr (MN) {
+        const unsigned hmn = (unsigned)H * (unsigned)g.nsx * (unsigned)kMinimaSeg;
+        const unsigned vmn = (unsigned)g.nty * uW * (unsigned)kMinimaSeg;
+        const unsigned vo = ((unsigned)ty * uW + xv) * (unsigned)kMinimaSeg;
+        const unsigned ho = ((unsigned)(y0 + (slot / SPR)) * (unsigned)g.nsx +
+                             (unsigned)((x0 + (slot % SPR) * TY) >> TYL)) * (unsigned)kMinimaSeg;
+#pragma unroll
+        for (int d = 0; d < 2; d++) {
+            mv[d] = bload<2>(make_rsrc(MNP + 2 * (size_t)hmn + (size_t)d * vmn, vmn), vo);
+            mh[d] = bload<2>(make_rsrc(MNP + (size_t)d * hmn, hmn), ho);
+        }
+    }
+    auto given_m = [](unsigned& m, const Words<2>& w, int i) {
+        if constexpr (MN) m = minima_byte(w, i);
+    };
 
     auto zero_state = [](unsigned (&A)[NP], unsigned& m) {
 #pragma unroll
@@ -107,12 +125,12 @@
     Edges ea, eb;
     if (vcol) {
         if (ty > 0)
-            load_state<DPL, PAD, PIN>(make_rsrc(CKV, g.vck), ((unsigned)(ty - 1) * uW + xv) * uD + lane_d,
+            load_state<DPL, PAD, PIN, MN>(make_rsrc(CKV, g.vck), ((unsigned)(ty - 1) * uW + xv) * uD + lane_d,
                                  Aa, ma, padm);
         else
             zero_state(Aa, ma);
         if (y0 + TY < H)
-            load_state<DPL, PAD, PIN>(make_rsrc(CKV + g.vck, g.vck),
+            load_state<DPL, PAD, PIN, MN>(make_rsrc(CKV + g.vck, g.vck),
                                  ((unsigned)(ty + 1) * uW + xv) * uD + lane_d, Ab, mb, padm);
         else
             zero_state(Ab, mb);
@@ -147,8 +165,16 @@
             for_seq<TY>([&](auto I) {
                 constexpr int i = decltype(I)::value, ru = TY - 1 - i;
                 unsigned ow[NW];
-                if (i < ny) { sgm_step<DPL, PIN>(cv[i].w, Aa, ma, ow, P1, P2, ea); keep(LD[i], Aa, ow); }
-                if (ru < ny) { sgm_step<DPL, PIN>(cv[ru].w, Ab, mb, ow, P1, P2, eb); keep(LU[ru], Ab, ow); }
+                if (i < ny) {
+                    given_m(ma, mv[0], i);
+                    sgm_step<DPL, PIN, MN>(cv[i].w, Aa, ma, ow, P1, P2, ea);
+                    keep(LD[i], Aa, ow);
+                }
+                if (ru < ny) {
+                    given_m(mb, mv[1], i);
+                    sgm_step<DPL, PIN, MN>(cv[ru].w, Ab, mb, ow, P1, P2, eb);
+                    keep(LU[ru], Ab, ow);
+                }
             });
             for_seq<TY>([&](auto R) {
                 constexpr int r = decltype(R)::value;
@@ -168,11 +194,12 @@
                 constexpr int i = decltype(I)::value;
                 unsigned ow[NW];
                 if (i < ny) {
+                    given_m(ma, mv[0], i);
                     if constexpr (UNPACK1) {
                         words_to_pairs<DPL>(cv[i].w, cvp[i]);
-                        sgm_step_c<DPL, PIN>(cvp[i], Aa, ma, ow, P1, P2, ea);
+                        sgm_step_c<DPL, PIN, MN>(cvp[i], Aa, ma, ow, P1, P2, ea);
                     } else {
-                        sgm_step<DPL, PIN>(cv[i].w, Aa, ma, ow, P1, P2, ea);
+                        sgm_step<DPL, PIN, MN>(cv[i].w, Aa, ma, ow, P1, P2, ea);
                     }
                     keep(LD[i], Aa, ow);
                 }
@@ -181,8 +208,9 @@
                 constexpr int r = TY - 1 - decltype(Q)::value;
                 if (r < ny) {
                     unsigned lu[NW];
-                    if constexpr (UNPACK1) sgm_step_c<DPL, PIN>(cvp[UNPACK1 ? r : 0], Ab, mb, lu, P1, P2, eb);
-                    else sgm_step<DPL, PIN>(cv[r].w, Ab, mb, lu, P1, P2, eb);
+                    given_m(mb, mv[1], TY - 1 - r);
+                    if constexpr (UNPACK1) sgm_step_c<DPL, PIN, MN>(cvp[UNPACK1 ? r : 0], Ab, mb, lu, P1, P2, eb);
+                    else sgm_step<DPL, PIN, MN>(cv[r].w, Ab, mb, lu, P1, P2, eb);
                     put_v(r, LD[r], Ab, lu, cv[r].w);
                 }
             });
@@ -293,7 +321,7 @@
 
     if (!hrow) return;
     if constexpr (tune::kWtahvEarlyLoads == 0) issue_first();
-    if (hs > 0) state_from_words<DPL, PAD, PIN>(ckw[0], Aa, ma, padm);
+    if (hs > 0) state_from_words<DPL, PAD, PIN, MN>(ckw[0], Aa, ma, padm);
     else zero_state(Aa, ma);
     constexpr int NKH = KEEP16H ? NP : NW;
     unsigned LF[TY][NKH];
@@ -302,17 +330,18 @@
         constexpr int i = decltype(I)::value;
         unsigned ow[NW];
         if (i < nh) {
+            given_m(ma, mh[0], i);
             if constexpr (UNPACK1) {
                 words_to_pairs<DPL>(ch[i].w, chp[i]);
-                sgm_step_c<DPL, PIN>(chp[i], Aa, ma, ow, P1, P2, ea);
+                sgm_step_c<DPL, PIN, MN>(chp[i], Aa, ma, ow, P1, P2, ea);
             } else {
-                sgm_step<DPL, PIN>(ch[i].w, Aa, ma, ow, P1, P2, ea);
+                sgm_step<DPL, PIN, MN>(ch[i].w, Aa, ma, ow, P1, P2, ea);
             }
 #pragma unroll
             for (int q = 0; q < NKH; q++) LF[i][q] = KEEP16H ? Aa[q] : ow[q];
         }
     });
-    if (hx + TY < W) state_from_words<DPL, PAD, PIN>(ckw[1], Aa, ma, padm);
+    if (hx + TY < W) state_from_words<DPL, PAD, PIN, MN>(ckw[1], Aa, ma, padm);
     else zero_state(Aa, ma);
     unsigned dres = 0u, sm = 0u, s0 = 0u;
     const bool want_sub = sub != nullptr;
@@ -326,8 +355,9 @@
         constexpr int q = decltype(Q)::value, j = TY - 1 - q, s = q % kPfVol;
         if (j < nh) {
             unsigned ow[NW];
-            if constexpr (UNPACK1) sgm_step_c<DPL, PIN>(chp[UNPACK1 ? j : 0], Aa, ma, ow, P1, P2, ea);
-            else sgm_step<DPL, PIN>(ch[j].w, Aa, ma, ow, P1, P2, ea);
+            given_m(ma, mh[1], q);
+            if constexpr (UNPACK1) sgm_step_c<DPL, PIN, MN>(chp[UNPACK1 ? j : 0], Aa, ma, ow, P1, P2, ea);
+            else sgm_step<DPL, PIN, MN>(ch[j].w, Aa, ma, ow, P1, P2, ea);
             unsigned* const vpix = vrow + j * 16 * NP;
             unsigned S[NP];
 #pragma unroll
@@ -414,16 +444,30 @@
     }
 }
 
-template <int DPL, int TYL, bool PAIR>
+template <int DPL, int TYL, bool PAIR, bool MN>
+void wtahv_launch_mn(bool pad, dim3 grid, hipStream_t s, hipEvent_t start, hipEvent_t stop,
+                     const uint8_t* C, const uint8_t* L4, const uint8_t* CK, const uint8_t* CKV,
+                     const uint8_t* MNP, const WtaHvGeom& g, uint16_t* disp, float* sub) {
+    if (pad)
+        hipExtLaunchKernelGGL((wta_hv_kernel<DPL, TYL, true, PAIR, MN>), grid, dim3(TB), 0, s, start,
+                              stop, 0, C, L4, CK, CKV, MNP, g, disp, sub);
+    else
+        hipExtLaunchKernelGGL((wta_hv_kernel<DPL, TYL, false, PAIR, MN>), grid, dim3(TB), 0, s, start,
+                              stop, 0, C, L4, CK, CKV, MNP, g, disp, sub);
+}
+template <int DPL, int TYL, bool PAIR, bool MNEN>
 void wtahv_launch(bool pad, dim3 grid, hipStream_t s, hipEvent_t start, hipEvent_t stop,
                   const uint8_t* C, const uint8_t* L4, const uint8_t* CK, const uint8_t* CKV,
-                  const WtaHvGeom& g, uint16_t* disp, float* sub) {
-    if (pad)
-        hipExtLaunchKernelGGL((wta_hv_kernel<DPL, TYL, true, PAIR>), grid, dim3(TB), 0, s, start,
-                              stop, 0, C, L4, CK, CKV, g, disp, sub);
-    else
-        hipExtLaunchKernelGGL((wta_hv_kernel<DPL, TYL, false, PAIR>), grid, dim3(TB), 0, s, start,
-                              stop, 0, C, L4, CK, CKV, g, disp, sub);
+                  const uint8_t* MNP, const WtaHvGeom& g, uint16_t* disp, float* sub) {
+    if constexpr (MNEN) {
+        if (MNP) {
+            wtahv_launch_mn<DPL, TYL, PAIR, true>(pad, grid, s, start, stop, C, L4, CK, CKV, MNP, g,
+                                                  disp, sub);
+            return;
+        }
+    }
+    wtahv_launch_mn<DPL, TYL, PAIR, false>(pad, grid, s, start, stop, C, L4, CK, CKV, nullptr, g,
+                                           disp, sub);
 }
 
 }
@@ -432,7 +476,8 @@
 
 hipError_t launch_wta_hv(Ctx& c, const uint8_t* C, const uint8_t* L4, const uint8_t* CK,
                          const uint8_t* CKV, int W, int H, int D, int P1, int P2, int dmin,
-                         uint16_t* disp, float* sub, int dreal, int npair, bool pair) {
+                         uint16_t* disp, float* sub, int dreal, int npair, bool pair,
+                         const uint8_t* MN) {
     if (tune::kStripRoute != 0 && wta_strip_supported(D))
         return launch_wta_strip(c, C, CK, CKV, W, H, D, P1, P2, dmin, disp, sub, dreal, npair);
     DispatchTimer t(c, "wta_hv");
@@ -453,26 +498,30 @@
     if (npair < 1) return hipErrorInvalidValue;
     g.tiles = g.ntx * g.nty;
     const dim3 grid((unsigned)(g.tiles * npair));
-#define SVA_WTAHV(DPL_, TYL_)                                                                 \
-    wtahv_launch<DPL_, TYL_, false>(pad, grid, c.stream, t.start, t.stop, C, L4, CK, CKV, g,  \
-                                    disp, sub);                                               \
+#define SVA_WTAHV(DPL_, TYL_, MN_)                                                            \
+    wtahv_launch<DPL_, TYL_, false, (MN_) != 0>(pad, grid, c.stream, t.start, t.stop, C, L4,  \
+                                                CK, CKV, MN, g, disp, sub);                   \
     t.used = true
-#define SVA_WTAHV_P(DPL_, TYL_, EN_)                                                          \
+#define SVA_WTAHV_P(DPL_, TYL_, EN_, MN_)                                                     \
     if (pair) {                                                                               \
-        wtahv_launch<DPL_, TYL_, (EN_) != 0>(pad, grid, c.stream, t.start, t.stop, C, L4, CK, \
-                                             CKV, g, disp, sub);                              \
+        wtahv_launch<DPL_, TYL_, (EN_) != 0, (MN_) != 0>(pad, grid, c.stream, t.start,        \
+                                                         t.stop, C, L4, CK, CKV, MN, g, disp, \
+                                                         sub);                                \
         t.used = true;                                                                        \
     } else {                                                                                  \
-        SVA_WTAHV(DPL_, TYL_);                                                                \
+        SVA_WTAHV(DPL_, TYL_, MN_);                                                           \
     }
     constexpr int TYL = tune::kWtahvTileLog2, TYLW = tune::kWtahvTileLog2Wide;
     if (tg.seg_log2 != (D <= 128 ? TYL : TYLW)) return hipErrorInvalidValue;
     if (pair && (npair != 1 || !diag_pair_ok(D, P2) || tg.nvol != 4)) return hipErrorInvalidValue;
+    if (MN && (npair != 1 || !path_minima_enabled(D) || (1 << tg.seg_log2) != sgm::kMinimaSeg ||
+               tg.nvol != 4))
+        return hipErrorInvalidValue;
     switch (D) {
-        case 64: SVA_WTAHV_P(4, TYL, tune::kDiagPair4); break;
-        case 128: SVA_WTAHV_P(8, TYL, tune::kDiagPair8); break;
-        case 192: SVA_WTAHV_P(12, TYLW, tune::kDiagPair12); break;
-        case 256: SVA_WTAHV_P(16, TYLW, tune::kDiagPair16); break;
+        case 64: SVA_WTAHV_P(4, TYL, tune::kDiagPair4, tune::kPathMinima4); break;
+        case 128: SVA_WTAHV_P(8, TYL, tune::kDiagPair8, tune::kPathMinima8); break;
+        case 192: SVA_WTAHV_P(12, TYLW, tune::kDiagPair12, tune::kPathMinima12); break;
+        case 256: SVA_WTAHV_P(16, TYLW, tune::kDiagPair16, tune::kPathMinima16); break;
         default: return hipErrorInvalidValue;
     }
 #undef SVA_WTAHV_P
```

Result: faster. 335,300 (median of 6 runs) (+1.1%).
